# OpenGVLab/MM-Interleaved

Measured on NVIDIA H100. Metric: interleaved_steps_per_sec, higher is better.
Workload: dtype bf16

## Files before the change

include/mmfs_b200.h:

```cpp
#ifndef MMFS_B200_H_
#define MMFS_B200_H_

#include <stdint.h>

#ifdef __cplusplus
extern "C" {
#endif

#define MMFS_B200_ABI_VERSION 3

#define MMFS_OK            0
#define MMFS_EINVAL       (-1)
#define MMFS_EUNSUPPORTED (-2)
#define MMFS_ECUDA        (-3)

#define MMFS_F32  0
#define MMFS_F16  1
#define MMFS_BF16 2
#define MMFS_F64  3

#define MMFS_MSDA_STRICT 1u

#define MMFS_SAMPLER_EXACT_WEIGHTS 4u
#define MMFS_SAMPLER_GENERIC       8u

int mmfs_abi_version(void);
const char *mmfs_last_error(void);

int mmfs_msda_forward(const void *value, const int64_t *spatial_shapes, const int64_t *level_start,
                      const void *sampling_loc, const void *attn_weight, void *out,
                      int N, int S, int M, int D, int L, int Lq, int P,
                      int dtype, unsigned flags, void *stream);

int mmfs_msda_backward(const void *value, const int64_t *spatial_shapes, const int64_t *level_start,
                       const void *sampling_loc, const void *attn_weight, const void *grad_out,
                       float *grad_value, float *grad_loc, float *grad_attn,
                       int N, int S, int M, int D, int L, int Lq, int P, int dtype, void *stream);

int mmfs_msda_backward_deterministic(const void *value, const int64_t *spatial_shapes, const int64_t *level_start,
                                     const void *sampling_loc, const void *attn_weight, const void *grad_out,
                                     long long *grad_value_fixed, float *grad_value, float *grad_loc, float *grad_attn,
                                     float *scratch2, int N, int S, int M, int D, int L, int Lq, int P, int dtype, void *stream);

int mmfs_msda_index_stream(const int64_t *spatial_shapes, const int64_t *level_start,
                           const void *sampling_loc, int32_t *idx,
                           int N, int M, int D, int L, int Lq, int P,
                           int dtype, void *stream);

int mmfs_msda_forward_host(const void *value, const int64_t *spatial_shapes, const int64_t *level_start,
                           const void *sampling_loc, const void *attn_weight, void *out,
                           int N, int S, int M, int D, int L, int Lq, int P,
                           int dtype, unsigned flags, void *stream);
void mmfs_release_scratch(void);

int mmfs_sampler_forward(const void *value, const int64_t *shapes, const int64_t *starts,
                         const void *qproj, const void *rtable, const uint8_t *relpos,
                         const float *refpts, const float *scale_ratios, void *out, float *null_mass,
                         int N, int S, int M, int D, int n_img, int n_lvl, int Lq, int P,
                         int Lq_r, int Nr, int Lr, int R, int dtype, unsigned flags, void *stream);

int mmfs_sampler_locw(const int64_t *shapes, const int64_t *starts, const void *qproj, const void *rtable,
                      const uint8_t *relpos, const float *refpts, const float *scale_ratios,
                      void *loc_out, void *attn_out, float *null_mass,
                      int N, int M, int n_img, int n_lvl, int Lq, int P,
                      int Lq_r, int Nr, int Lr, int R, int dtype, void *stream);

int mmfs_rmsnorm(const void *x, const void *weight, void *y, long rows, int cols, float eps, int dtype, void *stream);
int mmfs_layernorm(const void *x, const void *weight, const void *bias, void *y, long rows, int cols, float eps,
                   int dtype, void *stream);
int mmfs_rope_qk(void *q, void *k, const float *cos_table, const float *sin_table, const int64_t *position_ids,
                 long n_tokens, int T_len, int H, int hd, int q_stride, int k_stride, int pos_per_batch,
                 int dtype, void *stream);
int mmfs_rope_qk_append(void *q, const void *k, const void *v, const float *cos_table, const float *sin_table,
                        const int64_t *position_ids, void *k_cache, void *v_cache, const int64_t *slot_dev, long slot_host,
                        long n_tokens, int T_len, int H, int hd, int q_stride, int k_stride, int v_stride, long cache_bs,
                        long cache_ts, int pos_per_batch, int dtype, void *stream);
int mmfs_swiglu(const void *gate_up, void *out, long rows, int inter, int dtype, void *stream);
int mmfs_geglu(const void *value_gate, void *out, long rows, int inter, int dtype, void *stream);

int mmfs_attn_generic(const void *q, const void *k, const void *v, void *out, const uint8_t *key_mask,
                      int B, int H, int Tq, int Tkv, int hd,
                      long q_bs, long q_ts, long k_bs, long k_ts, long v_bs, long v_ts, long o_bs, long o_ts,
                      float scale, int causal, int past, int dtype, void *stream);
long mmfs_attn_decode_scratch_floats(int B, int H, int Tkv, int hd);
int mmfs_attn_decode(const void *q, const void *k, const void *v, void *out, const uint8_t *key_mask, float *scratch,
                     int B, int H, int Tkv, int hd, long q_bs, long k_bs, long k_ts, long v_bs, long v_ts, long o_bs,
                     float scale, int causal, int past, int dtype, void *stream);
int mmfs_attn_decode_shared(const void *q, const void *k_prefix, const void *v_prefix, const void *k_gen, const void *v_gen,
                            void *out, const uint8_t *key_mask, const long long *prefix_len, float *scratch,
                            int R, int G, int H, int Tkv, int Tp, int max_new, int hd, long q_bs,
                            long kp_bs, long kp_ts, long vp_bs, long vp_ts, long kg_bs, long kg_ts, long vg_bs, long vg_ts,
                            long o_bs, float scale, int causal, int past, int dtype, void *stream);

int mmfs_attn_forward(const void *q, const void *k, const void *v, void *out, const uint8_t *key_mask,
                      int B, int H, int Tq, int Tkv, int hd,
                      long q_bs, long q_ts, long k_bs, long k_ts, long v_bs, long v_ts, long o_bs, long o_ts,
                      float scale, int causal, int past, int dtype, unsigned *work_counter, void *stream);

int mmfs_attn_forward_lse(const void *q, const void *k, const void *v, void *out, float *lse, const uint8_t *key_mask,
                          int B, int H, int Tq, int Tkv, int hd,
                          long q_bs, long q_ts, long k_bs, long k_ts, long v_bs, long v_ts, long o_bs, long o_ts,
                          float scale, int causal, int past, int dtype, unsigned *work_counter, void *stream);

int mmfs_attn_backward(const void *q, const void *k, const void *v, const void *out, const void *d_out, const float *lse,
                       void *dq, void *dk, void *dv, float *delta, const uint8_t *key_mask, int B, int H, int T, int hd,
                       long q_bs, long q_ts, long k_bs, long k_ts, long v_bs, long v_ts, long o_bs, long o_ts,
                       long do_bs, long do_ts, long dq_bs, long dq_ts, long dk_bs, long dk_ts, long dv_bs, long dv_ts,
                       float scale, int dtype, void *stream);

int mmfs_attn_backward_general(const void *q, const void *k, const void *v, const void *out, const void *d_out,
                               const float *lse, void *dq, void *dk, void *dv, float *delta, const uint8_t *key_mask,
                               int B, int H, int Tq, int Tkv, int hd, long q_bs, long q_ts, long k_bs, long k_ts, long v_bs,
                               long v_ts, long o_bs, long o_ts, long do_bs, long do_ts, long dq_bs, long dq_ts, long dk_bs,
                               long dk_ts, long dv_bs, long dv_ts, float scale, int causal, int dtype, void *stream);

int mmfs_layernorm_backward(const void *x, const void *weight, const void *dy, void *dx, void *dweight, void *dbias,
                            float *partials, long rows, int cols, float eps, int dtype, void *stream);

#define MMFS_RMSNORM_BWD_PARTS 256
int mmfs_rmsnorm_backward(const void *x, const void *weight, const void *dy, void *dx, void *dweight, float *partials,
                          long rows, int cols, float eps, int dtype, void *stream);

int mmfs_swiglu_backward(const void *gate_up, const void *d_out, void *d_gate_up, long rows, int inter, int dtype,
                         void *stream);

int mmfs_geglu_backward(const void *value_gate, const void *d_out, void *d_value_gate, long rows, int inter, int dtype,
                        void *stream);

int mmfs_quick_gelu_backward(const void *h, const void *dy, void *dh, long n, int dtype, void *stream);

int mmfs_resize_bilinear_backward(const void *dy, void *dx, int B, int C, int Hin, int Win, int Hout, int Wout, long dy_bs,
                                  long dy_cs, long dy_ps, float scale_h, float scale_w, int dtype, void *stream);

int mmfs_conv2d_nhwc(const void *x, const void *w, const void *bias, const void *add_bc, const void *residual, void *out,
                     int B, int H, int W, int Cin, int Cout, int KH, int KW, int stride, int pad, int dtype, void *stream);

int mmfs_conv2d_up2x_nhwc(const void *x, const void *w_phases, const void *bias, void *out, int B, int H, int W, int Cin,
                          int Cout, int dtype, void *stream);

int mmfs_conv2d_down2x_nhwc(const void *x, const void *w, const void *bias, void *out, int B, int H, int W, int Cin,
                            int Cout, int dtype, void *stream);

int mmfs_groupnorm_nhwc(const void *x, const void *gamma, const void *beta, void *y, float *stats, int B, int HW, int C,
                        int G, float eps, int silu, int dtype, void *stream);

int mmfs_groupnorm_nhwc_backward(const void *x, const void *gamma, const void *beta, const void *dy, void *dx,
                                 float *scratch, int B, int HW, int C, int G, float eps, int silu, int dtype, void *stream);

#define MMFS_SELECT_GREEDY 0
#define MMFS_SELECT_SAMPLE 1

int mmfs_decode_select(const float *logits, long ld, int64_t *out_ids, const int64_t *step, uint8_t *finished,
                       int64_t *next_ids, const int64_t *eos_ids, int n_eos, long pad_id, int min_length,
                       const float *params, const int64_t *seed, const float *uniforms, int B, int V, int max_new,
                       int mode, void *stream);

int mmfs_beam_select(const float *logits, long ld, const int64_t *step, const double *params, float *beam_scores,
                     int64_t *history, int64_t *next_ids, int64_t *parent, uint8_t *done, double *hyp_scores,
                     int64_t *hyp_ids, int64_t *hyp_meta, const int64_t *eos_ids, int n_eos, long pad_id, int min_length,
                     uint64_t *scratch, int B, int num_beams, int V, int max_new, void *stream);

int mmfs_beam_sample(const float *logits, long ld, const int64_t *step, const double *params, const int64_t *seed,
                     const float *uniforms, float *beam_scores, int64_t *history, int64_t *next_ids, int64_t *parent,
                     uint8_t *done, double *hyp_scores, int64_t *hyp_ids, int64_t *hyp_meta, int32_t *error,
                     const int64_t *eos_ids, int n_eos, long pad_id, int min_length, int top_k, uint64_t *scratch, int B,
                     int num_beams, int V, int max_new, void *stream);

int mmfs_kv_beam_reorder(void *cache, int n_caches, long cache_stride, int rows, long row_stride, long pos_stride,
                         long row_bytes, int num_beams, const int64_t *parent, const int64_t *cur, const int64_t *step,
                         const uint8_t *done, int max_positions, void *stream);

int mmfs_image_reentry(const float *images, float *out, int N, int C, int H, int W, int R, void *stream);

int mmfs_linear_fp8(const void *x, const uint8_t *w8, const float *scale, const void *bias, const void *residual,
                    void *out, int M, int N, int K, int dtype, void *stream);

int mmfs_rope_qk_append_fp8(void *q, void *k, void *v, const float *cos_table, const float *sin_table,
                            const int64_t *position_ids, uint8_t *k_cache, uint8_t *v_cache, float *k_scale, float *v_scale,
                            const int64_t *slot_dev, long slot_host, long n_tokens, int T_len, int H, int hd, int q_stride,
                            int k_stride, int v_stride, long cache_bs, long cache_ts, long scale_bs, long scale_ts,
                            int pos_per_batch, int dtype, void *stream);
int mmfs_attn_decode_fp8(const void *q, const uint8_t *k, const uint8_t *v, const float *k_scale, const float *v_scale,
                         void *out, const uint8_t *key_mask, float *scratch, int B, int H, int Tkv, int hd, long q_bs,
                         long kv_bs, long kv_ts, long s_bs, long s_ts, long o_bs, float scale, int causal, int past,
                         int dtype, void *stream);
int mmfs_attn_decode_shared_fp8(const void *q, const uint8_t *k_prefix, const uint8_t *v_prefix, const float *ks_prefix,
                                const float *vs_prefix, const uint8_t *k_gen, const uint8_t *v_gen, const float *ks_gen,
                                const float *vs_gen, void *out, const uint8_t *key_mask, const long long *prefix_len,
                                float *scratch, int R, int G, int H, int Tkv, int Tp, int max_new, int hd, long q_bs,
                                long p_bs, long p_ts, long ps_bs, long ps_ts, long g_bs, long g_ts, long gs_bs, long gs_ts,
                                long o_bs, float scale, int causal, int past, int dtype, void *stream);
int mmfs_kv_dequantize_fp8(const uint8_t *x8, const float *scale, void *out, int B, int T_len, int H, int hd, long x_bs,
                           long x_ts, long s_bs, long s_ts, long o_bs, long o_ts, int dtype, void *stream);

#ifdef __cplusplus
}
#endif
#endif
```

mm-interleaved_b200/_lib.py:

```python
from __future__ import annotations

import ctypes
import os

_HERE = os.path.dirname(os.path.abspath(__file__))
LIB_PATH = os.environ.get("MMFS_B200_LIB", os.path.join(_HERE, "libmmfs_b200.so"))

OK, EINVAL, EUNSUPPORTED, ECUDA = 0, -1, -2, -3
F32, F16, BF16, F64 = 0, 1, 2, 3
MSDA_STRICT = 1
SAMPLER_EXACT_WEIGHTS = 4
SAMPLER_GENERIC = 8
SELECT_GREEDY, SELECT_SAMPLE = 0, 1

_lib = None

_I, _U, _P = ctypes.c_int, ctypes.c_uint, ctypes.c_void_p
_L, _F = ctypes.c_long, ctypes.c_float

SIGNATURES = {
    "mmfs_abi_version": (_I, []),
    "mmfs_last_error": (ctypes.c_char_p, []),
    "mmfs_msda_forward": (_I, [_P, _P, _P, _P, _P, _P, _I, _I, _I, _I, _I, _I, _I, _I, _U, _P]),
    "mmfs_msda_backward": (_I, [_P] * 9 + [_I] * 8 + [_P]),
    "mmfs_msda_backward_deterministic": (_I, [_P] * 11 + [_I] * 8 + [_P]),
    "mmfs_msda_index_stream": (_I, [_P, _P, _P, _P, _I, _I, _I, _I, _I, _I, _I, _P]),
    "mmfs_msda_forward_host": (_I, [_P, _P, _P, _P, _P, _P, _I, _I, _I, _I, _I, _I, _I, _I, _U, _P]),
    "mmfs_release_scratch": (None, []),
    "mmfs_sampler_forward": (_I, [_P] * 10 + [_I] * 13 + [_U, _P]),
    "mmfs_sampler_locw": (_I, [_P] * 10 + [_I] * 11 + [_P]),
    "mmfs_rmsnorm": (_I, [_P, _P, _P, _L, _I, _F, _I, _P]),
    "mmfs_layernorm": (_I, [_P, _P, _P, _P, _L, _I, _F, _I, _P]),
    "mmfs_rope_qk": (_I, [_P, _P, _P, _P, _P, _L, _I, _I, _I, _I, _I, _I, _I, _P]),
    "mmfs_rope_qk_append": (_I, [_P] * 9 + [_L, _L] + [_I] * 6 + [_L, _L, _I, _I, _P]),
    "mmfs_swiglu": (_I, [_P, _P, _L, _I, _I, _P]),
    "mmfs_geglu": (_I, [_P, _P, _L, _I, _I, _P]),
    "mmfs_attn_generic": (_I, [_P] * 5 + [_I] * 5 + [_L] * 8 + [_F, _I, _I, _I, _P]),
    "mmfs_groupnorm_nhwc": (_I, [_P] * 5 + [_I] * 4 + [_F, _I, _I, _P]),
    "mmfs_groupnorm_nhwc_backward": (_I, [_P] * 6 + [_I] * 4 + [_F, _I, _I, _P]),
    "mmfs_conv2d_nhwc": (_I, [_P] * 6 + [_I] * 10 + [_P]),
    "mmfs_conv2d_up2x_nhwc": (_I, [_P] * 4 + [_I] * 6 + [_P]),
    "mmfs_conv2d_down2x_nhwc": (_I, [_P] * 4 + [_I] * 6 + [_P]),
    "mmfs_attn_decode_scratch_floats": (_L, [_I] * 4),
    "mmfs_attn_decode": (_I, [_P] * 6 + [_I] * 4 + [_L] * 6 + [_F, _I, _I, _I, _P]),
    "mmfs_attn_decode_shared": (_I, [_P] * 9 + [_I] * 7 + [_L] * 10 + [_F, _I, _I, _I, _P]),
    "mmfs_attn_forward": (_I, [_P] * 5 + [_I] * 5 + [_L] * 8 + [_F, _I, _I, _I, _P, _P]),
    "mmfs_attn_forward_lse": (_I, [_P] * 6 + [_I] * 5 + [_L] * 8 + [_F, _I, _I, _I, _P, _P]),
    "mmfs_attn_backward": (_I, [_P] * 11 + [_I] * 4 + [_L] * 16 + [_F, _I, _P]),
    "mmfs_attn_backward_general": (_I, [_P] * 11 + [_I] * 5 + [_L] * 16 + [_F, _I, _I, _P]),
    "mmfs_rmsnorm_backward": (_I, [_P] * 6 + [_L, _I, _F, _I, _P]),
    "mmfs_layernorm_backward": (_I, [_P] * 7 + [_L, _I, _F, _I, _P]),
    "mmfs_swiglu_backward": (_I, [_P] * 3 + [_L, _I, _I, _P]),
    "mmfs_geglu_backward": (_I, [_P] * 3 + [_L, _I, _I, _P]),
    "mmfs_quick_gelu_backward": (_I, [_P] * 3 + [_L, _I, _P]),
    "mmfs_resize_bilinear_backward": (_I, [_P] * 2 + [_I] * 6 + [_L] * 3 + [_F, _F, _I, _P]),
    "mmfs_decode_select": (_I, [_P, _L] + [_P] * 5 + [_I, _L, _I] + [_P] * 3 + [_I] * 4 + [_P]),
    "mmfs_beam_select": (_I, [_P, _L] + [_P] * 11 + [_I, _L, _I, _P] + [_I] * 4 + [_P]),
    "mmfs_beam_sample": (_I, [_P, _L] + [_P] * 14 + [_I, _L, _I, _I, _P] + [_I] * 4 + [_P]),
    "mmfs_kv_beam_reorder": (_I, [_P, _I, _L, _I, _L, _L, _L, _I] + [_P] * 4 + [_I, _P]),
    "mmfs_image_reentry": (_I, [_P, _P] + [_I] * 5 + [_P]),
    "mmfs_linear_fp8": (_I, [_P] * 6 + [_I] * 4 + [_P]),
    "mmfs_rope_qk_append_fp8": (_I, [_P] * 11 + [_L, _L] + [_I] * 6 + [_L] * 4 + [_I, _I, _P]),
    "mmfs_attn_decode_fp8": (_I, [_P] * 8 + [_I] * 4 + [_L] * 6 + [_F, _I, _I, _I, _P]),
    "mmfs_attn_decode_shared_fp8": (_I, [_P] * 13 + [_I] * 7 + [_L] * 10 + [_F, _I, _I, _I, _P]),
    "mmfs_kv_dequantize_fp8": (_I, [_P] * 3 + [_I] * 4 + [_L] * 6 + [_I, _P]),
}
BEAM_MAX_BEAMS, BEAM_MAX_EOS = 8, 4
LINEAR_FP8_MAX_M = 64
RMSNORM_BWD_PARTS = 256


def lib() -> ctypes.CDLL:
    global _lib
    if _lib is None:
        if not os.path.exists(LIB_PATH):
            raise RuntimeError(
                f"libmmfs_b200.so not found at {LIB_PATH}: build it with "
                "`python mm-interleaved_b200/build.py` (there is no CPU / PyTorch fallback)")
        handle = ctypes.CDLL(LIB_PATH)
        for name, (res, args) in SIGNATURES.items():
            fn = getattr(handle, name)
            fn.restype = res
            fn.argtypes = args
        if handle.mmfs_abi_version() != 3:
            raise RuntimeError(f"libmmfs_b200.so ABI {handle.mmfs_abi_version()} != 3")
        _lib = handle
    return _lib


def check(rc: int, what: str) -> None:
    if rc != OK:
        msg = lib().mmfs_last_error().decode("utf-8", "replace")
        kind = {EINVAL: "invalid argument", EUNSUPPORTED: "unsupported", ECUDA: "CUDA error"}.get(rc, "error")
        raise RuntimeError(f"{what}: {kind} ({rc}): {msg}")
```

mm-interleaved_b200/csrc/llama_ops_sm100.cu:

```cuda
#include "common.cuh"

namespace mmfs {

template <typename T> __device__ __forceinline__ float rnd(float x) { return to_op(from_op<T>(x)); }
template <> __device__ __forceinline__ float rnd<float>(float x) { return x; }

__device__ __forceinline__ float block_sum(float v, float *s_red) {
#pragma unroll
    for (int o = 16; o > 0; o >>= 1) v += __shfl_xor_sync(0xffffffffu, v, o);
    const int lane = threadIdx.x & 31, warp = threadIdx.x >> 5, nw = (blockDim.x + 31) >> 5;
    if (lane == 0) s_red[warp] = v;
    __syncthreads();
    float t = (lane < nw) ? s_red[lane] : 0.f;
#pragma unroll
    for (int o = 16; o > 0; o >>= 1) t += __shfl_xor_sync(0xffffffffu, t, o);
    __syncthreads();
    return t;
}

template <typename T>
__global__ void __launch_bounds__(256) rmsnorm_kernel(const T *__restrict__ x, const T *__restrict__ w,
                                                       T *__restrict__ y, int cols, float eps) {
    constexpr int VEC = 16 / (int)sizeof(T);
    __shared__ float s_red[32];
    const size_t row = blockIdx.x;
    const T *xr = x + row * cols;
    T *yr = y + row * cols;
    const int nvec = cols / VEC;
    float ss = 0.f;
    for (int i = threadIdx.x; i < nvec; i += blockDim.x) {
        float f[VEC];
        Vec16<T>::unpack(*reinterpret_cast<const uint4 *>(xr + i * VEC), f);
#pragma unroll
        for (int k = 0; k < VEC; ++k) ss += f[k] * f[k];
    }
    for (int i = nvec * VEC + threadIdx.x; i < cols; i += blockDim.x) { const float v = to_op(xr[i]); ss += v * v; }
    const float var = block_sum(ss, s_red) / (float)cols;
    const float r = rsqrtf(var + eps);
    for (int i = threadIdx.x; i < nvec; i += blockDim.x) {
        float f[VEC], g[VEC], o[VEC];
        Vec16<T>::unpack(*reinterpret_cast<const uint4 *>(xr + i * VEC), f);
        Vec16<T>::unpack(*reinterpret_cast<const uint4 *>(w + i * VEC), g);
#pragma unroll
        for (int k = 0; k < VEC; ++k) o[k] = g[k] * rnd<T>(f[k] * r);
        *reinterpret_cast<uint4 *>(yr + i * VEC) = Vec16<T>::pack(o);
    }
    for (int i = nvec * VEC + threadIdx.x; i < cols; i += blockDim.x)
        yr[i] = from_op<T>(to_op(w[i]) * rnd<T>(to_op(xr[i]) * r));
}

constexpr int kRmsChunks = 8;
constexpr int kRmsThreads = 128;

template <typename T>
__global__ void __launch_bounds__(kRmsThreads) rmsnorm_reg_kernel(const T *__restrict__ x, const T *__restrict__ w,
                                                                  T *__restrict__ y, int cols, float eps) {
    constexpr int VEC = 16 / (int)sizeof(T);
    __shared__ float s_red[kRmsThreads / 32];
    const size_t row = blockIdx.x;
    const T *xr = x + row * cols;
    T *yr = y + row * cols;
    const int nvec = cols / VEC;
    uint4 v[kRmsChunks], wv[kRmsChunks];
#pragma unroll
    for (int c = 0; c < kRmsChunks; ++c) {
        const int i = threadIdx.x + c * kRmsThreads;
        if (i < nvec) {
            v[c] = ldg_nc_v4(xr + i * VEC);
            wv[c] = ldg_nc_v4(w + i * VEC);
        }
    }
    float ss = 0.f;
#pragma unroll
    for (int c = 0; c < kRmsChunks; ++c)
        if (threadIdx.x + c * kRmsThreads < nvec) {
            float f[VEC];
            Vec16<T>::unpack(v[c], f);
#pragma unroll
            for (int k = 0; k < VEC; ++k) ss = fmaf(f[k], f[k], ss);
        }
#pragma unroll
    for (int o = 16; o > 0; o >>= 1) ss += __shfl_xor_sync(0xffffffffu, ss, o);
    if ((threadIdx.x & 31) == 0) s_red[threadIdx.x >> 5] = ss;
    __syncthreads();
    float tot = 0.f;
#pragma unroll
    for (int i = 0; i < kRmsThreads / 32; ++i) tot += s_red[i];
    const float r = rsqrtf(tot / (float)cols + eps);
#pragma unroll
    for (int c = 0; c < kRmsChunks; ++c) {
        const int i = threadIdx.x + c * kRmsThreads;
        if (i < nvec) {
            float f[VEC], g[VEC], o[VEC];
            Vec16<T>::unpack(v[c], f);
            Vec16<T>::unpack(wv[c], g);
#pragma unroll
            for (int k = 0; k < VEC; ++k) o[k] = g[k] * rnd<T>(f[k] * r);
            stg_v4(yr + i * VEC, Vec16<T>::pack(o));
        }
    }
}

constexpr int kLnChunks = 8;

template <typename T, int CH>
__global__ void __launch_bounds__(256, CH == 8 ? 2 : 4) layernorm_warp_kernel(const T *__restrict__ x, const T *__restrict__ w,
                                                              const T *__restrict__ b, T *__restrict__ y, long rows, int cols, float eps) {
    constexpr int VEC = 16 / (int)sizeof(T);
    const int lane = threadIdx.x & 31;
    const long row = (long)blockIdx.x * (blockDim.x >> 5) + (threadIdx.x >> 5);
    if (row >= rows) return;
    const T *xr = x + row * cols;
    T *yr = y + row * cols;
    const int nvec = cols / VEC;
    uint4 v[CH];
#pragma unroll
    for (int c = 0; c < CH; ++c) {
        const int i = lane + 32 * c;
        v[c] = (i < nvec) ? ldg_nc_v4(xr + i * VEC) : make_uint4(0u, 0u, 0u, 0u);
    }
    float s = 0.f;
#pragma unroll
    for (int c = 0; c < CH; ++c) {
        float f[VEC];
        Vec16<T>::unpack(v[c], f);
#pragma unroll
        for (int k = 0; k < VEC; ++k) s += f[k];
    }
#pragma unroll
    for (int o = 16; o > 0; o >>= 1) s += __shfl_xor_sync(0xffffffffu, s, o);
    const float mean = s / (float)cols;
    float ss = 0.f;
#pragma unroll
    for (int c = 0; c < CH; ++c)
        if (lane + 32 * c < nvec) {
            float f[VEC];
            Vec16<T>::unpack(v[c], f);
#pragma unroll
            for (int k = 0; k < VEC; ++k) { const float d = f[k] - mean; ss = fmaf(d, d, ss); }
        }
#pragma unroll
    for (int o = 16; o > 0; o >>= 1) ss += __shfl_xor_sync(0xffffffffu, ss, o);
    const float r = rsqrtf(ss / (float)cols + eps);
#pragma unroll
    for (int c = 0; c < CH; ++c) {
        const int i = lane + 32 * c;
        if (i < nvec) {
            float f[VEC], g[VEC], bb[VEC], o[VEC];
            Vec16<T>::unpack(v[c], f);
            if (w) Vec16<T>::unpack(*reinterpret_cast<const uint4 *>(w + i * VEC), g);
            if (b) Vec16<T>::unpack(*reinterpret_cast<const uint4 *>(b + i * VEC), bb);
#pragma unroll
            for (int k = 0; k < VEC; ++k) o[k] = (f[k] - mean) * r * (w ? g[k] : 1.f) + (b ? bb[k] : 0.f);
            stg_v4(yr + i * VEC, Vec16<T>::pack(o));
        }
    }
}

template <typename T>
__global__ void __launch_bounds__(256) layernorm_kernel(const T *__restrict__ x, const T *__restrict__ w,
                                                         const T *__restrict__ b, T *__restrict__ y, int cols, float eps) {
    __shared__ float s_red[32];
    const size_t row = blockIdx.x;
    const T *xr = x + row * cols;
    T *yr = y + row * cols;
    float s = 0.f;
    for (int i = threadIdx.x; i < cols; i += blockDim.x) s += to_op(xr[i]);
    const float mean = block_sum(s, s_red) / (float)cols;
    float ss = 0.f;
    for (int i = threadIdx.x; i < cols; i += blockDim.x) { const float d = to_op(xr[i]) - mean; ss += d * d; }
    const float r = rsqrtf(block_sum(ss, s_red) / (float)cols + eps);
    for (int i = threadIdx.x; i < cols; i += blockDim.x) {
        const float n = (to_op(xr[i]) - mean) * r;
        yr[i] = from_op<T>(n * (w ? to_op(w[i]) : 1.f) + (b ? to_op(b[i]) : 0.f));
    }
}

template <typename T>
__global__ void __launch_bounds__(256) rope_qk_kernel(T *__restrict__ q, T *__restrict__ k, const float *__restrict__ cos_t,
                                                       const float *__restrict__ sin_t, const int64_t *__restrict__ pos,
                                                       long n_tok, int H, int hd, int q_stride, int k_stride, int pos_per_batch,
                                                       int T_len) {
    constexpr int VEC = 16 / (int)sizeof(T);
    const int half = hd >> 1;
    const int chunks = half / VEC;
    const int per_tok = 2 * H * chunks;
    const bool hoist = (blockDim.x % chunks) == 0;
    for (long tok = blockIdx.x; tok < n_tok; tok += gridDim.x) {
        const long p = pos[pos_per_batch ? tok : (tok % T_len)];
        const float *cp = cos_t + p * hd, *sp = sin_t + p * hd;
        T *qt = q + tok * q_stride, *kt = k + tok * k_stride;
        float cs[VEC], sn[VEC];
        auto load_table = [&](int c) {
#pragma unroll
            for (int i = 0; i < VEC; i += 4) {
                const float4 a = *reinterpret_cast<const float4 *>(cp + c * VEC + i);
                const float4 b = *reinterpret_cast<const float4 *>(sp + c * VEC + i);
                cs[i] = rnd<T>(a.x); cs[i + 1] = rnd<T>(a.y); cs[i + 2] = rnd<T>(a.z); cs[i + 3] = rnd<T>(a.w);
                sn[i] = rnd<T>(b.x); sn[i + 1] = rnd<T>(b.y); sn[i + 2] = rnd<T>(b.z); sn[i + 3] = rnd<T>(b.w);
            }
        };
        if (hoist) load_table(threadIdx.x % chunks);
        for (int it = threadIdx.x; it < per_tok; it += blockDim.x) {
            const int c = it % chunks;
            const int hh = it / chunks;
            T *x = (hh >= H ? kt + (size_t)(hh - H) * hd : qt + (size_t)hh * hd) + c * VEC;
            float x1[VEC], x2[VEC], o1[VEC], o2[VEC];
            const uint4 v1 = *reinterpret_cast<const uint4 *>(x), v2 = *reinterpret_cast<const uint4 *>(x + half);
            if (!hoist) load_table(c);
            Vec16<T>::unpack(v1, x1);
            Vec16<T>::unpack(v2, x2);
#pragma unroll
            for (int i = 0; i < VEC; ++i) {
                o1[i] = rnd<T>(x1[i] * cs[i]) + rnd<T>(-x2[i] * sn[i]);
                o2[i] = rnd<T>(x2[i] * cs[i]) + rnd<T>(x1[i] * sn[i]);
            }
            *reinterpret_cast<uint4 *>(x) = Vec16<T>::pack(o1);
            *reinterpret_cast<uint4 *>(x + half) = Vec16<T>::pack(o2);
        }
    }
}

template <typename T>
__global__ void __launch_bounds__(256) rope_append_kernel(T *__restrict__ q, const T *__restrict__ k, const T *__restrict__ v,
                                                           const float *__restrict__ cos_t, const float *__restrict__ sin_t,
                                                           const int64_t *__restrict__ pos, T *__restrict__ k_cache,
                                                           T *__restrict__ v_cache, const int64_t *__restrict__ slot_dev,
                                                           long slot_host, long n_tok, int H, int hd, int q_stride, int k_stride,
                                                           int v_stride, long cache_bs, long cache_ts, int pos_per_batch, int T_len) {
    constexpr int VEC = 16 / (int)sizeof(T);
    const int half = hd >> 1;
    const int chunks = half / VEC;
    const int n_rot = 2 * H * chunks;
    const int n_copy = H * hd / VEC;
    const long slot = slot_dev != nullptr ? (long)*slot_dev : slot_host;
    for (long tok = blockIdx.x; tok < n_tok; tok += gridDim.x) {
        const long p = pos[pos_per_batch ? tok : (tok % T_len)];
        const float *cp = cos_t + p * hd, *sp = sin_t + p * hd;
        const long b = tok / T_len, tt = tok - b * T_len;
        T *qt = q + tok * q_stride;
        const T *kt = k + tok * k_stride, *vt = v + tok * v_stride;
        T *kc = k_cache + b * cache_bs + (slot + tt) * cache_ts, *vc = v_cache + b * cache_bs + (slot + tt) * cache_ts;
        for (int it = threadIdx.x; it < n_rot + n_copy; it += blockDim.x) {
            if (it >= n_rot) {
                const int i = (it - n_rot) * VEC;
                *reinterpret_cast<uint4 *>(vc + i) = *reinterpret_cast<const uint4 *>(vt + i);
                continue;
            }
            const int c = it % chunks, hh = it / chunks;
            const bool is_k = hh >= H;
            const T *src = (is_k ? kt + (size_t)(hh - H) * hd : qt + (size_t)hh * hd) + c * VEC;
            T *dst = (is_k ? kc + (size_t)(hh - H) * hd : qt + (size_t)hh * hd) + c * VEC;
            float cs[VEC], sn[VEC], x1[VEC], x2[VEC], o1[VEC], o2[VEC];
#pragma unroll
            for (int i = 0; i < VEC; i += 4) {
                const float4 a = *reinterpret_cast<const float4 *>(cp + c * VEC + i);
                const float4 bb = *reinterpret_cast<const float4 *>(sp + c * VEC + i);
                cs[i] = rnd<T>(a.x); cs[i + 1] = rnd<T>(a.y); cs[i + 2] = rnd<T>(a.z); cs[i + 3] = rnd<T>(a.w);
                sn[i] = rnd<T>(bb.x); sn[i + 1] = rnd<T>(bb.y); sn[i + 2] = rnd<T>(bb.z); sn[i + 3] = rnd<T>(bb.w);
            }
            Vec16<T>::unpack(*reinterpret_cast<const uint4 *>(src), x1);
            Vec16<T>::unpack(*reinterpret_cast<const uint4 *>(src + half), x2);
#pragma unroll
            for (int i = 0; i < VEC; ++i) {
                o1[i] = rnd<T>(x1[i] * cs[i]) + rnd<T>(-x2[i] * sn[i]);
                o2[i] = rnd<T>(x2[i] * cs[i]) + rnd<T>(x1[i] * sn[i]);
            }
            *reinterpret_cast<uint4 *>(dst) = Vec16<T>::pack(o1);
            *reinterpret_cast<uint4 *>(dst + half) = Vec16<T>::pack(o2);
        }
    }
}

template <typename T> __device__ __forceinline__ float silu_op(float g) { return __fdividef(g, 1.f + __expf(-g)); }
template <> __device__ __forceinline__ float silu_op<float>(float g) { return g / (1.f + expf(-g)); }

template <typename T, int ACT> __device__ __forceinline__ float glu_act(float g) {
    if (ACT == 0) return silu_op<T>(g);
    return 0.5f * g * (1.f + erff(g * 0.70710678118654752f));
}

template <typename T, int ACT = 0, bool GATE_SECOND = false>
__global__ void __launch_bounds__(256) swiglu_kernel(const T *__restrict__ gu, T *__restrict__ out, long rows, int I) {
    constexpr int VEC = 16 / (int)sizeof(T);
    const int per = (I / VEC + gridDim.y - 1) / gridDim.y;
    const int v0 = blockIdx.y * per, nvec = min(I / VEC, v0 + per);
    for (long r = blockIdx.x; r < rows; r += gridDim.x) {
        const T *g_row = gu + r * 2 * I + (GATE_SECOND ? I : 0), *u_row = gu + r * 2 * I + (GATE_SECOND ? 0 : I);
        T *o_row = out + r * I;
        int i = v0 + threadIdx.x;
        for (; i + (int)blockDim.x < nvec; i += 2 * blockDim.x) {
            const int j = i + blockDim.x;
            const uint4 g0 = ldg_nc_v4(g_row + i * VEC), u0 = ldg_nc_v4(u_row + i * VEC);
            const uint4 g1 = ldg_nc_v4(g_row + j * VEC), u1 = ldg_nc_v4(u_row + j * VEC);
            float g[VEC], u[VEC], o[VEC];
            Vec16<T>::unpack(g0, g); Vec16<T>::unpack(u0, u);
#pragma unroll
            for (int k = 0; k < VEC; ++k) o[k] = rnd<T>(glu_act<T, ACT>(g[k])) * u[k];
            stg_v4(o_row + i * VEC, Vec16<T>::pack(o));
            Vec16<T>::unpack(g1, g); Vec16<T>::unpack(u1, u);
#pragma unroll
            for (int k = 0; k < VEC; ++k) o[k] = rnd<T>(glu_act<T, ACT>(g[k])) * u[k];
            stg_v4(o_row + j * VEC, Vec16<T>::pack(o));
        }
        if (i < nvec) {
            float g[VEC], u[VEC], o[VEC];
            Vec16<T>::unpack(ldg_nc_v4(g_row + i * VEC), g); Vec16<T>::unpack(ldg_nc_v4(u_row + i * VEC), u);
#pragma unroll
            for (int k = 0; k < VEC; ++k) o[k] = rnd<T>(glu_act<T, ACT>(g[k])) * u[k];
            stg_v4(o_row + i * VEC, Vec16<T>::pack(o));
        }
    }
}

template <typename T>
static int launch_rmsnorm(const void *x, const void *w, void *y, long rows, int cols, float eps, cudaStream_t st) {
    if (cols % (16 / (int)sizeof(T)) == 0 && cols / (16 / (int)sizeof(T)) <= kRmsThreads * kRmsChunks)
        rmsnorm_reg_kernel<T><<<(unsigned)rows, kRmsThreads, 0, st>>>((const T *)x, (const T *)w, (T *)y, cols, eps);
    else
        rmsnorm_kernel<T><<<(unsigned)rows, 256, 0, st>>>((const T *)x, (const T *)w, (T *)y, cols, eps);
    MMFS_CUDA(cudaGetLastError());
    return MMFS_OK;
}

template <typename T>
static int launch_layernorm(const void *x, const void *w, const void *b, void *y, long rows, int cols, float eps, cudaStream_t st) {
    constexpr int VEC = 16 / (int)sizeof(T);
    const bool vec_ok = (cols % VEC == 0) && (cols / VEC <= 32 * kLnChunks) &&
                        (((uintptr_t)x | (uintptr_t)y | (uintptr_t)w | (uintptr_t)b) % 16 == 0);
    if (vec_ok) {
        const int nvec = cols / VEC;
        const unsigned grid = (unsigned)((rows + 7) / 8);
#define MMFS_LN(CH) layernorm_warp_kernel<T, CH><<<grid, 256, 0, st>>>((const T *)x, (const T *)w, (const T *)b, (T *)y, rows, cols, eps)
        if (nvec <= 32) MMFS_LN(1); else if (nvec <= 64) MMFS_LN(2); else if (nvec <= 128) MMFS_LN(4); else MMFS_LN(8);
#undef MMFS_LN
    } else
        layernorm_kernel<T><<<(unsigned)rows, 256, 0, st>>>((const T *)x, (const T *)w, (const T *)b, (T *)y, cols, eps);
    MMFS_CUDA(cudaGetLastError());
    return MMFS_OK;
}

template <typename T>
static int launch_rope(void *q, void *k, const float *cos_t, const float *sin_t, const int64_t *pos, long n_tok, int T_len,
                       int H, int hd, int qs, int ks, int ppb, cudaStream_t st) {
    const int per_tok = H * 2 * ((hd / 2) / (16 / (int)sizeof(T)));
    const int threads = per_tok >= 256 ? 256 : ((per_tok + 31) / 32) * 32;
    rope_qk_kernel<T><<<capped_grid(n_tok, 32), threads, 0, st>>>((T *)q, (T *)k, cos_t, sin_t, pos, n_tok, H, hd, qs, ks, ppb,
                                                                  T_len);
    MMFS_CUDA(cudaGetLastError());
    return MMFS_OK;
}

template <typename T>
static int launch_glu(const void *in, void *out, long rows, int inter, bool geglu, cudaStream_t st) {
    const int nvec = inter / (16 / (int)sizeof(T));
    const int threads = nvec >= 512 ? 256 : (nvec >= 64 ? 64 : 32);
    const int gx = capped_grid(rows, 64);
    int gy = 1;
    if (gx < num_sms()) { gy = (nvec + 2 * threads - 1) / (2 * threads); if (gy > 64) gy = 64; if (gy < 1) gy = 1; }
    const dim3 grid(gx, gy);
    if (geglu)
        swiglu_kernel<T, 1, true><<<grid, threads, 0, st>>>((const T *)in, (T *)out, rows, inter);
    else
        swiglu_kernel<T, 0, false><<<grid, threads, 0, st>>>((const T *)in, (T *)out, rows, inter);
    MMFS_CUDA(cudaGetLastError());
    return MMFS_OK;
}

template <typename T>
static int launch_rope_append(void *q, const void *k, const void *v, const float *cos_t, const float *sin_t, const int64_t *pos,
                              void *kc, void *vc, const int64_t *slot_dev, long slot_host, long n_tok, int T_len, int H, int hd,
                              int qs, int ks, int vs, long cbs, long cts, int ppb, cudaStream_t st) {
    const int items = H * ((hd / 2) / (16 / (int)sizeof(T))) * 2 + H * hd / (16 / (int)sizeof(T));
    const int threads = items >= 256 ? 256 : ((items + 31) / 32) * 32;
    rope_append_kernel<T><<<capped_grid(n_tok, 32), threads, 0, st>>>((T *)q, (const T *)k, (const T *)v, cos_t, sin_t, pos, (T *)kc,
                                                                      (T *)vc, slot_dev, slot_host, n_tok, H, hd, qs, ks, vs, cbs,
                                                                      cts, ppb, T_len);
    MMFS_CUDA(cudaGetLastError());
    return MMFS_OK;
}


constexpr int kRmsBwdParts = MMFS_RMSNORM_BWD_PARTS;
constexpr int kRmsBwdMaxCols = 8192;

template <typename T>
__global__ void __launch_bounds__(256) rmsnorm_bwd_kernel(const T *__restrict__ x, const T *__restrict__ w,
                                                          const T *__restrict__ dy, T *__restrict__ dx,
                                                          float *__restrict__ partials, long rows, int cols, float eps) {
    constexpr int VEC = 16 / (int)sizeof(T);
    extern __shared__ float s_dw[];
    __shared__ float s_red[32];
    const int nvec = cols / VEC;
    if (partials)
        for (int i = threadIdx.x; i < nvec; i += blockDim.x)
#pragma unroll
            for (int k = 0; k < VEC; ++k) s_dw[i * VEC + k] = 0.f;
    for (long row = blockIdx.x; row < rows; row += gridDim.x) {
        const T *xr = x + row * cols, *dyr = dy + row * cols;
        float ss = 0.f, sg = 0.f;
        for (int i = threadIdx.x; i < nvec; i += blockDim.x) {
            float f[VEC], g[VEC], d[VEC];
            Vec16<T>::unpack(ldg_nc_v4(xr + i * VEC), f);
            Vec16<T>::unpack(ldg_nc_v4(w + i * VEC), g);
            Vec16<T>::unpack(ldg_nc_v4(dyr + i * VEC), d);
#pragma unroll
            for (int k = 0; k < VEC; ++k) { ss = fmaf(f[k], f[k], ss); sg = fmaf(d[k] * g[k], f[k], sg); }
        }
        ss = block_sum(ss, s_red);
        sg = block_sum(sg, s_red);
        const float r = rsqrtf(ss / (float)cols + eps);
        const float coef = r * r * r * sg / (float)cols;
        for (int i = threadIdx.x; i < nvec; i += blockDim.x) {
            float f[VEC], g[VEC], d[VEC], o[VEC];
            Vec16<T>::unpack(ldg_nc_v4(xr + i * VEC), f);
            Vec16<T>::unpack(ldg_nc_v4(w + i * VEC), g);
            Vec16<T>::unpack(ldg_nc_v4(dyr + i * VEC), d);
#pragma unroll
            for (int k = 0; k < VEC; ++k) o[k] = fmaf(r * d[k], g[k], -f[k] * coef);
            stg_v4(dx + row * cols + i * VEC, Vec16<T>::pack(o));
            if (partials)
#pragma unroll
                for (int k = 0; k < VEC; ++k) s_dw[i * VEC + k] = fmaf(d[k], rnd<T>(f[k] * r), s_dw[i * VEC + k]);
        }
    }
    if (partials)
        for (int i = threadIdx.x; i < nvec; i += blockDim.x)
#pragma unroll
            for (int k = 0; k < VEC; ++k) partials[(long)blockIdx.x * cols + i * VEC + k] = s_dw[i * VEC + k];
}

template <typename T>
__global__ void __launch_bounds__(256) rmsnorm_dw_reduce_kernel(const float *__restrict__ partials, T *__restrict__ dw,
                                                                int parts, int cols) {
    const int c = blockIdx.x * blockDim.x + threadIdx.x;
    if (c >= cols) return;
    float s = 0.f;
    for (int p = 0; p < parts; ++p) s += partials[(long)p * cols + c];
    dw[c] = from_op<T>(s);
}

template <typename T>
__global__ void __launch_bounds__(256) layernorm_bwd_kernel(const T *__restrict__ x, const T *__restrict__ w,
                                                            const T *__restrict__ dy, T *__restrict__ dx,
                                                            float *__restrict__ partials, long rows, int cols, float eps) {
    constexpr int VEC = 16 / (int)sizeof(T);
    extern __shared__ float s_part[];
    __shared__ float s_red[32];
    const int nvec = cols / VEC;
    float *s_dw = s_part, *s_db = s_part + cols;
    if (partials)
        for (int i = threadIdx.x; i < nvec; i += blockDim.x)
#pragma unroll
            for (int k = 0; k < VEC; ++k) s_dw[i * VEC + k] = s_db[i * VEC + k] = 0.f;
    const float inv_n = 1.f / (float)cols;
    for (long row = blockIdx.x; row < rows; row += gridDim.x) {
        const T *xr = x + row * cols, *dyr = dy + row * cols;
        float s = 0.f;
        for (int i = threadIdx.x; i < nvec; i += blockDim.x) {
            float f[VEC];
            Vec16<T>::unpack(ldg_nc_v4(xr + i * VEC), f);
#pragma unroll
            for (int k = 0; k < VEC; ++k) s += f[k];
        }
        const float mean = block_sum(s, s_red) * inv_n;
        float ss = 0.f, sg = 0.f, sgx = 0.f;
        for (int i = threadIdx.x; i < nvec; i += blockDim.x) {
            float f[VEC], g[VEC], d[VEC];
            Vec16<T>::unpack(ldg_nc_v4(xr + i * VEC), f);
            Vec16<T>::unpack(ldg_nc_v4(w + i * VEC), g);
            Vec16<T>::unpack(ldg_nc_v4(dyr + i * VEC), d);
#pragma unroll
            for (int k = 0; k < VEC; ++k) {
                const float c = f[k] - mean, gk = d[k] * g[k];
                ss = fmaf(c, c, ss);
                sg += gk;
                sgx = fmaf(gk, c, sgx);
            }
        }
        ss = block_sum(ss, s_red);
        sg = block_sum(sg, s_red);
        sgx = block_sum(sgx, s_red);
        const float r = rsqrtf(ss * inv_n + eps);
        const float mg = sg * inv_n, mgx = sgx * r * inv_n;
        for (int i = threadIdx.x; i < nvec; i += blockDim.x) {
            float f[VEC], g[VEC], d[VEC], o[VEC];
            Vec16<T>::unpack(ldg_nc_v4(xr + i * VEC), f);
            Vec16<T>::unpack(ldg_nc_v4(w + i * VEC), g);
            Vec16<T>::unpack(ldg_nc_v4(dyr + i * VEC), d);
#pragma unroll
            for (int k = 0; k < VEC; ++k) {
                const float xh = (f[k] - mean) * r;
                o[k] = r * (fmaf(d[k], g[k], -mg) - xh * mgx);
                if (partials) {
                    s_dw[i * VEC + k] = fmaf(d[k], xh, s_dw[i * VEC + k]);
                    s_db[i * VEC + k] += d[k];
                }
            }
            stg_v4(dx + row * cols + i * VEC, Vec16<T>::pack(o));
        }
    }
    if (partials)
        for (int i = threadIdx.x; i < nvec; i += blockDim.x)
#pragma unroll
            for (int k = 0; k < VEC; ++k) {
                partials[(long)blockIdx.x * cols + i * VEC + k] = s_dw[i * VEC + k];
                partials[((long)gridDim.x + blockIdx.x) * cols + i * VEC + k] = s_db[i * VEC + k];
            }
}

template <typename T>
__global__ void __launch_bounds__(256) layernorm_dwdb_reduce_kernel(const float *__restrict__ partials, T *__restrict__ dw,
                                                                    T *__restrict__ db, int parts, int cols) {
    const int c = blockIdx.x * blockDim.x + threadIdx.x;
    if (c >= cols) return;
    float sw = 0.f, sb = 0.f;
    for (int p = 0; p < parts; ++p) {
        sw += partials[(long)p * cols + c];
        sb += partials[((long)parts + p) * cols + c];
    }
    if (dw) dw[c] = from_op<T>(sw);
    if (db) db[c] = from_op<T>(sb);
}

template <typename T>
__global__ void __launch_bounds__(256) swiglu_bwd_kernel(const T *__restrict__ gu, const T *__restrict__ d_out,
                                                         T *__restrict__ d_gu, long rows, int I) {
    constexpr int VEC = 16 / (int)sizeof(T);
    const int nvec = I / VEC;
    for (long r = blockIdx.x; r < rows; r += gridDim.x)
        for (int i = threadIdx.x; i < nvec; i += blockDim.x) {
            float g[VEC], u[VEC], d[VEC], dg[VEC], du[VEC];
            Vec16<T>::unpack(ldg_nc_v4(gu + r * 2 * I + i * VEC), g);
            Vec16<T>::unpack(ldg_nc_v4(gu + r * 2 * I + I + i * VEC), u);
            Vec16<T>::unpack(ldg_nc_v4(d_out + r * I + i * VEC), d);
#pragma unroll
            for (int k = 0; k < VEC; ++k) {
                const float s = 1.f / (1.f + expf(-g[k]));
                dg[k] = d[k] * u[k] * s * fmaf(g[k], 1.f - s, 1.f);
                du[k] = d[k] * g[k] * s;
            }
            stg_v4(d_gu + r * 2 * I + i * VEC, Vec16<T>::pack(dg));
            stg_v4(d_gu + r * 2 * I + I + i * VEC, Vec16<T>::pack(du));
        }
}

__device__ __forceinline__ void geglu_grad(float v, float g, float d, float &dv, float &dg) {
    const float cdf = 0.5f * (1.f + erff(g * 0.70710678118654752f));
    const float pdf = 0.39894228040143268f * expf(-0.5f * g * g);
    dv = d * g * cdf;
    dg = d * v * fmaf(g, pdf, cdf);
}

template <typename T, bool kVec>
__global__ void __launch_bounds__(256) geglu_bwd_kernel(const T *__restrict__ vg, const T *__restrict__ d_out,
                                                        T *__restrict__ d_vg, long rows, int I) {
    constexpr int VEC = kVec ? 16 / (int)sizeof(T) : 1;
    const long per_row = I / VEC, n = rows * per_row;
    const long stride = (long)gridDim.x * blockDim.x;
    for (long t = (long)blockIdx.x * blockDim.x + threadIdx.x; t < n; t += stride) {
        const long r = t / per_row, i = (t - r * per_row) * VEC;
        const long v_at = r * 2 * I + i, g_at = v_at + I;
        float v[VEC], g[VEC], d[VEC], dv[VEC], dg[VEC];
        if constexpr (kVec) {
            Vec16<T>::unpack(ldg_nc_v4(vg + v_at), v);
            Vec16<T>::unpack(ldg_nc_v4(vg + g_at), g);
            Vec16<T>::unpack(ldg_nc_v4(d_out + r * I + i), d);
        } else {
            v[0] = to_op(vg[v_at]);
            g[0] = to_op(vg[g_at]);
            d[0] = to_op(d_out[r * I + i]);
        }
#pragma unroll
        for (int k = 0; k < VEC; ++k) geglu_grad(v[k], g[k], d[k], dv[k], dg[k]);
        if constexpr (kVec) {
            stg_v4(d_vg + v_at, Vec16<T>::pack(dv));
            stg_v4(d_vg + g_at, Vec16<T>::pack(dg));
        } else {
            d_vg[v_at] = from_op<T>(dv[0]);
            d_vg[g_at] = from_op<T>(dg[0]);
        }
    }
}

template <typename T>
static int launch_geglu_bwd(const void *vg, const void *d_out, void *d_vg, long rows, int inter, bool vec, cudaStream_t st) {
    const long items = rows * (vec ? inter / (16 / (int)sizeof(T)) : inter);
    const int grid = capped_grid((items + 255) / 256, 8);
    if (vec)
        geglu_bwd_kernel<T, true><<<grid, 256, 0, st>>>((const T *)vg, (const T *)d_out, (T *)d_vg, rows, inter);
    else
        geglu_bwd_kernel<T, false><<<grid, 256, 0, st>>>((const T *)vg, (const T *)d_out, (T *)d_vg, rows, inter);
    MMFS_CUDA(cudaGetLastError());
    return MMFS_OK;
}

template <typename T>
static int launch_rmsnorm_bwd(const void *x, const void *w, const void *dy, void *dx, void *dw, float *partials, long rows,
                              int cols, float eps, cudaStream_t st) {
    const int parts = (int)(rows < kRmsBwdParts ? rows : kRmsBwdParts);
    rmsnorm_bwd_kernel<T><<<parts, 256, dw ? cols * sizeof(float) : 0, st>>>(
        (const T *)x, (const T *)w, (const T *)dy, (T *)dx, dw ? partials : nullptr, rows, cols, eps);
    MMFS_CUDA(cudaGetLastError());
    if (dw) {
        rmsnorm_dw_reduce_kernel<T><<<(cols + 255) / 256, 256, 0, st>>>(partials, (T *)dw, parts, cols);
        MMFS_CUDA(cudaGetLastError());
    }
    return MMFS_OK;
}

template <typename T>
static int launch_layernorm_bwd(const void *x, const void *w, const void *dy, void *dx, void *dw, void *db, float *partials,
                                long rows, int cols, float eps, cudaStream_t st) {
    const int parts = (int)(rows < kRmsBwdParts ? rows : kRmsBwdParts);
    const int nvec = cols / (16 / (int)sizeof(T));
    const int threads = nvec >= 256 ? 256 : (nvec + 31) / 32 * 32;
    const bool red = dw != nullptr || db != nullptr;
    const size_t smem = red ? 2 * (size_t)cols * sizeof(float) : 0;
    const int rc = ensure_dynamic_smem<layernorm_bwd_kernel<T>>(smem);
    if (rc != MMFS_OK) return rc;
    layernorm_bwd_kernel<T><<<parts, threads, smem, st>>>((const T *)x, (const T *)w, (const T *)dy, (T *)dx,
                                                           red ? partials : nullptr, rows, cols, eps);
    MMFS_CUDA(cudaGetLastError());
    if (red) {
        layernorm_dwdb_reduce_kernel<T><<<(cols + 255) / 256, 256, 0, st>>>(partials, (T *)dw, (T *)db, parts, cols);
        MMFS_CUDA(cudaGetLastError());
    }
    return MMFS_OK;
}

template <typename T>
static int launch_swiglu_bwd(const void *gu, const void *d_out, void *d_gu, long rows, int inter, cudaStream_t st) {
    swiglu_bwd_kernel<T><<<capped_grid(rows, 8), 256, 0, st>>>((const T *)gu, (const T *)d_out, (T *)d_gu, rows, inter);
    MMFS_CUDA(cudaGetLastError());
    return MMFS_OK;
}

}

using namespace mmfs;

extern "C" int mmfs_rmsnorm(const void *x, const void *weight, void *y, long rows, int cols, float eps, int dtype, void *stream) {
    MMFS_CHECK_ARG(rows >= 0 && cols > 0, "rmsnorm: bad shape");
    if (rows == 0) return MMFS_OK;
    MMFS_CHECK_ARG(x && weight && y, "rmsnorm: null pointer argument");
    MMFS_CHECK_ARG(((uintptr_t)x | (uintptr_t)weight | (uintptr_t)y) % 16 == 0 && (cols * dtype_size(dtype)) % 16 == 0,
                   "rmsnorm: rows must be 16-byte aligned");
    return dispatch_dtype<kF32Types>(dtype, "rmsnorm", [&](auto tag) {
        return launch_rmsnorm<typename decltype(tag)::type>(x, weight, y, rows, cols, eps, (cudaStream_t)stream);
    });
}

extern "C" int mmfs_layernorm(const void *x, const void *weight, const void *bias, void *y, long rows, int cols, float eps,
                              int dtype, void *stream) {
    MMFS_CHECK_ARG(rows >= 0 && cols > 0, "layernorm: bad shape");
    if (rows == 0) return MMFS_OK;
    MMFS_CHECK_ARG(x && y, "layernorm: null pointer argument");
    return dispatch_dtype<kF32Types>(dtype, "layernorm", [&](auto tag) {
        return launch_layernorm<typename decltype(tag)::type>(x, weight, bias, y, rows, cols, eps, (cudaStream_t)stream);
    });
}

extern "C" int mmfs_rope_qk(void *q, void *k, const float *cos_table, const float *sin_table, const int64_t *position_ids,
                            long n_tokens, int T_len, int H, int hd, int q_stride, int k_stride, int pos_per_batch,
                            int dtype, void *stream) {
    MMFS_CHECK_ARG(n_tokens >= 0 && H > 0 && hd > 0 && hd % 2 == 0 && T_len > 0, "rope_qk: bad shape");
    if (n_tokens == 0) return MMFS_OK;
    MMFS_CHECK_ARG(q && k && cos_table && sin_table && position_ids, "rope_qk: null pointer argument");
    MMFS_CHECK_ARG((hd / 2) % (16 / (int)dtype_size(dtype)) == 0 && ((uintptr_t)q | (uintptr_t)k) % 16 == 0 &&
                   (q_stride * dtype_size(dtype)) % 16 == 0 && (k_stride * dtype_size(dtype)) % 16 == 0,
                   "rope_qk: head_dim/2 must be a multiple of the 16-byte vector and rows 16-byte aligned");
    return dispatch_dtype<kF32Types>(dtype, "rope_qk", [&](auto tag) {
        return launch_rope<typename decltype(tag)::type>(q, k, cos_table, sin_table, position_ids, n_tokens, T_len, H, hd, q_stride,
                                                         k_stride, pos_per_batch, (cudaStream_t)stream);
    });
}

extern "C" int mmfs_rope_qk_append(void *q, const void *k, const void *v, const float *cos_table, const float *sin_table,
                                   const int64_t *position_ids, void *k_cache, void *v_cache, const int64_t *slot_dev,
                                   long slot_host, long n_tokens, int T_len, int H, int hd, int q_stride, int k_stride,
                                   int v_stride, long cache_bs, long cache_ts, int pos_per_batch, int dtype, void *stream) {
    MMFS_CHECK_ARG(n_tokens >= 0 && H > 0 && hd > 0 && hd % 2 == 0 && T_len > 0 && slot_host >= 0, "rope_qk_append: bad shape");
    if (n_tokens == 0) return MMFS_OK;
    MMFS_CHECK_ARG(q && k && v && cos_table && sin_table && position_ids && k_cache && v_cache, "rope_qk_append: null pointer argument");
    const size_t es = dtype_size(dtype);
    MMFS_CHECK_ARG(es == 2 || es == 4, "rope_qk_append: f32 / f16 / bf16");
    MMFS_CHECK_ARG((hd / 2) % (16 / (int)es) == 0 &&
                       ((uintptr_t)q | (uintptr_t)k | (uintptr_t)v | (uintptr_t)k_cache | (uintptr_t)v_cache) % 16 == 0 &&
                       (q_stride * es) % 16 == 0 && (k_stride * es) % 16 == 0 && (v_stride * es) % 16 == 0 &&
                       (cache_bs * es) % 16 == 0 && (cache_ts * es) % 16 == 0,
                   "rope_qk_append: head_dim/2 must be a multiple of the 16-byte vector and all rows 16-byte aligned");
    return dispatch_dtype<kF32Types>(dtype, "rope_qk_append", [&](auto tag) {
        return launch_rope_append<typename decltype(tag)::type>(q, k, v, cos_table, sin_table, position_ids, k_cache, v_cache,
                                                                slot_dev, slot_host, n_tokens, T_len, H, hd, q_stride, k_stride,
                                                                v_stride, cache_bs, cache_ts, pos_per_batch, (cudaStream_t)stream);
    });
}

extern "C" int mmfs_swiglu(const void *gate_up, void *out, long rows, int inter, int dtype, void *stream) {
    MMFS_CHECK_ARG(rows >= 0 && inter > 0, "swiglu: bad shape");
    if (rows == 0) return MMFS_OK;
    MMFS_CHECK_ARG(gate_up && out, "swiglu: null pointer argument");
    MMFS_CHECK_ARG(((uintptr_t)gate_up | (uintptr_t)out) % 16 == 0 && (inter * dtype_size(dtype)) % 16 == 0,
                   "swiglu: rows must be 16-byte aligned");
    return dispatch_dtype<kF32Types>(dtype, "swiglu", [&](auto tag) {
        return launch_glu<typename decltype(tag)::type>(gate_up, out, rows, inter, false, (cudaStream_t)stream);
    });
}

extern "C" int mmfs_geglu(const void *value_gate, void *out, long rows, int inter, int dtype, void *stream) {
    MMFS_CHECK_ARG(rows >= 0 && inter > 0, "geglu: bad shape");
    if (rows == 0) return MMFS_OK;
    MMFS_CHECK_ARG(value_gate && out, "geglu: null pointer argument");
    MMFS_CHECK_ARG(((uintptr_t)value_gate | (uintptr_t)out) % 16 == 0 && (inter * dtype_size(dtype)) % 16 == 0,
                   "geglu: rows must be 16-byte aligned");
    return dispatch_dtype<kF32Types>(dtype, "geglu", [&](auto tag) {
        return launch_glu<typename decltype(tag)::type>(value_gate, out, rows, inter, true, (cudaStream_t)stream);
    });
}

extern "C" int mmfs_rmsnorm_backward(const void *x, const void *weight, const void *dy, void *dx, void *dweight,
                                     float *partials, long rows, int cols, float eps, int dtype, void *stream) {
    MMFS_CHECK_ARG(rows >= 0 && cols > 0, "rmsnorm_backward: bad shape");
    if (rows == 0) return MMFS_OK;
    MMFS_CHECK_ARG(x && weight && dy && dx && (!dweight || partials), "rmsnorm_backward: null pointer argument");
    if (!(dtype == MMFS_BF16 || dtype == MMFS_F16) || cols % 8 != 0 || cols > kRmsBwdMaxCols ||
        ((uintptr_t)x | (uintptr_t)weight | (uintptr_t)dy | (uintptr_t)dx) % 16 != 0) {
        set_error("rmsnorm_backward: needs bf16 / f16, cols %% 8 == 0, cols <= %d, 16-byte aligned rows (got cols=%d dtype=%d)",
                  kRmsBwdMaxCols, cols, dtype);
        return MMFS_EUNSUPPORTED;
    }
    return dispatch_dtype<kF16Types, MMFS_EUNSUPPORTED>(dtype, "rmsnorm_backward", [&](auto tag) {
        return launch_rmsnorm_bwd<typename decltype(tag)::type>(x, weight, dy, dx, dweight, partials, rows, cols, eps,
                                                                (cudaStream_t)stream);
    });
}

extern "C" int mmfs_swiglu_backward(const void *gate_up, const void *d_out, void *d_gate_up, long rows, int inter, int dtype,
                                    void *stream) {
    MMFS_CHECK_ARG(rows >= 0 && inter > 0, "swiglu_backward: bad shape");
    if (rows == 0) return MMFS_OK;
    MMFS_CHECK_ARG(gate_up && d_out && d_gate_up, "swiglu_backward: null pointer argument");
    if (!(dtype == MMFS_BF16 || dtype == MMFS_F16) || inter % 8 != 0 ||
        ((uintptr_t)gate_up | (uintptr_t)d_out | (uintptr_t)d_gate_up) % 16 != 0) {
        set_error("swiglu_backward: needs bf16 / f16, inter %% 8 == 0 and 16-byte aligned rows (got inter=%d dtype=%d)", inter, dtype);
        return MMFS_EUNSUPPORTED;
    }
    return dispatch_dtype<kF16Types, MMFS_EUNSUPPORTED>(dtype, "swiglu_backward", [&](auto tag) {
        return launch_swiglu_bwd<typename decltype(tag)::type>(gate_up, d_out, d_gate_up, rows, inter, (cudaStream_t)stream);
    });
}

extern "C" int mmfs_geglu_backward(const void *value_gate, const void *d_out, void *d_value_gate, long rows, int inter,
                                   int dtype, void *stream) {
    MMFS_CHECK_ARG(rows >= 0 && inter > 0, "geglu_backward: bad shape");
    if (rows == 0) return MMFS_OK;
    MMFS_CHECK_ARG(value_gate && d_out && d_value_gate, "geglu_backward: null pointer argument");
    if (!(dtype == MMFS_BF16 || dtype == MMFS_F16)) {
        set_error("geglu_backward: needs bf16 / f16 (got dtype=%d)", dtype);
        return MMFS_EUNSUPPORTED;
    }
    const bool vec = inter % 8 == 0 && ((uintptr_t)value_gate | (uintptr_t)d_out | (uintptr_t)d_value_gate) % 16 == 0;
    return dispatch_dtype<kF16Types, MMFS_EUNSUPPORTED>(dtype, "geglu_backward", [&](auto tag) {
        return launch_geglu_bwd<typename decltype(tag)::type>(value_gate, d_out, d_value_gate, rows, inter, vec,
                                                              (cudaStream_t)stream);
    });
}

extern "C" int mmfs_layernorm_backward(const void *x, const void *weight, const void *dy, void *dx, void *dweight, void *dbias,
                                       float *partials, long rows, int cols, float eps, int dtype, void *stream) {
    MMFS_CHECK_ARG(rows >= 0 && cols > 0, "layernorm_backward: bad shape");
    if (rows == 0) return MMFS_OK;
    MMFS_CHECK_ARG(x && weight && dy && dx && (!(dweight || dbias) || partials), "layernorm_backward: null pointer argument");
    if (!(dtype == MMFS_BF16 || dtype == MMFS_F16) || cols % 8 != 0 || cols > kRmsBwdMaxCols ||
        ((uintptr_t)x | (uintptr_t)weight | (uintptr_t)dy | (uintptr_t)dx) % 16 != 0) {
        set_error("layernorm_backward: needs bf16 / f16, cols %% 8 == 0, cols <= %d, 16-byte aligned rows (got cols=%d dtype=%d)",
                  kRmsBwdMaxCols, cols, dtype);
        return MMFS_EUNSUPPORTED;
    }
    return dispatch_dtype<kF16Types, MMFS_EUNSUPPORTED>(dtype, "layernorm_backward", [&](auto tag) {
        return launch_layernorm_bwd<typename decltype(tag)::type>(x, weight, dy, dx, dweight, dbias, partials, rows, cols, eps,
                                                                  (cudaStream_t)stream);
    });
}
```

mm-interleaved_b200/csrc/tc_common.cuh:

```cuda
#pragma once
#include <cuda.h>

#include "common.cuh"

namespace mmfs {

__device__ __forceinline__ void tma_load_4d(void *dst, const CUtensorMap *map, uint64_t *bar, int c0, int c1, int c2, int c3) {
    asm volatile(
        "cp.async.bulk.tensor.4d.shared::cluster.global.mbarrier::complete_tx::bytes [%0], [%1, {%3, %4, %5, %6}], [%2];" ::
        "r"(s_addr(dst)), "l"(map), "r"(s_addr(bar)), "r"(c0), "r"(c1), "r"(c2), "r"(c3) : "memory");
}
__device__ __forceinline__ void fence_async_smem() { asm volatile("fence.proxy.async.shared::cta;" ::: "memory"); }

__device__ __forceinline__ void wgmma_fence() { asm volatile("wgmma.fence.sync.aligned;" ::: "memory"); }
__device__ __forceinline__ void wgmma_commit() { asm volatile("wgmma.commit_group.sync.aligned;" ::: "memory"); }
template <int N> __device__ __forceinline__ void wgmma_wait() { asm volatile("wgmma.wait_group.sync.aligned %0;" ::"n"(N) : "memory"); }
template <int N> __device__ __forceinline__ void reg_fence(float (&d)[N]) {
#pragma unroll
    for (int i = 0; i < N; ++i) asm volatile("" : "+f"(d[i])::"memory");
}

__device__ __forceinline__ uint64_t smem_desc(uint32_t saddr, uint32_t lbo_bytes, uint32_t sbo_bytes) {
    return (uint64_t)((saddr >> 4) & 0x3fffu) | ((uint64_t)((lbo_bytes >> 4) & 0x3fffu) << 16) |
           ((uint64_t)((sbo_bytes >> 4) & 0x3fffu) << 32) | (1ull << 62);
}

template <typename T> struct Wgmma;
#define MMFS_WGMMA_OPS(TY) \
     \
    __device__ __forceinline__ static void ss_n64(float (&d)[32], uint64_t da, uint64_t db, int acc) { \
        asm volatile( \
            "{\n\t.reg .pred p;\n\tsetp.ne.b32 p, %34, 0;\n\t" \
            "wgmma.mma_async.sync.aligned.m64n64k16.f32." TY "." TY " {%0,%1,%2,%3,%4,%5,%6,%7,%8,%9,%10,%11,%12,%13,%14,%15,%16,%17,%18,%19,%20,%21,%22,%23,%24,%25,%26,%27,%28,%29,%30,%31}, %32, %33, p, 1, 1, 0, 0;\n\t}" \
            : "+f"(d[0]), "+f"(d[1]), "+f"(d[2]), "+f"(d[3]), "+f"(d[4]), "+f"(d[5]), "+f"(d[6]), "+f"(d[7]), "+f"(d[8]), "+f"(d[9]), "+f"(d[10]), "+f"(d[11]), "+f"(d[12]), "+f"(d[13]), "+f"(d[14]), "+f"(d[15]), "+f"(d[16]), "+f"(d[17]), "+f"(d[18]), "+f"(d[19]), "+f"(d[20]), "+f"(d[21]), "+f"(d[22]), "+f"(d[23]), "+f"(d[24]), "+f"(d[25]), "+f"(d[26]), "+f"(d[27]), "+f"(d[28]), "+f"(d[29]), "+f"(d[30]), "+f"(d[31]) \
            : "l"(da), "l"(db), "r"(acc)); \
    } \
     \
    __device__ __forceinline__ static void ss_n128(float (&d)[64], uint64_t da, uint64_t db, int acc) { \
        asm volatile( \
            "{\n\t.reg .pred p;\n\tsetp.ne.b32 p, %66, 0;\n\t" \
            "wgmma.mma_async.sync.aligned.m64n128k16.f32." TY "." TY " {%0,%1,%2,%3,%4,%5,%6,%7,%8,%9,%10,%11,%12,%13,%14,%15,%16,%17,%18,%19,%20,%21,%22,%23,%24,%25,%26,%27,%28,%29,%30,%31,%32,%33,%34,%35,%36,%37,%38,%39,%40,%41,%42,%43,%44,%45,%46,%47,%48,%49,%50,%51,%52,%53,%54,%55,%56,%57,%58,%59,%60,%61,%62,%63}, %64, %65, p, 1, 1, 0, 0;\n\t}" \
            : "+f"(d[0]), "+f"(d[1]), "+f"(d[2]), "+f"(d[3]), "+f"(d[4]), "+f"(d[5]), "+f"(d[6]), "+f"(d[7]), "+f"(d[8]), "+f"(d[9]), "+f"(d[10]), "+f"(d[11]), "+f"(d[12]), "+f"(d[13]), "+f"(d[14]), "+f"(d[15]), "+f"(d[16]), "+f"(d[17]), "+f"(d[18]), "+f"(d[19]), "+f"(d[20]), "+f"(d[21]), "+f"(d[22]), "+f"(d[23]), "+f"(d[24]), "+f"(d[25]), "+f"(d[26]), "+f"(d[27]), "+f"(d[28]), "+f"(d[29]), "+f"(d[30]), "+f"(d[31]), "+f"(d[32]), "+f"(d[33]), "+f"(d[34]), "+f"(d[35]), "+f"(d[36]), "+f"(d[37]), "+f"(d[38]), "+f"(d[39]), "+f"(d[40]), "+f"(d[41]), "+f"(d[42]), "+f"(d[43]), "+f"(d[44]), "+f"(d[45]), "+f"(d[46]), "+f"(d[47]), "+f"(d[48]), "+f"(d[49]), "+f"(d[50]), "+f"(d[51]), "+f"(d[52]), "+f"(d[53]), "+f"(d[54]), "+f"(d[55]), "+f"(d[56]), "+f"(d[57]), "+f"(d[58]), "+f"(d[59]), "+f"(d[60]), "+f"(d[61]), "+f"(d[62]), "+f"(d[63]) \
            : "l"(da), "l"(db), "r"(acc)); \
    } \
     \
    __device__ __forceinline__ static void ss_n160(float (&d)[80], uint64_t da, uint64_t db, int acc) { \
        asm volatile( \
            "{\n\t.reg .pred p;\n\tsetp.ne.b32 p, %82, 0;\n\t" \
            "wgmma.mma_async.sync.aligned.m64n160k16.f32." TY "." TY " {%0,%1,%2,%3,%4,%5,%6,%7,%8,%9,%10,%11,%12,%13,%14,%15,%16,%17,%18,%19,%20,%21,%22,%23,%24,%25,%26,%27,%28,%29,%30,%31,%32,%33,%34,%35,%36,%37,%38,%39,%40,%41,%42,%43,%44,%45,%46,%47,%48,%49,%50,%51,%52,%53,%54,%55,%56,%57,%58,%59,%60,%61,%62,%63,%64,%65,%66,%67,%68,%69,%70,%71,%72,%73,%74,%75,%76,%77,%78,%79}, %80, %81, p, 1, 1, 0, 0;\n\t}" \
            : "+f"(d[0]), "+f"(d[1]), "+f"(d[2]), "+f"(d[3]), "+f"(d[4]), "+f"(d[5]), "+f"(d[6]), "+f"(d[7]), "+f"(d[8]), "+f"(d[9]), "+f"(d[10]), "+f"(d[11]), "+f"(d[12]), "+f"(d[13]), "+f"(d[14]), "+f"(d[15]), "+f"(d[16]), "+f"(d[17]), "+f"(d[18]), "+f"(d[19]), "+f"(d[20]), "+f"(d[21]), "+f"(d[22]), "+f"(d[23]), "+f"(d[24]), "+f"(d[25]), "+f"(d[26]), "+f"(d[27]), "+f"(d[28]), "+f"(d[29]), "+f"(d[30]), "+f"(d[31]), "+f"(d[32]), "+f"(d[33]), "+f"(d[34]), "+f"(d[35]), "+f"(d[36]), "+f"(d[37]), "+f"(d[38]), "+f"(d[39]), "+f"(d[40]), "+f"(d[41]), "+f"(d[42]), "+f"(d[43]), "+f"(d[44]), "+f"(d[45]), "+f"(d[46]), "+f"(d[47]), "+f"(d[48]), "+f"(d[49]), "+f"(d[50]), "+f"(d[51]), "+f"(d[52]), "+f"(d[53]), "+f"(d[54]), "+f"(d[55]), "+f"(d[56]), "+f"(d[57]), "+f"(d[58]), "+f"(d[59]), "+f"(d[60]), "+f"(d[61]), "+f"(d[62]), "+f"(d[63]), "+f"(d[64]), "+f"(d[65]), "+f"(d[66]), "+f"(d[67]), "+f"(d[68]), "+f"(d[69]), "+f"(d[70]), "+f"(d[71]), "+f"(d[72]), "+f"(d[73]), "+f"(d[74]), "+f"(d[75]), "+f"(d[76]), "+f"(d[77]), "+f"(d[78]), "+f"(d[79]) \
            : "l"(da), "l"(db), "r"(acc)); \
    } \
     \
    __device__ __forceinline__ static void rs_n64(float (&d)[32], const uint32_t (&a)[4], uint64_t db, int acc) { \
        asm volatile( \
            "{\n\t.reg .pred p;\n\tsetp.ne.b32 p, %37, 0;\n\t" \
            "wgmma.mma_async.sync.aligned.m64n64k16.f32." TY "." TY " {%0,%1,%2,%3,%4,%5,%6,%7,%8,%9,%10,%11,%12,%13,%14,%15,%16,%17,%18,%19,%20,%21,%22,%23,%24,%25,%26,%27,%28,%29,%30,%31}, {%32,%33,%34,%35}, %36, p, 1, 1, 1;\n\t}" \
            : "+f"(d[0]), "+f"(d[1]), "+f"(d[2]), "+f"(d[3]), "+f"(d[4]), "+f"(d[5]), "+f"(d[6]), "+f"(d[7]), "+f"(d[8]), "+f"(d[9]), "+f"(d[10]), "+f"(d[11]), "+f"(d[12]), "+f"(d[13]), "+f"(d[14]), "+f"(d[15]), "+f"(d[16]), "+f"(d[17]), "+f"(d[18]), "+f"(d[19]), "+f"(d[20]), "+f"(d[21]), "+f"(d[22]), "+f"(d[23]), "+f"(d[24]), "+f"(d[25]), "+f"(d[26]), "+f"(d[27]), "+f"(d[28]), "+f"(d[29]), "+f"(d[30]), "+f"(d[31]) \
            : "r"(a[0]), "r"(a[1]), "r"(a[2]), "r"(a[3]), "l"(db), "r"(acc)); \
    } \
     \
    __device__ __forceinline__ static void rs_n128(float (&d)[64], const uint32_t (&a)[4], uint64_t db, int acc) { \
        asm volatile( \
            "{\n\t.reg .pred p;\n\tsetp.ne.b32 p, %69, 0;\n\t" \
            "wgmma.mma_async.sync.aligned.m64n128k16.f32." TY "." TY " {%0,%1,%2,%3,%4,%5,%6,%7,%8,%9,%10,%11,%12,%13,%14,%15,%16,%17,%18,%19,%20,%21,%22,%23,%24,%25,%26,%27,%28,%29,%30,%31,%32,%33,%34,%35,%36,%37,%38,%39,%40,%41,%42,%43,%44,%45,%46,%47,%48,%49,%50,%51,%52,%53,%54,%55,%56,%57,%58,%59,%60,%61,%62,%63}, {%64,%65,%66,%67}, %68, p, 1, 1, 1;\n\t}" \
            : "+f"(d[0]), "+f"(d[1]), "+f"(d[2]), "+f"(d[3]), "+f"(d[4]), "+f"(d[5]), "+f"(d[6]), "+f"(d[7]), "+f"(d[8]), "+f"(d[9]), "+f"(d[10]), "+f"(d[11]), "+f"(d[12]), "+f"(d[13]), "+f"(d[14]), "+f"(d[15]), "+f"(d[16]), "+f"(d[17]), "+f"(d[18]), "+f"(d[19]), "+f"(d[20]), "+f"(d[21]), "+f"(d[22]), "+f"(d[23]), "+f"(d[24]), "+f"(d[25]), "+f"(d[26]), "+f"(d[27]), "+f"(d[28]), "+f"(d[29]), "+f"(d[30]), "+f"(d[31]), "+f"(d[32]), "+f"(d[33]), "+f"(d[34]), "+f"(d[35]), "+f"(d[36]), "+f"(d[37]), "+f"(d[38]), "+f"(d[39]), "+f"(d[40]), "+f"(d[41]), "+f"(d[42]), "+f"(d[43]), "+f"(d[44]), "+f"(d[45]), "+f"(d[46]), "+f"(d[47]), "+f"(d[48]), "+f"(d[49]), "+f"(d[50]), "+f"(d[51]), "+f"(d[52]), "+f"(d[53]), "+f"(d[54]), "+f"(d[55]), "+f"(d[56]), "+f"(d[57]), "+f"(d[58]), "+f"(d[59]), "+f"(d[60]), "+f"(d[61]), "+f"(d[62]), "+f"(d[63]) \
            : "r"(a[0]), "r"(a[1]), "r"(a[2]), "r"(a[3]), "l"(db), "r"(acc)); \
    }
template <> struct Wgmma<__nv_bfloat16> { MMFS_WGMMA_OPS("bf16") };
template <> struct Wgmma<__half> { MMFS_WGMMA_OPS("f16") };
#undef MMFS_WGMMA_OPS


__device__ __forceinline__ void tma_load_2d(void *dst, const CUtensorMap *map, uint64_t *bar, int c0, int c1) {
    asm volatile(
        "cp.async.bulk.tensor.2d.shared::cluster.global.mbarrier::complete_tx::bytes [%0], [%1, {%3, %4}], [%2];" ::
        "r"(s_addr(dst)), "l"(map), "r"(s_addr(bar)), "r"(c0), "r"(c1) : "memory");
}

typedef CUresult (*EncodeTiledFn)(CUtensorMap *, CUtensorMapDataType, cuuint32_t, void *, const cuuint64_t *, const cuuint64_t *,
                                  const cuuint32_t *, const cuuint32_t *, CUtensorMapInterleave, CUtensorMapSwizzle,
                                  CUtensorMapL2promotion, CUtensorMapFloatOOBfill);

inline EncodeTiledFn tensor_map_encoder() {
    static EncodeTiledFn fn = nullptr;
    if (!fn) {
        void *ptr = nullptr;
        cudaDriverEntryPointQueryResult qres;
        if (cudaGetDriverEntryPoint("cuTensorMapEncodeTiled", &ptr, cudaEnableDefault, &qres) == cudaSuccess &&
            qres == cudaDriverEntryPointSuccess)
            fn = (EncodeTiledFn)ptr;
    }
    return fn;
}

}
```

mm-interleaved_b200/llama_mmfs.py:

```python
from __future__ import annotations

import math
from dataclasses import dataclass, field
from types import SimpleNamespace
from typing import List, Optional, Tuple

import torch
import torch.nn.functional as F
from torch import nn

import torch.utils.checkpoint

from . import autograd_ops, ops
from ._cache import SourceCache, WeightCache
from .mmfs import MMFS
from .msda import records


@dataclass
class LlamaMMFSConfig:
    vocab_size: int = 32002
    hidden_size: int = 5120
    intermediate_size: int = 13824
    num_hidden_layers: int = 40
    num_attention_heads: int = 40
    hidden_act: str = "silu"
    max_position_embeddings: int = 2048
    rms_norm_eps: float = 1e-6
    pad_token_id: int = 0
    cross_attention_frequency: int = 4
    spatial_shapes: List[int] = field(default_factory=lambda: [32, 16, 8])
    image_embed_dim: int = 1024
    use_cache: bool = True


class LlamaRMSNorm(nn.Module):
    def __init__(self, hidden_size, eps=1e-6):
        super().__init__()
        self.weight = nn.Parameter(torch.ones(hidden_size))
        self.variance_epsilon = eps

    def forward(self, hidden_states):
        return autograd_ops.rmsnorm(hidden_states, self.weight, self.variance_epsilon)


def rotary_tables(dim: int, max_pos: int, base: float = 10000.0, device=None):
    inv_freq = 1.0 / (base ** (torch.arange(0, dim, 2, device=device).float() / dim))
    t = torch.arange(max_pos, device=device, dtype=torch.float32)
    freqs = torch.outer(t, inv_freq)
    emb = torch.cat((freqs, freqs), dim=-1)
    return emb.cos().contiguous(), emb.sin().contiguous()


_ROPE_TABLES = {}


def shared_rotary_tables(dim: int, need_pos: int, min_pos: int, device):
    key = (str(device), dim)
    hit = _ROPE_TABLES.get(key)
    if hit is None or hit[0] < need_pos:
        n = max(min_pos, need_pos if hit is None else max(need_pos, 2 * hit[0]))
        hit = (n,) + rotary_tables(dim, n, device=device)
        _ROPE_TABLES[key] = hit
    return hit[1], hit[2]


class _CatWeight:

    def __init__(self, *linears):
        self.linears = linears
        self._cache = WeightCache()

    def get(self):
        ws = [l.weight for l in self.linears]
        if records(*ws):
            return torch.cat(ws, 0)
        return self._cache.get(ws, lambda: torch.cat(ws, 0).contiguous())


def _addmm_residual(residual, x, weight, inplace):
    r2 = residual.view(-1, residual.shape[-1])
    x2 = x.reshape(-1, x.shape[-1])
    if inplace:
        r2.addmm_(x2, weight.t())
        return residual
    return torch.addmm(r2, x2, weight.t()).view_as(residual)


FP8_DECODE_MAX_ROWS = 5


def decode_linear(x, weight, fp8, key, bias=None, residual=None, inplace=False):
    if (fp8 is not None and x.dim() == 3 and x.shape[1] == 1 and x.shape[0] <= FP8_DECODE_MAX_ROWS
            and weight.shape[0] >= 2 * weight.shape[1] and not records(x, residual)):
        w8, scale = fp8.get(weight, lambda: ops.quantize_fp8_per_channel(weight), key)
        return ops.linear_fp8(x, w8, scale, bias, residual, out=residual if inplace else None)
    if residual is None:
        return F.linear(x, weight, bias)
    return _addmm_residual(residual, x, weight, inplace)


class LlamaMLP(nn.Module):
    def __init__(self, hidden_size: int, intermediate_size: int, hidden_act: str):
        super().__init__()
        if hidden_act != "silu":
            raise NotImplementedError("only the SiLU gate of Llama is implemented")
        self.gate_proj = nn.Linear(hidden_size, intermediate_size, bias=False)
        self.down_proj = nn.Linear(intermediate_size, hidden_size, bias=False)
        self.up_proj = nn.Linear(hidden_size, intermediate_size, bias=False)
        self._gate_up = _CatWeight(self.gate_proj, self.up_proj)
        self._fp8 = None

    def forward(self, x, residual=None, inplace=False):
        gu = decode_linear(x, self._gate_up.get(), self._fp8, "gate_up")
        act = autograd_ops.swiglu(gu)
        return decode_linear(act, self.down_proj.weight, self._fp8, "down", residual=residual, inplace=inplace)


class StaticKV:

    __slots__ = ("k", "v", "k_scale", "v_scale", "length", "slot")

    def __init__(self, batch, max_len, heads, head_dim, dtype, device, kv_fp8=False):
        kv, scales = kv_storage(2, batch, max_len, heads, head_dim, dtype, device, kv_fp8, torch.empty)
        self.k, self.v = kv[0], kv[1]
        self.k_scale, self.v_scale = (None, None) if scales is None else (scales[0], scales[1])
        self.length = 0
        self.slot = None

    @classmethod
    def over(cls, k, v, k_scale=None, v_scale=None) -> "StaticKV":
        c = cls.__new__(cls)
        c.k, c.v, c.k_scale, c.v_scale, c.length, c.slot = k, v, k_scale, v_scale, 0, None
        return c

    @property
    def fp8(self) -> bool:
        return self.k_scale is not None

    def _tensors(self):
        if self.k_scale is None:
            return self.k, self.v
        return self.k.view(torch.uint8), self.v.view(torch.uint8), self.k_scale, self.v_scale

    def copy_rows_(self, src: "StaticKV", rows: torch.Tensor, n: int) -> None:
        if src.fp8 != self.fp8:
            raise RuntimeError("StaticKV.copy_rows_: an FP8 and a 16-bit cache do not mix")
        for dst, s in zip(self._tensors(), src._tensors()):
            dst[:, :n].copy_(s[:, :n].index_select(0, rows))

    def reorder_rows_(self, rows: torch.Tensor, n: int) -> None:
        for t in self._tensors():
            t[:, :n].copy_(t.index_select(0, rows)[:, :n])

    def zero_from_(self, n: int) -> None:
        for t in self._tensors():
            t[:, n:].zero_()


def kv_storage(n, rows, max_len, heads, head_dim, dtype, device, kv_fp8=False, alloc=torch.zeros):
    data = alloc((n, rows, max_len, heads, head_dim), dtype=torch.float8_e4m3fn if kv_fp8 else dtype, device=device)
    if not kv_fp8:
        return data, None
    return data, torch.ones((n, rows, max_len, ops.kv_scale_heads(heads)), dtype=torch.float32, device=device)


class SharedPrefixKV:

    __slots__ = ("k", "v", "k_gen", "v_gen", "G", "prefix_len", "slot", "k_scale", "v_scale", "ks_gen", "vs_gen")

    def __init__(self, k, v, k_gen, v_gen, prefix_len, slot, scales=None):
        self.k, self.v, self.k_gen, self.v_gen = k, v, k_gen, v_gen
        self.G = k_gen.shape[0] // k.shape[0]
        self.prefix_len, self.slot = prefix_len, slot
        self.k_scale, self.v_scale, self.ks_gen, self.vs_gen = scales if scales is not None else (None,) * 4

    @property
    def length(self):
        return self.k.shape[1] + self.k_gen.shape[1] - 1


class PreparedVision:

    __slots__ = ("raw_shape", "values")

    def __init__(self, raw_shape):
        self.raw_shape = tuple(raw_shape)
        self.values = {}


class LlamaAttention(nn.Module):
    def __init__(self, config: LlamaMMFSConfig):
        super().__init__()
        self.config = config
        self.hidden_size = config.hidden_size
        self.num_heads = config.num_attention_heads
        self.head_dim = self.hidden_size // self.num_heads
        self.max_position_embeddings = config.max_position_embeddings
        if self.head_dim * self.num_heads != self.hidden_size:
            raise ValueError("hidden_size must be divisible by num_heads")
        self.q_proj = nn.Linear(self.hidden_size, self.hidden_size, bias=False)
        self.k_proj = nn.Linear(self.hidden_size, self.hidden_size, bias=False)
        self.v_proj = nn.Linear(self.hidden_size, self.hidden_size, bias=False)
        self.o_proj = nn.Linear(self.hidden_size, self.hidden_size, bias=False)
        self._qkv = _CatWeight(self.q_proj, self.k_proj, self.v_proj)
        self._rope = None
        self._fp8 = None

    def rope_tables(self, device, need_pos):
        if self._rope is None or self._rope[0] != device or self._rope[1] < need_pos:
            cos, sin = shared_rotary_tables(self.head_dim, need_pos, self.max_position_embeddings, device)
            self._rope = (device, cos.shape[0], cos, sin)
        return self._rope[2], self._rope[3]

    def forward(self, hidden_states, attention_mask=None, position_ids=None, past_key_value=None,
                output_attentions=False, use_cache=False, residual=None, inplace=False):
        if output_attentions:
            raise NotImplementedError("attention probabilities are never materialised by the fused kernel")
        B, T, _ = hidden_states.shape
        H, hd = self.num_heads, self.head_dim
        if records(hidden_states, residual, self):
            return self._forward_training(hidden_states, attention_mask, position_ids, past_key_value, use_cache, residual)
        qkv = decode_linear(hidden_states, self._qkv.get(), self._fp8, "qkv").view(B, T, 3, H, hd)
        q, k, v = qkv[:, :, 0], qkv[:, :, 1], qkv[:, :, 2]
        shared = isinstance(past_key_value, SharedPrefixKV)
        static = shared or isinstance(past_key_value, StaticKV)
        past = 0 if past_key_value is None else (past_key_value.length if static else past_key_value[0].shape[1])
        if position_ids is None:
            position_ids = torch.arange(past, past + T, device=hidden_states.device)
        cos, sin = self.rope_tables(hidden_states.device, past + T)
        if static and past_key_value.k_scale is not None:
            return self._forward_fp8(q, k, v, cos, sin, position_ids, past_key_value, past, attention_mask, residual,
                                     inplace)
        if shared:
            if T != 1:
                raise RuntimeError("SharedPrefixKV is a graph-decode cache (one token per step): prefill into its prefix "
                                   "through StaticKV.over, and decode eagerly over a StaticKV")
            ops.rope_qk_append_(q, k, v, cos, sin, position_ids, past_key_value.k_gen, past_key_value.v_gen,
                                past_key_value.slot)
            present = past_key_value
        elif static and past_key_value.slot is not None:
            if T != 1:
                raise RuntimeError("StaticKV.slot (graph decode) takes one token per step")
            ops.rope_qk_append_(q, k, v, cos, sin, position_ids, past_key_value.k, past_key_value.v, past_key_value.slot)
            k, v = past_key_value.k, past_key_value.v
            past = k.shape[1] - 1
            present = past_key_value
        elif static:
            if past + T > past_key_value.k.shape[1]:
                raise RuntimeError(f"StaticKV of {past_key_value.k.shape[1]} positions cannot take {past} + {T}")
            ops.rope_qk_append_(q, k, v, cos, sin, position_ids, past_key_value.k, past_key_value.v, past)
            past_key_value.length = past + T
            k, v = past_key_value.k[:, :past + T], past_key_value.v[:, :past + T]
            present = past_key_value
        else:
            ops.rope_qk_(q, k, cos, sin, position_ids)
            if past_key_value is not None:
                k = torch.cat([past_key_value[0], k], dim=1)
                v = torch.cat([past_key_value[1], v], dim=1)
            present = (k, v) if use_cache else None
        key_mask = None
        if attention_mask is not None:
            if attention_mask.dim() == 4:
                key_mask = attention_mask[:, 0, -1, :] > (torch.finfo(attention_mask.dtype).min / 2)
            else:
                key_mask = attention_mask
        if shared:
            c = past_key_value
            ctx = ops.attention_decode_shared(q, c.k, c.v, c.k_gen, c.v_gen, c.prefix_len, key_mask=key_mask, past=past)
        else:
            ctx = ops.attention(q, k, v, key_mask=key_mask, causal=True, past=past)
        out = decode_linear(ctx, self.o_proj.weight, self._fp8, "o", residual=residual, inplace=inplace)
        return out, None, present

    def _forward_fp8(self, q, k, v, cos, sin, position_ids, c, past, attention_mask, residual, inplace):
        B, T = q.shape[:2]
        shared = isinstance(c, SharedPrefixKV)
        if (shared or c.slot is not None) and T != 1:
            raise RuntimeError("a graph-decode cache (SharedPrefixKV, StaticKV.slot) takes one token per step")
        key_mask = attention_mask
        if attention_mask is not None and attention_mask.dim() == 4:
            key_mask = attention_mask[:, 0, -1, :] > (torch.finfo(attention_mask.dtype).min / 2)
        if shared:
            ops.rope_qk_append_fp8_(q, k, v, cos, sin, position_ids, c.k_gen, c.v_gen, c.ks_gen, c.vs_gen, c.slot)
            ctx = ops.attention_decode_shared_fp8(q, c.k, c.v, c.k_scale, c.v_scale, c.k_gen, c.v_gen, c.ks_gen, c.vs_gen,
                                                  c.prefix_len, key_mask=key_mask, past=past)
        else:
            if c.slot is not None:
                slot, n, past = c.slot, c.k.shape[1], c.k.shape[1] - 1
            else:
                if past + T > c.k.shape[1]:
                    raise RuntimeError(f"StaticKV of {c.k.shape[1]} positions cannot take {past} + {T}")
                slot, n = past, past + T
                c.length = n
            ops.rope_qk_append_fp8_(q, k, v, cos, sin, position_ids, c.k, c.v, c.k_scale, c.v_scale, slot)
            if T == 1:
                ctx = ops.attention_decode_fp8(q, c.k[:, :n], c.v[:, :n], c.k_scale[:, :n], c.v_scale[:, :n],
                                               key_mask=key_mask, past=past)
            else:
                if past > 0:
                    k = ops.kv_dequantize_fp8(c.k[:, :n], c.k_scale[:, :n], q.dtype)
                    v = ops.kv_dequantize_fp8(c.v[:, :n], c.v_scale[:, :n], q.dtype)
                ctx = ops.attention(q, k, v, key_mask=key_mask, causal=True, past=past)
        out = decode_linear(ctx, self.o_proj.weight, self._fp8, "o", residual=residual, inplace=inplace)
        return out, None, c

    def _forward_training(self, hidden_states, attention_mask, position_ids, past_key_value, use_cache, residual):
        if past_key_value is not None or use_cache:
            raise RuntimeError("LlamaAttention under autograd runs the prefill without a KV cache: pass use_cache=False "
                               "and no past_key_values, or run under torch.no_grad()")
        autograd_ops.check_training_dtype("LlamaAttention", hidden_states)
        if self.head_dim != 128:
            raise RuntimeError(f"LlamaAttention under autograd needs head dim 128 (the attention backward kernel's), "
                               f"got {self.head_dim}")
        B, T, _ = hidden_states.shape
        qkv = F.linear(hidden_states, self._qkv.get()).view(B, T, 3, self.num_heads, self.head_dim)
        if position_ids is None:
            position_ids = torch.arange(T, device=hidden_states.device)
        cos, sin = self.rope_tables(hidden_states.device, T)
        qkv = autograd_ops.rope_qkv(qkv, cos, sin, position_ids)
        key_mask = attention_mask
        if attention_mask is not None and attention_mask.dim() == 4:
            key_mask = attention_mask[:, 0, -1, :] > (torch.finfo(attention_mask.dtype).min / 2)
        ctx = autograd_ops.attention(qkv, key_mask)
        out = self.o_proj(ctx) if residual is None else _addmm_residual(residual, ctx, self.o_proj.weight, False)
        return out, None, None


class LlamaMMFSAttention(nn.Module):
    def __init__(self, config: LlamaMMFSConfig, layer_idx):
        super().__init__()
        self.layer_idx = layer_idx
        self.config = config
        self.spatial_shapes = [(s, s) for s in config.spatial_shapes]
        self.hidden_size = config.hidden_size
        self.vision_hidden_size = config.image_embed_dim
        self.gate = nn.Parameter(torch.tensor([0.0]))
        self.attn = MMFS(layer_idx=layer_idx, d_model=self.hidden_size, d_query=self.hidden_size,
                         d_value=self.vision_hidden_size, d_out=self.hidden_size,
                         n_levels=len(config.spatial_shapes), n_heads=16, n_points=8,
                         ratio=self.vision_hidden_size / self.hidden_size, offset_init_magnitude=3.0,
                         spatial_shapes=config.spatial_shapes, max_num_image_per_seq=50)
        self.norm1 = LlamaRMSNorm(config.hidden_size, eps=config.rms_norm_eps)
        self.norm2 = LlamaRMSNorm(self.vision_hidden_size, eps=config.rms_norm_eps)
        self._vision_cache = SourceCache()
        self._gated = WeightCache()
        self._geom_cache = {}

    def _geometry(self, device, n_img, hw, len_q):
        per_img = sum(h * w for h, w in self.spatial_shapes)
        if hw != per_img:
            raise RuntimeError(f"vision features have {hw} positions per image, expected {per_img}")
        key = ("s", device, n_img)
        if key not in self._geom_cache:
            ss = torch.tensor(self.spatial_shapes * n_img, dtype=torch.long)
            starts = torch.cat((ss.new_zeros((1,)), ss.prod(1).cumsum(0)[:-1]))
            self._geom_cache[key] = (ss.to(device), starts.to(device))
        rkey = ("r", device, len_q)
        if rkey not in self._geom_cache:
            self._geom_cache[rkey] = torch.full((1, len_q, 1, 2), 0.5, dtype=torch.float32, device=device)
        return self._geom_cache[key] + (self._geom_cache[rkey],)

    def _gated_output(self):
        w, b, g = ps = self.attn.output_proj.weight, self.attn.output_proj.bias, self.gate

        def build():
            t = g.float().tanh()
            return (w.float() * t).to(w.dtype), (b.float() * t).to(b.dtype)
        return self._gated.get(ps, build)

    def project_vision(self, vision_hidden_states):
        return self.attn.project_value(self.norm2(vision_hidden_states))

    def forward(self, hidden_states, vision_hidden_states=None, cross_attention_mask=None, residual=None, inplace=False):
        if records(hidden_states, residual, vision_hidden_states, self):
            return self._forward_training(hidden_states, vision_hidden_states, cross_attention_mask, residual)
        h = self.norm1(hidden_states)
        value = None
        if isinstance(vision_hidden_states, PreparedVision):
            value = vision_hidden_states.values[self.layer_idx]
            _, n_img, hw, _ = vision_hidden_states.raw_shape
            v = None
        else:
            v = self._vision_cache.get_or_build((vision_hidden_states, self.norm2.weight),
                                                lambda: self.norm2(vision_hidden_states), cache=not torch.is_grad_enabled())
            _, n_img, hw, _ = v.shape
        shapes, starts, ref = self._geometry(h.device, n_img, hw, h.shape[1])
        if not torch.is_grad_enabled():
            gw, gb = self._gated_output()
            out = self.attn(query=h, reference_points=ref, input_flatten=v, input_spatial_shapes=shapes,
                            input_level_start_index=starts, input_padding_mask=None, attention_mask=cross_attention_mask,
                            output_weight=gw, output_bias=gb, value=value)
            if residual is None:
                return out
            return residual.add_(out) if inplace else residual + out
        out = self.attn(query=h, reference_points=ref, input_flatten=v, input_spatial_shapes=shapes,
                        input_level_start_index=starts, input_padding_mask=None, attention_mask=cross_attention_mask,
                        value=value)
        gate = self.gate.tanh().to(out.dtype)
        if residual is None:
            return out * gate
        return torch.addcmul(residual, out, gate)

    def _forward_training(self, hidden_states, vision_hidden_states, cross_attention_mask, residual):
        if isinstance(vision_hidden_states, PreparedVision):
            raise RuntimeError("LlamaMMFSAttention under autograd takes the vision feature tensor, not PreparedVision "
                               "(an inference-only cache)")
        h = self.norm1(hidden_states)
        v = self.norm2(vision_hidden_states)
        _, n_img, hw, _ = v.shape
        shapes, starts, ref = self._geometry(h.device, n_img, hw, h.shape[1])
        out = self.attn.forward_differentiable(h, ref, v, shapes, starts, cross_attention_mask)
        out = out * self.gate.tanh().to(out.dtype)
        return out if residual is None else residual + out


class LlamaDecoderLayer(nn.Module):
    def __init__(self, config: LlamaMMFSConfig, use_cross_attn: bool, layer_idx):
        super().__init__()
        self.hidden_size = config.hidden_size
        self.self_attn = LlamaAttention(config=config)
        self.layer_idx = layer_idx
        self.llama_cross_attn = LlamaMMFSAttention(config=config, layer_idx=layer_idx) if use_cross_attn else None
        self.mlp = LlamaMLP(self.hidden_size, config.intermediate_size, config.hidden_act)
        self.input_layernorm = LlamaRMSNorm(config.hidden_size, eps=config.rms_norm_eps)
        self.post_attention_layernorm = LlamaRMSNorm(config.hidden_size, eps=config.rms_norm_eps)

    def forward(self, hidden_states, vision_hidden_states, cross_attention_mask, attention_mask=None,
                position_ids=None, past_key_value=None, output_attentions=False, use_cache=False, inplace=False):
        residual = hidden_states.contiguous()
        inplace = inplace and not torch.is_grad_enabled()
        hidden_states, _, present = self.self_attn(self.input_layernorm(residual), attention_mask=attention_mask,
                                                   position_ids=position_ids, past_key_value=past_key_value,
                                                   use_cache=use_cache, residual=residual, inplace=inplace)
        if self.llama_cross_attn is not None and vision_hidden_states is not None:
            hidden_states = self.llama_cross_attn(hidden_states, vision_hidden_states, cross_attention_mask,
                                                  residual=hidden_states, inplace=inplace)
        hidden_states = self.mlp(self.post_attention_layernorm(hidden_states), residual=hidden_states, inplace=inplace)
        outputs = (hidden_states,)
        if use_cache:
            outputs += (present,)
        return outputs


class LlamaModel(nn.Module):

    def __init__(self, config: LlamaMMFSConfig):
        super().__init__()
        self.config = config
        self.padding_idx = config.pad_token_id
        self.vocab_size = config.vocab_size
        self.cross_attention_frequency = config.cross_attention_frequency
        self.embed_tokens = nn.Embedding(config.vocab_size, config.hidden_size, self.padding_idx)
        use_cross = [i % self.cross_attention_frequency == 0 for i in range(config.num_hidden_layers)]
        self.layers = nn.ModuleList([LlamaDecoderLayer(config, use_cross[i], i) for i in range(config.num_hidden_layers)])
        self.norm = LlamaRMSNorm(config.hidden_size, eps=config.rms_norm_eps)
        self.gradient_checkpointing = False

    def static_cache(self, batch: int, max_len: int, dtype=None, device=None, kv_fp8: bool = False):
        p = self.embed_tokens.weight
        H = self.config.num_attention_heads
        return [StaticKV(batch, max_len, H, self.config.hidden_size // H, dtype or p.dtype, device or p.device, kv_fp8)
                for _ in self.layers]

    @torch.no_grad()
    def prepare_vision(self, vision_hidden_states, out: Optional[PreparedVision] = None) -> PreparedVision:
        pv = PreparedVision(vision_hidden_states.shape) if out is None else out
        if tuple(vision_hidden_states.shape) != pv.raw_shape:
            raise RuntimeError(f"prepare_vision: features {tuple(vision_hidden_states.shape)} do not fit {pv.raw_shape}")
        for layer in self.layers:
            if layer.llama_cross_attn is None:
                continue
            val = layer.llama_cross_attn.project_vision(vision_hidden_states)
            if out is None:
                pv.values[layer.layer_idx] = val
            else:
                pv.values[layer.layer_idx].copy_(val)
        return pv

    def get_input_embeddings(self):
        return self.embed_tokens

    def set_input_embeddings(self, value):
        self.embed_tokens = value

    def forward(self, input_ids=None, attention_mask=None, position_ids=None, past_key_values=None,
                inputs_embeds=None, vision_hidden_states=None, cross_attention_mask=None, use_cache=None,
                output_attentions=None, output_hidden_states=None, return_dict=None):
        training = records(inputs_embeds, vision_hidden_states, self)
        if use_cache is None:
            use_cache = False if training else self.config.use_cache
        return_dict = True if return_dict is None else return_dict
        if output_attentions:
            raise NotImplementedError("attention probabilities are never materialised")
        if input_ids is not None and inputs_embeds is not None:
            raise ValueError("You cannot specify both decoder_input_ids and decoder_inputs_embeds at the same time")
        if input_ids is None and inputs_embeds is None:
            raise ValueError("You have to specify either decoder_input_ids or decoder_inputs_embeds")
        if inputs_embeds is None:
            inputs_embeds = self.embed_tokens(input_ids)
        B, T, _ = inputs_embeds.shape
        if past_key_values is None:
            past = 0
        else:
            past = (past_key_values[0].length if isinstance(past_key_values[0], (StaticKV, SharedPrefixKV))
                    else past_key_values[0][0].shape[1])
        if position_ids is None:
            position_ids = torch.arange(past, past + T, dtype=torch.long, device=inputs_embeds.device)
        else:
            position_ids = position_ids.view(-1, T).long()
        key_mask = None
        if attention_mask is not None:
            if tuple(attention_mask.shape) != (B, past + T):
                raise ValueError(f"attention_mask should be of size {(B, past + T)}, but is {tuple(attention_mask.shape)}")
            key_mask = attention_mask.to(torch.uint8)

        if training:
            if use_cache or past_key_values is not None:
                raise RuntimeError("LlamaModel under autograd runs the prefill without a KV cache: pass use_cache=False "
                                   "and no past_key_values, or run under torch.no_grad()")
            autograd_ops.check_training_dtype("LlamaModel", inputs_embeds)
        hidden_states = inputs_embeds
        inplace = not torch.is_grad_enabled() and not output_hidden_states
        if inplace:
            hidden_states = hidden_states.clone(memory_format=torch.contiguous_format)
        all_hidden = () if output_hidden_states else None
        next_cache = () if use_cache else None
        for idx, layer in enumerate(self.layers):
            if output_hidden_states:
                all_hidden += (hidden_states,)
            if training and self.gradient_checkpointing:
                outs = torch.utils.checkpoint.checkpoint(layer, hidden_states, vision_hidden_states, cross_attention_mask,
                                                         attention_mask=key_mask, position_ids=position_ids,
                                                         use_reentrant=False)
            else:
                outs = layer(hidden_states, vision_hidden_states, cross_attention_mask, attention_mask=key_mask,
                             position_ids=position_ids,
                             past_key_value=past_key_values[idx] if past_key_values is not None else None,
                             use_cache=use_cache, inplace=inplace)
            hidden_states = outs[0]
            if use_cache:
                next_cache += (outs[1],)
        hidden_states = self.norm(hidden_states)
        if output_hidden_states:
            all_hidden += (hidden_states,)
        if not return_dict:
            return tuple(v for v in [hidden_states, next_cache, all_hidden] if v is not None)
        return SimpleNamespace(last_hidden_state=hidden_states, past_key_values=next_cache, hidden_states=all_hidden,
                               attentions=None)
```

mm-interleaved_b200/ops.py:

```python
from __future__ import annotations

import math
from typing import Optional

import torch

from . import _lib
from .msda import _DTYPE_CODE, _require, inference_only

launch_counter = [0]


def _stream():
    return torch.cuda.current_stream().cuda_stream


def rmsnorm(x: torch.Tensor, weight: torch.Tensor, eps: float) -> torch.Tensor:
    inference_only("rmsnorm", x, weight)
    _require(x.is_cuda and x.is_contiguous() and weight.is_contiguous(), "rmsnorm: contiguous CUDA tensors required")
    _require(weight.dtype == x.dtype and weight.numel() == x.shape[-1], "rmsnorm: weight dtype / size mismatch")
    y = torch.empty_like(x)
    rows = x.numel() // x.shape[-1]
    with torch.cuda.device(x.device):
        rc = _lib.lib().mmfs_rmsnorm(x.data_ptr(), weight.data_ptr(), y.data_ptr(), rows, x.shape[-1], float(eps),
                                     _DTYPE_CODE[x.dtype], _stream())
    _lib.check(rc, "rmsnorm")
    launch_counter[0] += 1
    return y


def _check_affine(what: str, x: torch.Tensor, n: int, *params) -> None:
    for p in params:
        if p is not None:
            _require(p.dtype == x.dtype and p.numel() == n and p.is_contiguous() and p.device == x.device,
                     f"{what}: weight / bias must be contiguous {x.dtype} tensors of {n} elements on {x.device}")


def layernorm(x: torch.Tensor, weight, bias, eps: float) -> torch.Tensor:
    inference_only("layernorm", x, weight, bias)
    _require(x.is_cuda and x.is_contiguous(), "layernorm: contiguous CUDA tensor required")
    _check_affine("layernorm", x, x.shape[-1], weight, bias)
    y = torch.empty_like(x)
    rows = x.numel() // x.shape[-1]
    with torch.cuda.device(x.device):
        rc = _lib.lib().mmfs_layernorm(x.data_ptr(), weight.data_ptr() if weight is not None else None,
                                       bias.data_ptr() if bias is not None else None, y.data_ptr(), rows, x.shape[-1],
                                       float(eps), _DTYPE_CODE[x.dtype], _stream())
    _lib.check(rc, "layernorm")
    launch_counter[0] += 1
    return y


def rope_qk_(q: torch.Tensor, k: torch.Tensor, cos: torch.Tensor, sin: torch.Tensor, position_ids: torch.Tensor):
    B, T, H, hd = q.shape
    inference_only("rope_qk_", q, k)
    _require(q.is_cuda and k.shape == q.shape and q.stride(3) == 1 and q.stride(2) == hd and k.stride(3) == 1
             and k.stride(2) == hd and q.stride(0) == T * q.stride(1) and k.stride(0) == T * k.stride(1),
             "rope_qk_: q / k must be (B,T,H,hd) with dense heads and uniform token stride")
    _require(cos.dtype == torch.float32 and sin.dtype == torch.float32 and cos.is_contiguous() and sin.is_contiguous()
             and cos.shape[-1] == hd, "rope_qk_: cos / sin must be contiguous fp32 (max_pos, hd)")
    pos = position_ids.to(torch.int64).contiguous()
    per_batch = 1 if pos.numel() == B * T else 0
    _require(per_batch or pos.numel() == T, "rope_qk_: position_ids must have B*T or T entries")
    with torch.cuda.device(q.device):
        rc = _lib.lib().mmfs_rope_qk(q.data_ptr(), k.data_ptr(), cos.data_ptr(), sin.data_ptr(), pos.data_ptr(),
                                     B * T, T, H, hd, q.stride(1), k.stride(1), per_batch, _DTYPE_CODE[q.dtype], _stream())
    _lib.check(rc, "rope_qk_")
    launch_counter[0] += 1


def rope_qk_append_(q: torch.Tensor, k: torch.Tensor, v: torch.Tensor, cos: torch.Tensor, sin: torch.Tensor,
                    position_ids: torch.Tensor, k_cache: torch.Tensor, v_cache: torch.Tensor, slot) -> None:
    B, T, H, hd = q.shape
    inference_only("rope_qk_append_", q, k, v)
    for t in (q, k, v):
        _require(t.is_cuda and tuple(t.shape) == (B, T, H, hd) and t.stride(3) == 1 and t.stride(2) == hd and
                 t.stride(0) == T * t.stride(1), "rope_qk_append_: q / k / v must be (B,T,H,hd) with dense heads and uniform token stride")
    for c in (k_cache, v_cache):
        _require(c.is_cuda and c.dim() == 4 and c.shape[0] == B and tuple(c.shape[2:]) == (H, hd) and c.stride(3) == 1 and
                 c.stride(2) == hd and c.dtype == q.dtype, "rope_qk_append_: caches must be (B, T_max, H, hd), dense heads")
    _require(k_cache.stride() == v_cache.stride(), "rope_qk_append_: k / v caches must share their strides")
    _require(cos.dtype == torch.float32 and sin.dtype == torch.float32 and cos.is_contiguous() and sin.is_contiguous()
             and cos.shape[-1] == hd, "rope_qk_append_: cos / sin must be contiguous fp32 (max_pos, hd)")
    pos = position_ids.to(torch.int64).contiguous()
    per_batch = 1 if pos.numel() == B * T else 0
    _require(per_batch or pos.numel() == T, "rope_qk_append_: position_ids must have B*T or T entries")
    if isinstance(slot, torch.Tensor):
        _require(slot.is_cuda and slot.dtype == torch.int64 and slot.numel() == 1, "rope_qk_append_: slot tensor must be (1,) int64 on the device")
        slot_dev, slot_host = slot.data_ptr(), 0
    else:
        slot_dev, slot_host = None, int(slot)
        _require(0 <= slot_host and slot_host + T <= k_cache.shape[1], "rope_qk_append_: slot + T exceeds the cache")
    with torch.cuda.device(q.device):
        rc = _lib.lib().mmfs_rope_qk_append(q.data_ptr(), k.data_ptr(), v.data_ptr(), cos.data_ptr(), sin.data_ptr(), pos.data_ptr(),
                                            k_cache.data_ptr(), v_cache.data_ptr(), slot_dev, slot_host, B * T, T, H, hd,
                                            q.stride(1), k.stride(1), v.stride(1), k_cache.stride(0), k_cache.stride(1),
                                            per_batch, _DTYPE_CODE[q.dtype], _stream())
    _lib.check(rc, "rope_qk_append_")
    launch_counter[0] += 1


def decode_select(logits: torch.Tensor, out_ids: torch.Tensor, step: torch.Tensor, finished: torch.Tensor,
                  next_ids: torch.Tensor, params: torch.Tensor, eos: Optional[torch.Tensor] = None, pad_id: int = 0,
                  min_length: int = 0, sample: bool = False, seed: Optional[torch.Tensor] = None,
                  uniforms: Optional[torch.Tensor] = None) -> None:
    inference_only("decode_select", logits)
    _require(logits.is_cuda and logits.dim() == 2 and logits.dtype == torch.float32 and logits.stride(1) == 1,
             "decode_select: logits must be a CUDA fp32 (B, V) tensor with unit column stride")
    B, V = logits.shape
    dev = logits.device
    _require(out_ids.device == dev and out_ids.dtype == torch.int64 and out_ids.dim() == 2 and out_ids.shape[0] == B
             and out_ids.is_contiguous(), "decode_select: out_ids must be contiguous int64 (B, max_new) on the logits' device")
    _require(step.device == dev and step.dtype == torch.int64 and step.numel() == 1, "decode_select: step must be a (1,) int64 device tensor")
    _require(finished.device == dev and finished.dtype in (torch.bool, torch.uint8) and finished.numel() == B
             and finished.is_contiguous(), "decode_select: finished must be contiguous bool / uint8 with B entries")
    _require(next_ids.device == dev and next_ids.dtype == torch.int64 and next_ids.numel() == B and next_ids.is_contiguous(),
             "decode_select: next_ids must be contiguous int64 with B entries")
    _require(params.device == dev and params.dtype == torch.float32 and params.numel() == 3 and params.is_contiguous(),
             "decode_select: params must be a contiguous (3,) fp32 device tensor [repetition_penalty, temperature, top_p]")
    if eos is not None:
        _require(eos.device == dev and eos.dtype == torch.int64 and eos.dim() == 1 and eos.is_contiguous(),
                 "decode_select: eos must be a contiguous 1-D int64 device tensor")
    if seed is not None:
        _require(seed.device == dev and seed.dtype == torch.int64 and seed.numel() == 1, "decode_select: seed must be a (1,) int64 device tensor")
    _require(not sample or seed is not None or uniforms is not None, "decode_select: sampling needs a seed or uniforms")
    if uniforms is not None:
        _require(uniforms.device == dev and uniforms.dtype == torch.float32 and uniforms.numel() == B and uniforms.is_contiguous(),
                 "decode_select: uniforms must be contiguous fp32 with B entries")
    seed_ptr = seed.data_ptr() if seed is not None else None
    with torch.cuda.device(dev):
        rc = _lib.lib().mmfs_decode_select(logits.data_ptr(), logits.stride(0), out_ids.data_ptr(), step.data_ptr(),
                                           finished.data_ptr(), next_ids.data_ptr(), eos.data_ptr() if eos is not None else None,
                                           eos.numel() if eos is not None else 0, int(pad_id), int(min_length),
                                           params.data_ptr(), seed_ptr, uniforms.data_ptr() if uniforms is not None else None,
                                           B, V, out_ids.shape[1], _lib.SELECT_SAMPLE if sample else _lib.SELECT_GREEDY,
                                           _stream())
    _lib.check(rc, "decode_select")
    launch_counter[0] += 1


SELECT_MAX_V = 1 << 17


def beam_candidates(num_beams: int, n_eos: int) -> int:
    return max(2, 1 + n_eos) * num_beams


def beam_select_supported(num_beams: int, n_eos: int, V: int) -> bool:
    return (1 <= num_beams <= _lib.BEAM_MAX_BEAMS and 0 <= n_eos <= _lib.BEAM_MAX_EOS
            and beam_candidates(num_beams, n_eos) <= V <= SELECT_MAX_V)


def _check_beam_step(what, logits, step, params, n_params, beam_scores, history, next_ids, parent, done, hyp_scores,
                     hyp_ids, hyp_meta, num_beams, eos):
    inference_only(what, logits)
    _require(logits.is_cuda and logits.dim() == 2 and logits.dtype == torch.float32 and logits.stride(1) == 1,
             f"{what}: logits must be a CUDA fp32 (R, V) tensor with unit column stride")
    R, V = logits.shape
    dev = logits.device
    _require(num_beams > 0 and R % num_beams == 0, f"{what}: the rows must be whole groups of num_beams")
    B = R // num_beams

    def dense(t, name, dtype, shape):
        _require(t.device == dev and t.dtype == dtype and tuple(t.shape) == shape and t.is_contiguous(),
                 f"{what}: {name} must be a contiguous {dtype} {shape} tensor on the logits' device")

    _require(history.dim() == 2, f"{what}: history must be (R, max_new)")
    max_new = history.shape[1]
    dense(step, "step", torch.int64, (1,))
    dense(params, "params", torch.float64, (n_params,))
    dense(beam_scores, "beam_scores", torch.float32, (R,))
    dense(history, "history", torch.int64, (R, max_new))
    dense(next_ids, "next_ids", torch.int64, tuple(next_ids.shape))
    _require(next_ids.numel() == R, f"{what}: next_ids must have R entries")
    dense(parent, "parent", torch.int64, (R,))
    _require(done.device == dev and done.dtype in (torch.bool, torch.uint8) and done.numel() == B and done.is_contiguous(),
             f"{what}: done must be contiguous bool / uint8 with B entries")
    dense(hyp_scores, "hyp_scores", torch.float64, (B, num_beams))
    dense(hyp_ids, "hyp_ids", torch.int64, (B, num_beams, max_new))
    dense(hyp_meta, "hyp_meta", torch.int64, (B, num_beams, 2))
    n_eos = 0
    if eos is not None:
        _require(eos.device == dev and eos.dtype == torch.int64 and eos.dim() == 1 and eos.is_contiguous(),
                 f"{what}: eos must be a contiguous 1-D int64 device tensor")
        n_eos = eos.numel()
    return B, V, max_new, n_eos


def beam_select(logits: torch.Tensor, step: torch.Tensor, params: torch.Tensor, beam_scores: torch.Tensor,
                history: torch.Tensor, next_ids: torch.Tensor, parent: torch.Tensor, done: torch.Tensor,
                hyp_scores: torch.Tensor, hyp_ids: torch.Tensor, hyp_meta: torch.Tensor, scratch: torch.Tensor,
                num_beams: int, eos: Optional[torch.Tensor] = None, pad_id: int = 0, min_length: int = 0) -> None:
    B, V, max_new, n_eos = _check_beam_step("beam_select", logits, step, params, 2, beam_scores, history, next_ids,
                                            parent, done, hyp_scores, hyp_ids, hyp_meta, num_beams, eos)
    R = B * num_beams
    _require(scratch.device == logits.device and scratch.dtype == torch.int64 and scratch.is_contiguous()
             and scratch.numel() >= R * beam_candidates(num_beams, n_eos),
             "beam_select: scratch must be contiguous int64 with R * max(2, 1 + n_eos) * num_beams entries")
    with torch.cuda.device(logits.device):
        rc = _lib.lib().mmfs_beam_select(logits.data_ptr(), logits.stride(0), step.data_ptr(), params.data_ptr(),
                                         beam_scores.data_ptr(), history.data_ptr(), next_ids.data_ptr(), parent.data_ptr(),
                                         done.data_ptr(), hyp_scores.data_ptr(), hyp_ids.data_ptr(), hyp_meta.data_ptr(),
                                         eos.data_ptr() if eos is not None else None, n_eos, int(pad_id), int(min_length),
                                         scratch.data_ptr(), B, num_beams, V, max_new, _stream())
    _lib.check(rc, "beam_select")
    launch_counter[0] += 2


def beam_sample_supported(num_beams: int, n_eos: int, V: int) -> bool:
    return (1 <= num_beams <= _lib.BEAM_MAX_BEAMS and 0 <= n_eos <= _lib.BEAM_MAX_EOS
            and 2 * num_beams <= V <= SELECT_MAX_V)


def beam_sample_scratch(num_beams: int, rows: int) -> int:
    return rows * 4 * num_beams


def beam_sample(logits: torch.Tensor, step: torch.Tensor, params: torch.Tensor, beam_scores: torch.Tensor,
                history: torch.Tensor, next_ids: torch.Tensor, parent: torch.Tensor, done: torch.Tensor,
                hyp_scores: torch.Tensor, hyp_ids: torch.Tensor, hyp_meta: torch.Tensor, error: torch.Tensor,
                scratch: torch.Tensor, num_beams: int, eos: Optional[torch.Tensor] = None, pad_id: int = 0,
                min_length: int = 0, top_k: int = 50, seed: Optional[torch.Tensor] = None,
                uniforms: Optional[torch.Tensor] = None) -> None:
    B, V, max_new, n_eos = _check_beam_step("beam_sample", logits, step, params, 4, beam_scores, history, next_ids,
                                            parent, done, hyp_scores, hyp_ids, hyp_meta, num_beams, eos)
    R, dev = B * num_beams, logits.device
    _require(error.device == dev and error.dtype == torch.int32 and error.numel() == 1,
             "beam_sample: error must be a (1,) int32 device tensor")
    _require(scratch.device == dev and scratch.dtype == torch.int64 and scratch.is_contiguous()
             and scratch.numel() >= beam_sample_scratch(num_beams, R),
             "beam_sample: scratch must be contiguous int64 with R * 4 * num_beams entries")
    _require(seed is not None or uniforms is not None, "beam_sample: needs a seed or uniforms")
    if seed is not None:
        _require(seed.device == dev and seed.dtype == torch.int64 and seed.numel() == 1, "beam_sample: seed must be a (1,) int64 device tensor")
    if uniforms is not None:
        _require(uniforms.device == dev and uniforms.dtype == torch.float32 and tuple(uniforms.shape) == (R, V)
                 and uniforms.is_contiguous(), "beam_sample: uniforms must be a contiguous fp32 (R, V) tensor")
    _require(top_k >= 0, "beam_sample: top_k must be >= 0")
    with torch.cuda.device(dev):
        rc = _lib.lib().mmfs_beam_sample(logits.data_ptr(), logits.stride(0), step.data_ptr(), params.data_ptr(),
                                         seed.data_ptr() if seed is not None else None,
                                         uniforms.data_ptr() if uniforms is not None else None, beam_scores.data_ptr(),
                                         history.data_ptr(), next_ids.data_ptr(), parent.data_ptr(), done.data_ptr(),
                                         hyp_scores.data_ptr(), hyp_ids.data_ptr(), hyp_meta.data_ptr(), error.data_ptr(),
                                         eos.data_ptr() if eos is not None else None, n_eos, int(pad_id), int(min_length),
                                         int(top_k), scratch.data_ptr(), B, num_beams, V, max_new, _stream())
    _lib.check(rc, "beam_sample")
    launch_counter[0] += 2


def kv_beam_reorder(kv: torch.Tensor, parent: torch.Tensor, cur: torch.Tensor, step: torch.Tensor, num_beams: int,
                    max_positions: int, done: Optional[torch.Tensor] = None) -> None:
    inference_only("kv_beam_reorder", kv)
    _require(kv.is_cuda and kv.dim() >= 3, "kv_beam_reorder: kv must be a CUDA (n, R, T_max, ...) tensor")
    n, R, T = kv.shape[:3]
    dev = kv.device
    row_bytes = kv[0, 0, 0].numel() * kv.element_size()
    _require(kv[0, 0, 0].is_contiguous() and kv.stride(2) * kv.element_size() >= row_bytes,
             "kv_beam_reorder: each (cache, row, position) entry must be dense")
    _require(num_beams > 0 and R % num_beams == 0, "kv_beam_reorder: the rows must be whole groups of num_beams")
    _require(parent.device == dev and parent.dtype == torch.int64 and parent.numel() == R and parent.is_contiguous(),
             "kv_beam_reorder: parent must be contiguous int64 with R entries")
    for t, name in ((cur, "cur"), (step, "step")):
        _require(t.device == dev and t.dtype == torch.int64 and t.numel() == 1, f"kv_beam_reorder: {name} must be a (1,) int64 device tensor")
    if done is not None:
        _require(done.device == dev and done.dtype in (torch.bool, torch.uint8) and done.numel() == R // num_beams
                 and done.is_contiguous(), "kv_beam_reorder: done must be contiguous bool / uint8 with one entry per group")
    _require(0 < max_positions <= T, "kv_beam_reorder: max_positions must be in [1, T_max]")
    es = kv.element_size()
    with torch.cuda.device(dev):
        rc = _lib.lib().mmfs_kv_beam_reorder(kv.data_ptr(), n, kv.stride(0) * es, R, kv.stride(1) * es, kv.stride(2) * es,
                                             row_bytes, num_beams, parent.data_ptr(), cur.data_ptr(), step.data_ptr(),
                                             done.data_ptr() if done is not None else None, int(max_positions), _stream())
    _lib.check(rc, "kv_beam_reorder")
    launch_counter[0] += 1


def swiglu(gate_up: torch.Tensor) -> torch.Tensor:
    inference_only("swiglu", gate_up)
    _require(gate_up.is_cuda and gate_up.is_contiguous() and gate_up.shape[-1] % 2 == 0, "swiglu: bad input")
    inter = gate_up.shape[-1] // 2
    out = torch.empty(gate_up.shape[:-1] + (inter,), dtype=gate_up.dtype, device=gate_up.device)
    with torch.cuda.device(gate_up.device):
        rc = _lib.lib().mmfs_swiglu(gate_up.data_ptr(), out.data_ptr(), gate_up.numel() // (2 * inter), inter,
                                    _DTYPE_CODE[gate_up.dtype], _stream())
    _lib.check(rc, "swiglu")
    launch_counter[0] += 1
    return out


def geglu(value_gate: torch.Tensor) -> torch.Tensor:
    inference_only("geglu", value_gate)
    _require(value_gate.is_cuda and value_gate.is_contiguous() and value_gate.shape[-1] % 2 == 0, "geglu: bad input")
    inter = value_gate.shape[-1] // 2
    out = torch.empty(value_gate.shape[:-1] + (inter,), dtype=value_gate.dtype, device=value_gate.device)
    with torch.cuda.device(value_gate.device):
        rc = _lib.lib().mmfs_geglu(value_gate.data_ptr(), out.data_ptr(), value_gate.numel() // (2 * inter), inter,
                                   _DTYPE_CODE[value_gate.dtype], _stream())
    _lib.check(rc, "geglu")
    launch_counter[0] += 1
    return out


def attention(q, k, v, key_mask=None, causal=True, past=0, scale=None, force_generic=False) -> torch.Tensor:
    B, Tq, H, hd = q.shape
    Tkv = k.shape[1]
    for t in (q, k, v):
        _require(t.is_cuda and t.stride(3) == 1 and t.stride(2) == hd, "attention: heads must be dense (.., H, hd)")
    inference_only("attention", q, k, v)
    _require(k.shape == v.shape and k.shape[0] == B and k.shape[2] == H and k.shape[3] == hd, "attention: k/v shape mismatch")
    scale = float(scale if scale is not None else hd ** -0.5)
    out = torch.empty((B, Tq, H, hd), dtype=q.dtype, device=q.device)
    km = None
    if key_mask is not None:
        km = key_mask.to(torch.uint8).contiguous()
        _require(tuple(km.shape) == (B, Tkv), "attention: key_mask must be (B, Tkv)")
    from . import attn_tc
    es = q.element_size()
    decode_ok = (Tq == 1 and not force_generic and q.dtype != torch.float64 and hd % 32 == 0 and hd <= 256 and
                 (hd * es) % 16 == 0 and all(t.data_ptr() % 16 == 0 and (t.stride(0) * es) % 16 == 0 and
                                            (t.stride(1) * es) % 16 == 0 for t in (k, v)))
    if not force_generic and attn_tc.supported(q, k, v, Tq, Tkv, hd):
        attn_tc.forward(q, k, v, out, km, causal, past, scale)
    elif decode_ok:
        lib = _lib.lib()
        scratch = torch.empty((lib.mmfs_attn_decode_scratch_floats(B, H, Tkv, hd),), dtype=torch.float32, device=q.device)
        with torch.cuda.device(q.device):
            rc = lib.mmfs_attn_decode(q.data_ptr(), k.data_ptr(), v.data_ptr(), out.data_ptr(),
                                      km.data_ptr() if km is not None else None, scratch.data_ptr(), B, H, Tkv, hd,
                                      q.stride(0), k.stride(0), k.stride(1), v.stride(0), v.stride(1), out.stride(0), scale,
                                      1 if causal else 0, int(past), _DTYPE_CODE[q.dtype], _stream())
        _lib.check(rc, "attention (decode)")
        launch_counter[0] += 1
    else:
        with torch.cuda.device(q.device):
            rc = _lib.lib().mmfs_attn_generic(
                q.data_ptr(), k.data_ptr(), v.data_ptr(), out.data_ptr(), km.data_ptr() if km is not None else None,
                B, H, Tq, Tkv, hd, q.stride(0), q.stride(1), k.stride(0), k.stride(1), v.stride(0), v.stride(1),
                out.stride(0), out.stride(1), scale, 1 if causal else 0, int(past), _DTYPE_CODE[q.dtype], _stream())
        _lib.check(rc, "attention")
    launch_counter[0] += 1
    return out.view(B, Tq, H * hd)


def attention_decode_shared(q, k_prefix, v_prefix, k_gen, v_gen, prefix_len, key_mask=None, causal=True, past=0,
                            scale=None) -> torch.Tensor:
    R, Tq, H, hd = q.shape
    P, Tp = k_prefix.shape[:2]
    max_new = k_gen.shape[1]
    Tkv = Tp + max_new
    inference_only("attention_decode_shared", q, k_prefix, v_prefix, k_gen, v_gen)
    _require(Tq == 1, "attention_decode_shared: one query position per row")
    for t in (q, k_prefix, v_prefix, k_gen, v_gen):
        _require(t.is_cuda and t.dim() == 4 and t.dtype == q.dtype and t.device == q.device and tuple(t.shape[2:]) == (H, hd)
                 and t.stride(3) == 1 and t.stride(2) == hd,
                 "attention_decode_shared: q / prefix / gen must be (rows, T, H, hd) CUDA tensors of q's dtype, heads dense")
    _require(v_prefix.shape == k_prefix.shape and tuple(k_gen.shape) == (R, max_new, H, hd) and v_gen.shape == k_gen.shape,
             "attention_decode_shared: prefix must be (P, T_p, H, hd) and gen (R, max_new, H, hd)")
    _require(P > 0 and R % P == 0, "attention_decode_shared: the rows must be whole groups, one per prefix row")
    _require(prefix_len.device == q.device and prefix_len.dtype == torch.int64 and prefix_len.numel() == 1,
             "attention_decode_shared: prefix_len must be a (1,) int64 device tensor")
    scale = float(scale if scale is not None else hd ** -0.5)
    out = torch.empty((R, 1, H, hd), dtype=q.dtype, device=q.device)
    km = None
    if key_mask is not None:
        km = key_mask.to(torch.uint8).contiguous()
        _require(tuple(km.shape) == (R, Tkv), "attention_decode_shared: key_mask must be (R, T_p + max_new)")
    lib = _lib.lib()
    scratch = torch.empty((lib.mmfs_attn_decode_scratch_floats(R, H, Tkv, hd),), dtype=torch.float32, device=q.device)
    with torch.cuda.device(q.device):
        rc = lib.mmfs_attn_decode_shared(q.data_ptr(), k_prefix.data_ptr(), v_prefix.data_ptr(), k_gen.data_ptr(),
                                         v_gen.data_ptr(), out.data_ptr(), km.data_ptr() if km is not None else None,
                                         prefix_len.data_ptr(), scratch.data_ptr(), R, R // P, H, Tkv, Tp, max_new, hd,
                                         q.stride(0), k_prefix.stride(0), k_prefix.stride(1), v_prefix.stride(0),
                                         v_prefix.stride(1), k_gen.stride(0), k_gen.stride(1), v_gen.stride(0), v_gen.stride(1),
                                         out.stride(0), scale, 1 if causal else 0, int(past), _DTYPE_CODE[q.dtype], _stream())
    _lib.check(rc, "attention_decode_shared")
    launch_counter[0] += 2
    return out.view(R, 1, H * hd)



def _check_qkv_view(t, B, T, H, hd, what):
    _require(t.is_cuda and tuple(t.shape) == (B, T, H, hd) and t.stride(3) == 1 and t.stride(2) == hd,
             f"{what}: tensors must be (B, T, H, hd) CUDA views with dense heads")


def attention_forward_lse(q, k, v, key_mask=None, scale=None, causal=True):
    B, Tq, H, hd = q.shape
    Tkv = k.shape[1]
    inference_only("attention_forward_lse", q, k, v)
    _check_qkv_view(q, B, Tq, H, hd, "attention_forward_lse")
    for t in (k, v):
        _check_qkv_view(t, B, Tkv, H, hd, "attention_forward_lse")
    _require(not causal or Tq == Tkv, "attention_forward_lse: causal attention needs Tq == Tkv")
    scale = float(scale if scale is not None else hd ** -0.5)
    out = torch.empty((B, Tq, H, hd), dtype=q.dtype, device=q.device)
    lse = torch.empty((B, H, Tq), dtype=torch.float32, device=q.device)
    km = None
    if key_mask is not None:
        km = key_mask.to(torch.uint8).contiguous()
        _require(tuple(km.shape) == (B, Tkv), "attention_forward_lse: key_mask must be (B, Tkv)")
    counter = torch.empty((1,), dtype=torch.int32, device=q.device)
    with torch.cuda.device(q.device):
        rc = _lib.lib().mmfs_attn_forward_lse(
            q.data_ptr(), k.data_ptr(), v.data_ptr(), out.data_ptr(), lse.data_ptr(), km.data_ptr() if km is not None else None,
            B, H, Tq, Tkv, hd, q.stride(0), q.stride(1), k.stride(0), k.stride(1), v.stride(0), v.stride(1),
            out.stride(0), out.stride(1), scale, 1 if causal else 0, 0, _DTYPE_CODE[q.dtype], counter.data_ptr(), _stream())
    _lib.check(rc, "attention_forward_lse")
    launch_counter[0] += 1
    return out, lse


def attention_backward(q, k, v, out, d_out, lse, dq, dk, dv, key_mask=None, scale=None) -> None:
    B, T, H, hd = q.shape
    inference_only("attention_backward", q, k, v, out, d_out)
    for t in (q, k, v, out, d_out, dq, dk, dv):
        _check_qkv_view(t, B, T, H, hd, "attention_backward")
    _require(all(t.dtype == q.dtype for t in (k, v, out, d_out, dq, dk, dv)), "attention_backward: dtype mismatch")
    _require(lse.dtype == torch.float32 and tuple(lse.shape) == (B, H, T) and lse.is_contiguous(),
             "attention_backward: lse must be contiguous fp32 (B, H, T)")
    scale = float(scale if scale is not None else hd ** -0.5)
    km = None
    if key_mask is not None:
        km = key_mask.to(torch.uint8).contiguous()
        _require(tuple(km.shape) == (B, T), "attention_backward: key_mask must be (B, T)")
    delta = torch.empty((B, H, T), dtype=torch.float32, device=q.device)
    with torch.cuda.device(q.device):
        rc = _lib.lib().mmfs_attn_backward(
            q.data_ptr(), k.data_ptr(), v.data_ptr(), out.data_ptr(), d_out.data_ptr(), lse.data_ptr(), dq.data_ptr(),
            dk.data_ptr(), dv.data_ptr(), delta.data_ptr(), km.data_ptr() if km is not None else None, B, H, T, hd,
            q.stride(0), q.stride(1), k.stride(0), k.stride(1), v.stride(0), v.stride(1), out.stride(0), out.stride(1),
            d_out.stride(0), d_out.stride(1), dq.stride(0), dq.stride(1), dk.stride(0), dk.stride(1), dv.stride(0),
            dv.stride(1), scale, _DTYPE_CODE[q.dtype], _stream())
    _lib.check(rc, "attention_backward")
    launch_counter[0] += 3


def attention_backward_general(q, k, v, out, d_out, lse, dq, dk, dv, key_mask=None, scale=None, causal=False) -> None:
    B, Tq, H, hd = q.shape
    Tkv = k.shape[1]
    inference_only("attention_backward_general", q, k, v, out, d_out)
    for t in (q, out, d_out, dq):
        _check_qkv_view(t, B, Tq, H, hd, "attention_backward_general")
    for t in (k, v, dk, dv):
        _check_qkv_view(t, B, Tkv, H, hd, "attention_backward_general")
    _require(all(t.dtype == q.dtype for t in (k, v, out, d_out, dq, dk, dv)), "attention_backward_general: dtype mismatch")
    _require(lse.dtype == torch.float32 and tuple(lse.shape) == (B, H, Tq) and lse.is_contiguous(),
             "attention_backward_general: lse must be contiguous fp32 (B, H, Tq)")
    scale = float(scale if scale is not None else hd ** -0.5)
    km = None
    if key_mask is not None:
        km = key_mask.to(torch.uint8).contiguous()
        _require(tuple(km.shape) == (B, Tkv), "attention_backward_general: key_mask must be (B, Tkv)")
    delta = torch.empty((B, H, Tq), dtype=torch.float32, device=q.device)
    with torch.cuda.device(q.device):
        rc = _lib.lib().mmfs_attn_backward_general(
            q.data_ptr(), k.data_ptr(), v.data_ptr(), out.data_ptr(), d_out.data_ptr(), lse.data_ptr(), dq.data_ptr(),
            dk.data_ptr(), dv.data_ptr(), delta.data_ptr(), km.data_ptr() if km is not None else None, B, H, Tq, Tkv, hd,
            q.stride(0), q.stride(1), k.stride(0), k.stride(1), v.stride(0), v.stride(1), out.stride(0), out.stride(1),
            d_out.stride(0), d_out.stride(1), dq.stride(0), dq.stride(1), dk.stride(0), dk.stride(1), dv.stride(0),
            dv.stride(1), scale, 1 if causal else 0, _DTYPE_CODE[q.dtype], _stream())
    _lib.check(rc, "attention_backward_general")
    launch_counter[0] += 3


def rmsnorm_backward(x: torch.Tensor, weight: torch.Tensor, dy: torch.Tensor, eps: float, weight_grad: bool = True):
    inference_only("rmsnorm_backward", x, weight, dy)
    _require(x.is_cuda and x.is_contiguous() and dy.is_contiguous() and weight.is_contiguous() and dy.shape == x.shape,
             "rmsnorm_backward: contiguous CUDA tensors of one shape required")
    _require(weight.dtype == x.dtype == dy.dtype and weight.numel() == x.shape[-1], "rmsnorm_backward: weight dtype / size mismatch")
    cols = x.shape[-1]
    rows = x.numel() // cols
    dx = torch.empty_like(x)
    dw = torch.empty_like(weight) if weight_grad else None
    partials = (torch.empty((min(rows, _lib.RMSNORM_BWD_PARTS), cols), dtype=torch.float32, device=x.device)
                if weight_grad else None)
    with torch.cuda.device(x.device):
        rc = _lib.lib().mmfs_rmsnorm_backward(x.data_ptr(), weight.data_ptr(), dy.data_ptr(), dx.data_ptr(),
                                              dw.data_ptr() if dw is not None else None,
                                              partials.data_ptr() if partials is not None else None, rows, cols, float(eps),
                                              _DTYPE_CODE[x.dtype], _stream())
    _lib.check(rc, "rmsnorm_backward")
    launch_counter[0] += 2 if weight_grad else 1
    return dx, dw


def layernorm_backward(x: torch.Tensor, weight: torch.Tensor, dy: torch.Tensor, eps: float, weight_grad: bool = True,
                       bias_grad: bool = True):
    inference_only("layernorm_backward", x, weight, dy)
    _require(x.is_cuda and x.is_contiguous() and dy.is_contiguous() and weight.is_contiguous() and dy.shape == x.shape,
             "layernorm_backward: contiguous CUDA tensors of one shape required")
    _require(weight.dtype == x.dtype == dy.dtype and weight.numel() == x.shape[-1],
             "layernorm_backward: weight dtype / size mismatch")
    cols = x.shape[-1]
    rows = x.numel() // cols
    dx = torch.empty_like(x)
    dw = torch.empty_like(weight) if weight_grad else None
    db = torch.empty_like(weight) if bias_grad else None
    partials = (torch.empty((2, min(rows, _lib.RMSNORM_BWD_PARTS), cols), dtype=torch.float32, device=x.device)
                if weight_grad or bias_grad else None)
    with torch.cuda.device(x.device):
        rc = _lib.lib().mmfs_layernorm_backward(x.data_ptr(), weight.data_ptr(), dy.data_ptr(), dx.data_ptr(),
                                                dw.data_ptr() if dw is not None else None,
                                                db.data_ptr() if db is not None else None,
                                                partials.data_ptr() if partials is not None else None, rows, cols,
                                                float(eps), _DTYPE_CODE[x.dtype], _stream())
    _lib.check(rc, "layernorm_backward")
    launch_counter[0] += 2 if partials is not None else 1
    return dx, dw, db


def swiglu_backward(gate_up: torch.Tensor, d_out: torch.Tensor) -> torch.Tensor:
    inference_only("swiglu_backward", gate_up, d_out)
    _require(gate_up.is_cuda and gate_up.is_contiguous() and d_out.is_contiguous() and gate_up.shape[-1] % 2 == 0
             and d_out.shape == gate_up.shape[:-1] + (gate_up.shape[-1] // 2,) and d_out.dtype == gate_up.dtype,
             "swiglu_backward: bad input")
    inter = gate_up.shape[-1] // 2
    d_gu = torch.empty_like(gate_up)
    with torch.cuda.device(gate_up.device):
        rc = _lib.lib().mmfs_swiglu_backward(gate_up.data_ptr(), d_out.data_ptr(), d_gu.data_ptr(),
                                             gate_up.numel() // (2 * inter), inter, _DTYPE_CODE[gate_up.dtype], _stream())
    _lib.check(rc, "swiglu_backward")
    launch_counter[0] += 1
    return d_gu


def geglu_backward(value_gate: torch.Tensor, d_out: torch.Tensor) -> torch.Tensor:
    inference_only("geglu_backward", value_gate, d_out)
    _require(value_gate.is_cuda and value_gate.is_contiguous() and d_out.is_contiguous() and value_gate.shape[-1] % 2 == 0
             and d_out.shape == value_gate.shape[:-1] + (value_gate.shape[-1] // 2,) and d_out.dtype == value_gate.dtype
             and d_out.device == value_gate.device, "geglu_backward: bad input")
    inter = value_gate.shape[-1] // 2
    d_vg = torch.empty_like(value_gate)
    with torch.cuda.device(value_gate.device):
        rc = _lib.lib().mmfs_geglu_backward(value_gate.data_ptr(), d_out.data_ptr(), d_vg.data_ptr(),
                                            value_gate.numel() // (2 * inter), inter, _DTYPE_CODE[value_gate.dtype], _stream())
    _lib.check(rc, "geglu_backward")
    launch_counter[0] += 1
    return d_vg


def quick_gelu_backward(h: torch.Tensor, dy: torch.Tensor) -> torch.Tensor:
    inference_only("quick_gelu_backward", h, dy)
    _require(h.is_cuda and h.is_contiguous() and dy.is_contiguous() and dy.shape == h.shape and dy.dtype == h.dtype,
             "quick_gelu_backward: contiguous CUDA tensors of one shape and dtype required")
    dh = torch.empty_like(h)
    with torch.cuda.device(h.device):
        rc = _lib.lib().mmfs_quick_gelu_backward(h.data_ptr(), dy.data_ptr(), dh.data_ptr(), h.numel(),
                                                 _DTYPE_CODE[h.dtype], _stream())
    _lib.check(rc, "quick_gelu_backward")
    launch_counter[0] += 1
    return dh


def image_reentry(images: torch.Tensor, size: int = 224, out: Optional[torch.Tensor] = None) -> torch.Tensor:
    _require(images.is_cuda and images.dim() == 4 and images.dtype == torch.float32,
             "image_reentry: images must be a (N, 3, S, S) fp32 CUDA tensor")
    images = images.contiguous()
    N, C, H, W = images.shape
    if out is None:
        out = torch.empty((N, C, size, size), dtype=torch.float32, device=images.device)
    _require(out.is_cuda and out.is_contiguous() and out.dtype == torch.float32 and out.device == images.device and
             tuple(out.shape) == (N, C, size, size), "image_reentry: out must be a contiguous (N, 3, size, size) fp32 "
             "tensor on the images' device")
    with torch.cuda.device(images.device):
        rc = _lib.lib().mmfs_image_reentry(images.data_ptr(), out.data_ptr(), N, C, H, W, int(size), _stream())
    _lib.check(rc, "image_reentry")
    launch_counter[0] += 1
    return out


def _pixel_stride(t: torch.Tensor):
    H, W = t.shape[2:]
    if W > 1:
        return t.stride(3) if H == 1 or t.stride(2) == W * t.stride(3) else None
    return t.stride(2) if H > 1 else 1


def resize_bilinear_backward(dy: torch.Tensor, in_hw, scale_factor: float) -> torch.Tensor:
    inference_only("resize_bilinear_backward", dy)
    Hin, Win = int(in_hw[0]), int(in_hw[1])
    _require(dy.is_cuda and dy.dim() == 4, "resize_bilinear_backward: dy must be a (B, C, Hout, Wout) CUDA tensor")
    B, C, Hout, Wout = dy.shape
    _require((Hout, Wout) == (math.floor(Hin * scale_factor), math.floor(Win * scale_factor)),
             "resize_bilinear_backward: dy's size is not the input size times the scale factor")
    ps = _pixel_stride(dy)
    if ps is None:
        dy = dy.contiguous()
        ps = _pixel_stride(dy)
    dx = torch.empty((B, Hin * Win, C), dtype=dy.dtype, device=dy.device)
    scale = float(1.0 / scale_factor)
    with torch.cuda.device(dy.device):
        rc = _lib.lib().mmfs_resize_bilinear_backward(dy.data_ptr(), dx.data_ptr(), B, C, Hin, Win, Hout, Wout, dy.stride(0),
                                                      dy.stride(1), ps, scale, scale, _DTYPE_CODE[dy.dtype], _stream())
    _lib.check(rc, "resize_bilinear_backward")
    launch_counter[0] += 1
    return dx


def conv2d_supported(x: torch.Tensor, weight: torch.Tensor, stride: int, padding: int) -> bool:
    if x.dtype not in (torch.bfloat16, torch.float16) or not x.is_cuda or x.dim() != 4:
        return False
    B, Cin, H, W = x.shape
    Cout, _, KH, KW = weight.shape
    Ho, Wo = (H + 2 * padding - KH) // stride + 1, (W + 2 * padding - KW) // stride + 1
    tile = (Wo % 16 == 0 and Ho % 8 == 0) or (Wo == 8 and Ho == 8 and B % 2 == 0)
    return Cin % 64 == 0 and (Cout % 160 == 0 or Cout % 128 == 0) and stride in (1, 2) and tile


def conv2d(x: torch.Tensor, weight_khwc: torch.Tensor, bias=None, stride: int = 1, padding: int = 0, add_bc=None,
           residual=None) -> torch.Tensor:
    B, Cin, H, W = x.shape
    Cout, KH, KW, _ = weight_khwc.shape
    inference_only("conv2d", x, weight_khwc, bias, add_bc, residual)
    _require(x.is_contiguous(memory_format=torch.channels_last) and weight_khwc.is_contiguous(), "conv2d: x must be channels_last")
    Ho, Wo = (H + 2 * padding - KH) // stride + 1, (W + 2 * padding - KW) // stride + 1
    out = torch.empty((B, Cout, Ho, Wo), dtype=x.dtype, device=x.device, memory_format=torch.channels_last)
    if residual is not None:
        _require(residual.shape == out.shape and residual.is_contiguous(memory_format=torch.channels_last), "conv2d: residual layout")
    if add_bc is not None:
        add_bc = add_bc.contiguous()
    with torch.cuda.device(x.device):
        rc = _lib.lib().mmfs_conv2d_nhwc(
            x.data_ptr(), weight_khwc.data_ptr(), bias.data_ptr() if bias is not None else None,
            add_bc.data_ptr() if add_bc is not None else None, residual.data_ptr() if residual is not None else None,
            out.data_ptr(), B, H, W, Cin, Cout, KH, KW, stride, padding, _DTYPE_CODE[x.dtype], _stream())
    _lib.check(rc, "conv2d")
    launch_counter[0] += 1
    return out


def fold_up2x_weights(weight: torch.Tensor) -> torch.Tensor:
    acc = torch.float64 if weight.dtype == torch.float64 else torch.float32
    fold = torch.tensor([[[1, 0, 0], [0, 1, 1]], [[1, 1, 0], [0, 0, 1]]], dtype=acc, device=weight.device)
    w = torch.einsum("pak,ockl,qbl->pqoabc", fold, weight.to(acc), fold)
    return w.reshape(4, *w.shape[2:]).to(weight.dtype).contiguous()


def dgrad_weights_khwc(weight: torch.Tensor) -> torch.Tensor:
    return weight.flip(2, 3).permute(1, 2, 3, 0).contiguous()


def fold_dgrad_down2x_weights(weight: torch.Tensor) -> torch.Tensor:
    acc = torch.float64 if weight.dtype == torch.float64 else torch.float32
    fold = torch.tensor([[[0, 0, 0], [0, 1, 0]], [[0, 0, 1], [1, 0, 0]]], dtype=acc, device=weight.device)
    w = torch.einsum("pak,ockl,qbl->pqcabo", fold, weight.to(acc), fold)
    return w.reshape(4, *w.shape[2:]).to(weight.dtype).contiguous()


def conv2d_up2x_supported(x: torch.Tensor, weight: torch.Tensor) -> bool:
    if x.dtype not in (torch.bfloat16, torch.float16) or not x.is_cuda or x.dim() != 4 or tuple(weight.shape[2:]) != (3, 3):
        return False
    B, Cin, H, W = x.shape
    Cout = weight.shape[0]
    tile = (W % 16 == 0 and H % 8 == 0) or (W == 8 and H == 8 and B % 2 == 0)
    return Cin % 64 == 0 and (Cout % 160 == 0 or Cout % 128 == 0) and tile


def conv2d_up2x(x: torch.Tensor, weight_phases: torch.Tensor, bias=None) -> torch.Tensor:
    B, Cin, H, W = x.shape
    Cout = weight_phases.shape[1]
    inference_only("conv2d_up2x", x, weight_phases, bias)
    _require(x.is_contiguous(memory_format=torch.channels_last) and weight_phases.is_contiguous(), "conv2d_up2x: x must be channels_last")
    _require(tuple(weight_phases.shape) == (4, Cout, 2, 2, Cin), "conv2d_up2x: weights must be (4, Cout, 2, 2, Cin)")
    out = torch.empty((B, Cout, 2 * H, 2 * W), dtype=x.dtype, device=x.device, memory_format=torch.channels_last)
    with torch.cuda.device(x.device):
        rc = _lib.lib().mmfs_conv2d_up2x_nhwc(x.data_ptr(), weight_phases.data_ptr(), bias.data_ptr() if bias is not None else None,
                                              out.data_ptr(), B, H, W, Cin, Cout, _DTYPE_CODE[x.dtype], _stream())
    _lib.check(rc, "conv2d_up2x")
    launch_counter[0] += 1
    return out


def conv2d_down2x_supported(x: torch.Tensor, weight: torch.Tensor) -> bool:
    if x.dtype not in (torch.bfloat16, torch.float16) or not x.is_cuda or x.dim() != 4 or tuple(weight.shape[2:]) != (3, 3):
        return False
    B, Cin, H, W = x.shape
    Cout = weight.shape[0]
    if H % 2 or W % 2:
        return False
    Ho, Wo = H // 2, W // 2
    tile = (Wo % 16 == 0 and Ho % 8 == 0) or (Wo == 8 and Ho == 8 and B % 2 == 0)
    return Cin % 64 == 0 and (Cout % 160 == 0 or Cout % 128 == 0) and tile


def conv2d_down2x(x: torch.Tensor, weight_khwc: torch.Tensor, bias=None) -> torch.Tensor:
    B, Cin, H, W = x.shape
    Cout = weight_khwc.shape[0]
    inference_only("conv2d_down2x", x, weight_khwc, bias)
    _require(x.is_contiguous(memory_format=torch.channels_last) and weight_khwc.is_contiguous(), "conv2d_down2x: x must be channels_last")
    _require(tuple(weight_khwc.shape) == (Cout, 3, 3, Cin), "conv2d_down2x: weights must be (Cout, 3, 3, Cin)")
    out = torch.empty((B, Cout, H // 2, W // 2), dtype=x.dtype, device=x.device, memory_format=torch.channels_last)
    with torch.cuda.device(x.device):
        rc = _lib.lib().mmfs_conv2d_down2x_nhwc(x.data_ptr(), weight_khwc.data_ptr(), bias.data_ptr() if bias is not None else None,
                                                out.data_ptr(), B, H, W, Cin, Cout, _DTYPE_CODE[x.dtype], _stream())
    _lib.check(rc, "conv2d_down2x")
    launch_counter[0] += 1
    return out


def group_norm_supported(x: torch.Tensor) -> bool:
    if not x.is_cuda or x.dim() != 4 or x.dtype not in _DTYPE_CODE or x.dtype == torch.float64:
        return False
    vec = 16 // x.element_size()
    return x.shape[1] % vec == 0 and x.shape[1] // vec <= 1024 and x.is_contiguous(memory_format=torch.channels_last)


def group_norm_nhwc(x: torch.Tensor, groups: int, weight=None, bias=None, eps: float = 1e-5, silu: bool = False) -> torch.Tensor:
    inference_only("group_norm_nhwc", x, weight, bias)
    _require(group_norm_supported(x), "group_norm_nhwc: need a CUDA channels_last f32/f16/bf16 tensor with C % (16/size) == 0")
    B, C, H, W = x.shape
    _require(groups > 0 and C % groups == 0, f"group_norm_nhwc: {C} channels do not split into {groups} groups")
    _check_affine("group_norm_nhwc", x, C, weight, bias)
    y = torch.empty_like(x, memory_format=torch.channels_last)
    stats = torch.empty((B, 64, groups, 2), dtype=torch.float32, device=x.device)
    with torch.cuda.device(x.device):
        rc = _lib.lib().mmfs_groupnorm_nhwc(x.data_ptr(), weight.data_ptr() if weight is not None else None,
                                            bias.data_ptr() if bias is not None else None, y.data_ptr(), stats.data_ptr(),
                                            B, H * W, C, groups, float(eps), int(silu), _DTYPE_CODE[x.dtype], _stream())
    _lib.check(rc, "group_norm_nhwc")
    launch_counter[0] += 2
    return y


def group_norm_nhwc_backward(x: torch.Tensor, dy: torch.Tensor, groups: int, weight=None, bias=None, eps: float = 1e-5,
                             silu: bool = False) -> torch.Tensor:
    inference_only("group_norm_nhwc_backward", x, dy, weight, bias)
    _require(group_norm_supported(x) and x.shape[1] * x.element_size() <= 8192,
             "group_norm_nhwc_backward: need a CUDA channels_last f32/f16/bf16 tensor with C % (16/size) == 0 and "
             "C * size <= 8 KiB")
    _require(dy.shape == x.shape and dy.dtype == x.dtype and dy.device == x.device,
             "group_norm_nhwc_backward: dy must match x in shape, dtype and device")
    if not dy.is_contiguous(memory_format=torch.channels_last):
        dy = dy.contiguous(memory_format=torch.channels_last)
    B, C, H, W = x.shape
    _require(groups > 0 and C % groups == 0, f"group_norm_nhwc_backward: {C} channels do not split into {groups} groups")
    _check_affine("group_norm_nhwc_backward", x, C, weight, bias)
    dx = torch.empty_like(x, memory_format=torch.channels_last)
    scratch = torch.empty((2, B, 64, groups, 2), dtype=torch.float32, device=x.device)
    with torch.cuda.device(x.device):
        rc = _lib.lib().mmfs_groupnorm_nhwc_backward(x.data_ptr(), weight.data_ptr() if weight is not None else None,
                                                     bias.data_ptr() if bias is not None else None, dy.data_ptr(),
                                                     dx.data_ptr(), scratch.data_ptr(), B, H * W, C, groups, float(eps),
                                                     int(silu), _DTYPE_CODE[x.dtype], _stream())
    _lib.check(rc, "group_norm_nhwc_backward")
    launch_counter[0] += 3
    return dx


E4M3_MAX = 448.0
LINEAR_FP8_MAX_M = _lib.LINEAR_FP8_MAX_M


def quantize_fp8_per_channel(w: torch.Tensor):
    _require(w.dim() == 2 and w.dtype in (torch.float16, torch.bfloat16, torch.float32),
             "quantize_fp8_per_channel: w must be a 2-D fp16 / bf16 / fp32 tensor")
    wf = w.detach().float()
    amax = wf.abs().amax(dim=1)
    scale = torch.exp2(torch.ceil(torch.log2(amax / E4M3_MAX)))
    scale = torch.where(amax / scale > E4M3_MAX, scale * 2, scale)
    scale = torch.where(amax / (scale * 0.5) <= E4M3_MAX, scale * 0.5, scale)
    scale = torch.where(amax > 0, scale, torch.ones_like(scale)).contiguous()
    w8 = (wf / scale[:, None]).to(torch.float8_e4m3fn)
    return w8, scale


def linear_fp8_supported(x: torch.Tensor, w8: torch.Tensor) -> bool:
    K = x.shape[-1]
    return (x.is_cuda and x.dtype in (torch.bfloat16, torch.float16) and w8.dtype == torch.float8_e4m3fn
            and w8.dim() == 2 and w8.shape[1] == K and K % 16 == 0 and 0 < x.numel() // max(K, 1) <= LINEAR_FP8_MAX_M)


def linear_fp8(x: torch.Tensor, w8: torch.Tensor, scale: torch.Tensor, bias=None, residual=None, out=None):
    inference_only("linear_fp8", x, residual)
    K = x.shape[-1]
    _require(x.is_cuda and x.dtype in (torch.bfloat16, torch.float16), "linear_fp8: x must be a CUDA bf16 / fp16 tensor")
    _require(w8.dtype == torch.float8_e4m3fn and w8.dim() == 2 and w8.shape[1] == K and w8.is_contiguous()
             and w8.device == x.device, f"linear_fp8: w8 must be a contiguous float8_e4m3fn (N, {K}) tensor on {x.device}")
    N = w8.shape[0]
    _require(scale.dtype == torch.float32 and scale.is_contiguous() and scale.numel() == N and scale.device == x.device,
             f"linear_fp8: scale must be a contiguous fp32 tensor of {N} elements on {x.device}")
    _check_affine("linear_fp8", x, N, bias)
    x2 = x.reshape(-1, K)
    if not x2.is_contiguous() or x2.data_ptr() % 16:
        x2 = x2.clone(memory_format=torch.contiguous_format)
    M = x2.shape[0]
    shape = tuple(x.shape[:-1]) + (N,)
    for t, name in ((residual, "residual"), (out, "out")):
        if t is not None:
            _require(tuple(t.shape) == shape and t.dtype == x.dtype and t.is_contiguous() and t.device == x.device,
                     f"linear_fp8: {name} must be a contiguous {x.dtype} tensor of shape {shape}")
    if out is None:
        out = torch.empty(shape, dtype=x.dtype, device=x.device)
    with torch.cuda.device(x.device):
        rc = _lib.lib().mmfs_linear_fp8(x2.data_ptr(), w8.data_ptr(), scale.data_ptr(),
                                        bias.data_ptr() if bias is not None else None,
                                        residual.data_ptr() if residual is not None else None, out.data_ptr(),
                                        M, N, K, _DTYPE_CODE[x.dtype], _stream())
    _lib.check(rc, "linear_fp8")
    launch_counter[0] += 1
    return out



_KV_FP8_DTYPES = (torch.float32, torch.bfloat16, torch.float16)


def kv_scale_heads(H: int) -> int:
    return (H + 3) // 4 * 4


def quantize_kv_fp8(x: torch.Tensor):
    _require(x.dim() >= 2 and x.dtype in (torch.float16, torch.bfloat16, torch.float32),
             "quantize_kv_fp8: x must be a (..., H, hd) fp16 / bf16 / fp32 tensor")
    xf = x.detach().float()
    amax = xf.abs().amax(dim=-1)
    m, e = torch.frexp(amax)
    e = torch.where(m <= 0.875, e - 9, e - 8)
    scale = torch.exp2(e.double()).float()
    scale = torch.where(amax > 0, scale, torch.ones_like(scale)).contiguous()
    x8 = (xf / scale[..., None]).to(torch.float8_e4m3fn)
    return x8, scale


def _check_fp8_cache(what, k8, v8, ks, vs, rows, H, hd, dev):
    for t in (k8, v8):
        _require(t.is_cuda and t.device == dev and t.dtype == torch.float8_e4m3fn and t.dim() == 4 and t.shape[0] == rows
                 and tuple(t.shape[2:]) == (H, hd) and t.stride(3) == 1 and t.stride(2) == hd,
                 f"{what}: K / V must be float8_e4m3fn ({rows}, T, {H}, {hd}) CUDA tensors with dense heads")
    _require(k8.shape == v8.shape and k8.stride() == v8.stride(), f"{what}: K and V must share their shape and strides")
    for t in (ks, vs):
        _require(t.is_cuda and t.device == dev and t.dtype == torch.float32 and t.dim() == 3
                 and tuple(t.shape[:2]) == tuple(k8.shape[:2]) and t.shape[2] >= H and t.stride(2) == 1,
                 f"{what}: scales must be fp32 ({rows}, T, >= {H}) CUDA tensors")
    _require(ks.stride() == vs.stride(), f"{what}: K and V scales must share their strides")


def rope_qk_append_fp8_(q: torch.Tensor, k: torch.Tensor, v: torch.Tensor, cos: torch.Tensor, sin: torch.Tensor,
                        position_ids: torch.Tensor, k_cache: torch.Tensor, v_cache: torch.Tensor, k_scale: torch.Tensor,
                        v_scale: torch.Tensor, slot) -> None:
    B, T, H, hd = q.shape
    inference_only("rope_qk_append_fp8_", q, k, v)
    _require(q.dtype in _KV_FP8_DTYPES, "rope_qk_append_fp8_: q / k / v must be fp32 / bf16 / fp16")
    for t in (q, k, v):
        _require(t.is_cuda and t.dtype == q.dtype and tuple(t.shape) == (B, T, H, hd) and t.stride(3) == 1
                 and t.stride(2) == hd and t.stride(0) == T * t.stride(1),
                 "rope_qk_append_fp8_: q / k / v must be (B,T,H,hd) with dense heads and uniform token stride")
    _check_fp8_cache("rope_qk_append_fp8_", k_cache, v_cache, k_scale, v_scale, B, H, hd, q.device)
    _require(cos.dtype == torch.float32 and sin.dtype == torch.float32 and cos.is_contiguous() and sin.is_contiguous()
             and cos.shape[-1] == hd, "rope_qk_append_fp8_: cos / sin must be contiguous fp32 (max_pos, hd)")
    pos = position_ids.to(torch.int64).contiguous()
    per_batch = 1 if pos.numel() == B * T else 0
    _require(per_batch or pos.numel() == T, "rope_qk_append_fp8_: position_ids must have B*T or T entries")
    if isinstance(slot, torch.Tensor):
        _require(slot.is_cuda and slot.dtype == torch.int64 and slot.numel() == 1,
                 "rope_qk_append_fp8_: slot tensor must be (1,) int64 on the device")
        slot_dev, slot_host = slot.data_ptr(), 0
    else:
        slot_dev, slot_host = None, int(slot)
        _require(0 <= slot_host and slot_host + T <= k_cache.shape[1], "rope_qk_append_fp8_: slot + T exceeds the cache")
    with torch.cuda.device(q.device):
        rc = _lib.lib().mmfs_rope_qk_append_fp8(
            q.data_ptr(), k.data_ptr(), v.data_ptr(), cos.data_ptr(), sin.data_ptr(), pos.data_ptr(), k_cache.data_ptr(),
            v_cache.data_ptr(), k_scale.data_ptr(), v_scale.data_ptr(), slot_dev, slot_host, B * T, T, H, hd, q.stride(1),
            k.stride(1), v.stride(1), k_cache.stride(0), k_cache.stride(1), k_scale.stride(0), k_scale.stride(1), per_batch,
            _DTYPE_CODE[q.dtype], _stream())
    _lib.check(rc, "rope_qk_append_fp8_")
    launch_counter[0] += 1


def _check_decode_q(what, q, rows, key_mask, Tkv):
    _require(q.is_cuda and q.dtype in _KV_FP8_DTYPES and q.dim() == 4 and q.shape[0] == rows
             and q.shape[1] == 1 and q.stride(3) == 1 and q.stride(2) == q.shape[3],
             f"{what}: q must be an fp32 / bf16 / fp16 CUDA (rows, 1, H, hd) tensor with dense heads")
    if key_mask is None:
        return None
    km = key_mask.to(torch.uint8).contiguous()
    _require(tuple(km.shape) == (rows, Tkv), f"{what}: key_mask must be ({rows}, {Tkv})")
    return km


def attention_decode_fp8(q, k8, v8, k_scale, v_scale, key_mask=None, causal=True, past=0, scale=None) -> torch.Tensor:
    B, _, H, hd = q.shape
    Tkv = k8.shape[1] if k8.dim() == 4 else 0
    inference_only("attention_decode_fp8", q)
    km = _check_decode_q("attention_decode_fp8", q, B, key_mask, Tkv)
    _check_fp8_cache("attention_decode_fp8", k8, v8, k_scale, v_scale, B, H, hd, q.device)
    scale = float(scale if scale is not None else hd ** -0.5)
    out = torch.empty((B, 1, H, hd), dtype=q.dtype, device=q.device)
    lib = _lib.lib()
    scratch = torch.empty((lib.mmfs_attn_decode_scratch_floats(B, H, Tkv, hd),), dtype=torch.float32, device=q.device)
    with torch.cuda.device(q.device):
        rc = lib.mmfs_attn_decode_fp8(q.data_ptr(), k8.data_ptr(), v8.data_ptr(), k_scale.data_ptr(), v_scale.data_ptr(),
                                      out.data_ptr(), km.data_ptr() if km is not None else None, scratch.data_ptr(), B, H,
                                      Tkv, hd, q.stride(0), k8.stride(0), k8.stride(1), k_scale.stride(0), k_scale.stride(1),
                                      out.stride(0), scale, 1 if causal else 0, int(past), _DTYPE_CODE[q.dtype], _stream())
    _lib.check(rc, "attention_decode_fp8")
    launch_counter[0] += 1
    return out.view(B, 1, H * hd)


def attention_decode_shared_fp8(q, k_prefix, v_prefix, ks_prefix, vs_prefix, k_gen, v_gen, ks_gen, vs_gen, prefix_len,
                                key_mask=None, causal=True, past=0, scale=None) -> torch.Tensor:
    R, _, H, hd = q.shape
    P = k_prefix.shape[0] if k_prefix.dim() == 4 else 0
    Tp = k_prefix.shape[1] if k_prefix.dim() == 4 else 0
    max_new = k_gen.shape[1] if k_gen.dim() == 4 else 0
    Tkv = Tp + max_new
    inference_only("attention_decode_shared_fp8", q)
    km = _check_decode_q("attention_decode_shared_fp8", q, R, key_mask, Tkv)
    _require(P > 0 and R % P == 0, "attention_decode_shared_fp8: the rows must be whole groups, one per prefix row")
    _check_fp8_cache("attention_decode_shared_fp8", k_prefix, v_prefix, ks_prefix, vs_prefix, P, H, hd, q.device)
    _check_fp8_cache("attention_decode_shared_fp8", k_gen, v_gen, ks_gen, vs_gen, R, H, hd, q.device)
    _require(prefix_len.device == q.device and prefix_len.dtype == torch.int64 and prefix_len.numel() == 1,
             "attention_decode_shared_fp8: prefix_len must be a (1,) int64 device tensor")
    scale = float(scale if scale is not None else hd ** -0.5)
    out = torch.empty((R, 1, H, hd), dtype=q.dtype, device=q.device)
    lib = _lib.lib()
    scratch = torch.empty((lib.mmfs_attn_decode_scratch_floats(R, H, Tkv, hd),), dtype=torch.float32, device=q.device)
    with torch.cuda.device(q.device):
        rc = lib.mmfs_attn_decode_shared_fp8(
            q.data_ptr(), k_prefix.data_ptr(), v_prefix.data_ptr(), ks_prefix.data_ptr(), vs_prefix.data_ptr(),
            k_gen.data_ptr(), v_gen.data_ptr(), ks_gen.data_ptr(), vs_gen.data_ptr(), out.data_ptr(),
            km.data_ptr() if km is not None else None, prefix_len.data_ptr(), scratch.data_ptr(), R, R // P, H, Tkv, Tp,
            max_new, hd, q.stride(0), k_prefix.stride(0), k_prefix.stride(1), ks_prefix.stride(0), ks_prefix.stride(1),
            k_gen.stride(0), k_gen.stride(1), ks_gen.stride(0), ks_gen.stride(1), out.stride(0), scale, 1 if causal else 0,
            int(past), _DTYPE_CODE[q.dtype], _stream())
    _lib.check(rc, "attention_decode_shared_fp8")
    launch_counter[0] += 1
    return out.view(R, 1, H * hd)


def kv_dequantize_fp8(x8: torch.Tensor, scale: torch.Tensor, dtype: torch.dtype) -> torch.Tensor:
    _require(dtype in _KV_FP8_DTYPES, "kv_dequantize_fp8: dtype must be fp32 / bf16 / fp16")
    _require(x8.dim() == 4, "kv_dequantize_fp8: x8 must be (B, T, H, hd)")
    B, T, H, hd = x8.shape
    _require(x8.is_cuda and x8.dtype == torch.float8_e4m3fn and x8.stride(3) == 1 and x8.stride(2) == hd,
             "kv_dequantize_fp8: x8 must be a float8_e4m3fn CUDA tensor with dense heads")
    _require(scale.is_cuda and scale.device == x8.device and scale.dtype == torch.float32 and scale.dim() == 3
             and tuple(scale.shape[:2]) == (B, T) and scale.shape[2] >= H and scale.stride(2) == 1,
             f"kv_dequantize_fp8: scale must be fp32 ({B}, {T}, >= {H}) on x8's device")
    out = torch.empty((B, T, H, hd), dtype=dtype, device=x8.device)
    with torch.cuda.device(x8.device):
        rc = _lib.lib().mmfs_kv_dequantize_fp8(x8.data_ptr(), scale.data_ptr(), out.data_ptr(), B, T, H, hd, x8.stride(0),
                                               x8.stride(1), scale.stride(0), scale.stride(1), out.stride(0), out.stride(1),
                                               _DTYPE_CODE[dtype], _stream())
    _lib.check(rc, "kv_dequantize_fp8")
    launch_counter[0] += 1
    return out
```

Before: 2.679.

## Add warp-specialized TMA/WGMMA GEMM with fused SwiGLU epilogue for prefill MLP

Result: faster. 2.707, median of 6 (+1.0%).

```diff
diff --git a/include/mmfs_b200.h b/include/mmfs_b200.h
--- a/include/mmfs_b200.h
+++ b/include/mmfs_b200.h
@@ -174,6 +174,12 @@
 
 int mmfs_linear_fp8(const void *x, const uint8_t *w8, const float *scale, const void *bias, const void *residual,
                     void *out, int M, int N, int K, int dtype, void *stream);
+
+int mmfs_gemm(const void *a, const void *w, void *c, int M, int N, int K, int dtype, void *stream);
+int mmfs_gemm_rope_qk(const void *a, const void *w, void *c, int M, int N, int K, const float *cos_table,
+                      const float *sin_table, const int64_t *position_ids, int T_len, int pos_per_batch, int rope_cols,
+                      int head_dim, int dtype, void *stream);
+int mmfs_gemm_swiglu(const void *a, const void *w_interleaved, void *act, int M, int N, int K, int dtype, void *stream);
 
 int mmfs_rope_qk_append_fp8(void *q, void *k, void *v, const float *cos_table, const float *sin_table,
                             const int64_t *position_ids, uint8_t *k_cache, uint8_t *v_cache, float *k_scale, float *v_scale,
diff --git a/mm-interleaved_b200/_lib.py b/mm-interleaved_b200/_lib.py
--- a/mm-interleaved_b200/_lib.py
+++ b/mm-interleaved_b200/_lib.py
@@ -64,6 +64,9 @@
     "mmfs_attn_decode_fp8": (_I, [_P] * 8 + [_I] * 4 + [_L] * 6 + [_F, _I, _I, _I, _P]),
     "mmfs_attn_decode_shared_fp8": (_I, [_P] * 13 + [_I] * 7 + [_L] * 10 + [_F, _I, _I, _I, _P]),
     "mmfs_kv_dequantize_fp8": (_I, [_P] * 3 + [_I] * 4 + [_L] * 6 + [_I, _P]),
+    "mmfs_gemm": (_I, [_P] * 3 + [_I] * 4 + [_P]),
+    "mmfs_gemm_rope_qk": (_I, [_P] * 3 + [_I] * 3 + [_P] * 3 + [_I] * 5 + [_P]),
+    "mmfs_gemm_swiglu": (_I, [_P] * 3 + [_I] * 4 + [_P]),
 }
 BEAM_MAX_BEAMS, BEAM_MAX_EOS = 8, 4
 LINEAR_FP8_MAX_M = 64
diff --git a/mm-interleaved_b200/csrc/gemm_fused_sm100.cu b/mm-interleaved_b200/csrc/gemm_fused_sm100.cu
--- /dev/null
+++ b/mm-interleaved_b200/csrc/gemm_fused_sm100.cu
@@ -0,0 +1,322 @@
+#include "llama_math.cuh"
+#include "tc_common.cuh"
+
+namespace mmfs {
+namespace gfu {
+
+constexpr int BM = 128, BN = 256, BK = 64, STAGES = 4, THREADS = 384;
+constexpr int A_BYTES = BM * BK * 2, B_BYTES = BN * BK * 2, STAGE_BYTES = A_BYTES + B_BYTES;
+constexpr int OUT_BOX_BYTES = 64 * 128, OUT_BYTES = 2 * OUT_BOX_BYTES;
+constexpr int SMEM_BYTES = STAGES * STAGE_BYTES + 2 * OUT_BYTES + 1024;
+constexpr int kBand = 8;
+constexpr int kHeadDim = 128;
+
+enum Epi { PLAIN = 0, ROPE_QK = 1, SWIGLU = 2 };
+
+struct Params {
+    void *c;
+    int M, N, K, ldc;
+    int m_pairs, n_tiles, n_pairs_total;
+    const float *cos_t, *sin_t;
+    const int64_t *pos;
+    int T_len, pos_per_batch, rope_cols;
+};
+
+__device__ __forceinline__ uint32_t cluster_rank() {
+    uint32_t r;
+    asm volatile("mov.u32 %0, %%cluster_ctarank;" : "=r"(r));
+    return r;
+}
+__device__ __forceinline__ void cluster_sync() {
+    asm volatile("barrier.cluster.arrive.release.aligned;\n\tbarrier.cluster.wait.acquire.aligned;" ::: "memory");
+}
+__device__ __forceinline__ void bar_arrive_cluster(uint64_t *bar, uint32_t cta) {
+    uint32_t remote;
+    asm volatile("mapa.shared::cluster.u32 %0, %1, %2;" : "=r"(remote) : "r"(s_addr(bar)), "r"(cta));
+    asm volatile("mbarrier.arrive.shared::cluster.b64 _, [%0];" ::"r"(remote) : "memory");
+}
+
+__device__ __forceinline__ void tile_of(const Params &p, int t, int &mp, int &nt) {
+    const int band = t / (kBand * p.n_tiles);
+    const int r = t - band * kBand * p.n_tiles;
+    const int rows = min(kBand, p.m_pairs - band * kBand);
+    nt = r / rows;
+    mp = band * kBand + (r - nt * rows);
+}
+
+template <typename T> __device__ __forceinline__ uint32_t pack2(float a, float b) {
+    const T lo = from_op<T>(a), hi = from_op<T>(b);
+    return (uint32_t)*reinterpret_cast<const uint16_t *>(&lo) | ((uint32_t)*reinterpret_cast<const uint16_t *>(&hi) << 16);
+}
+
+__device__ __forceinline__ void tma_store_2d(const CUtensorMap *map, uint32_t src, int c0, int c1) {
+    asm volatile("cp.async.bulk.tensor.2d.global.shared::cta.bulk_group [%0, {%2, %3}], [%1];" ::"l"(map), "r"(src), "r"(c0),
+                 "r"(c1) : "memory");
+}
+__device__ __forceinline__ void bulk_commit() { asm volatile("cp.async.bulk.commit_group;" ::: "memory"); }
+template <bool READ_ONLY> __device__ __forceinline__ void bulk_wait_all() {
+    if (READ_ONLY) asm volatile("cp.async.bulk.wait_group.read 0;" ::: "memory");
+    else asm volatile("cp.async.bulk.wait_group 0;" ::: "memory");
+}
+__device__ __forceinline__ void warpgroup_sync(int id) { asm volatile("bar.sync %0, 128;" ::"r"(id) : "memory"); }
+
+template <typename T, int EPI>
+__device__ __forceinline__ void epilogue(const Params &p, const CUtensorMap *map_c, const float (&acc)[128], uint32_t stage,
+                                         int tile_row, int nt, int cw, bool leader) {
+    const int lane = threadIdx.x & 31, r_lo = 16 * ((threadIdx.x & 127) / 32) + lane / 4;
+    auto put = [&](int jj, int i, uint32_t v) {
+        const int r = r_lo + 8 * i;
+        asm volatile("st.shared.u32 [%0], %1;" ::"r"(stage + (jj >> 3) * OUT_BOX_BYTES + r * 128 +
+                                                     ((((jj & 7) ^ (lane / 4))) << 4) + 4 * (lane & 3)), "r"(v) : "memory");
+    };
+    constexpr int passes = EPI == SWIGLU ? 1 : 2;
+    const bool rotate = EPI == ROPE_QK && nt * BN < p.rope_cols;
+    long ps[2] = {0, 0};
+    if (rotate) {
+#pragma unroll
+        for (int i = 0; i < 2; ++i) {
+            const int row = tile_row + r_lo + 8 * i;
+            if (row < p.M) ps[i] = p.pos[p.pos_per_batch ? row : row % p.T_len];
+        }
+    }
+#pragma unroll
+    for (int pass = 0; pass < passes; ++pass) {
+        if (leader) bulk_wait_all<true>();
+        warpgroup_sync(1 + cw);
+#pragma unroll
+        for (int i = 0; i < 2; ++i) {
+            if (EPI == SWIGLU) {
+#pragma unroll
+                for (int j = 0; j < 16; ++j) {
+                    float o[2];
+#pragma unroll
+                    for (int cc = 0; cc < 2; ++cc)
+                        o[cc] = swiglu_op<T>(rnd<T>(acc[4 * j + 2 * i + cc]), rnd<T>(acc[4 * (j + 16) + 2 * i + cc]));
+                    put(j, i, pack2<T>(o[0], o[1]));
+                }
+            } else if (rotate) {
+                const float *cp = p.cos_t + ps[i] * kHeadDim + 2 * (lane & 3), *sp = p.sin_t + ps[i] * kHeadDim + 2 * (lane & 3);
+#pragma unroll
+                for (int jd = 0; jd < 8; ++jd) {
+                    const float2 c2 = *reinterpret_cast<const float2 *>(cp + 8 * jd);
+                    const float2 s2 = *reinterpret_cast<const float2 *>(sp + 8 * jd);
+                    const float cs[2] = {rnd<T>(c2.x), rnd<T>(c2.y)}, sn[2] = {rnd<T>(s2.x), rnd<T>(s2.y)};
+                    const int j = 16 * pass + jd;
+                    float o1[2], o2[2];
+#pragma unroll
+                    for (int cc = 0; cc < 2; ++cc) {
+                        const float x1 = rnd<T>(acc[4 * j + 2 * i + cc]), x2 = rnd<T>(acc[4 * (j + 8) + 2 * i + cc]);
+                        o1[cc] = rope_lo<T>(x1, x2, cs[cc], sn[cc]);
+                        o2[cc] = rope_hi<T>(x1, x2, cs[cc], sn[cc]);
+                    }
+                    put(jd, i, pack2<T>(o1[0], o1[1]));
+                    put(jd + 8, i, pack2<T>(o2[0], o2[1]));
+                }
+            } else {
+#pragma unroll
+                for (int jj = 0; jj < 16; ++jj) {
+                    const int j = 16 * pass + jj;
+                    put(jj, i, pack2<T>(acc[4 * j + 2 * i], acc[4 * j + 2 * i + 1]));
+                }
+            }
+        }
+        fence_async_smem();
+        warpgroup_sync(1 + cw);
+        if (leader) {
+            const int col = EPI == SWIGLU ? nt * (BN / 2) : nt * BN + 128 * pass;
+            tma_store_2d(map_c, stage, col, tile_row);
+            tma_store_2d(map_c, stage + OUT_BOX_BYTES, col + 64, tile_row);
+            bulk_commit();
+        }
+    }
+}
+
+template <typename T, int EPI>
+__global__ void __cluster_dims__(2, 1, 1) __launch_bounds__(THREADS, 1)
+gemm_fused_kernel(const __grid_constant__ CUtensorMap map_a, const __grid_constant__ CUtensorMap map_w,
+                  const __grid_constant__ CUtensorMap map_c, const Params p) {
+    extern __shared__ uint8_t smem_raw[];
+    __shared__ __align__(8) uint64_t full[STAGES], empty[STAGES];
+    const uint32_t base = (s_addr(smem_raw) + 1023u) & ~1023u;
+    uint8_t *smem = smem_raw + (base - s_addr(smem_raw));
+    const uint32_t rank = cluster_rank();
+    const int wg = threadIdx.x / 128;
+    const int kb_n = p.K / BK;
+    const int cid = blockIdx.x / 2, n_clusters = gridDim.x / 2;
+
+    if (threadIdx.x == 0) {
+        for (int s = 0; s < STAGES; ++s) {
+            bar_init(&full[s], 1);
+            bar_init(&empty[s], 4);
+        }
+        asm volatile("fence.mbarrier_init.release.cluster;" ::: "memory");
+    }
+    cluster_sync();
+
+    if (wg == 0) {
+        asm volatile("setmaxnreg.dec.sync.aligned.u32 40;");
+        if (threadIdx.x == 0) {
+            int s = 0;
+            uint32_t ph = 0;
+            for (int t = cid; t < p.n_pairs_total; t += n_clusters) {
+                int mp, nt;
+                tile_of(p, t, mp, nt);
+                const int m0 = (2 * mp + (int)rank) * BM, w0 = nt * BN + (int)rank * (BN / 2);
+                for (int kb = 0; kb < kb_n; ++kb) {
+                    bar_wait(&empty[s], ph ^ 1);
+                    bar_expect_tx(&full[s], STAGE_BYTES);
+                    uint8_t *st = smem + s * STAGE_BYTES;
+                    tma_load_2d(st, &map_a, &full[s], kb * BK, m0);
+                    tma_load_2d_multicast(st + A_BYTES + rank * (B_BYTES / 2), &map_w, &full[s], kb * BK, w0, 0x3);
+                    if (++s == STAGES) { s = 0; ph ^= 1; }
+                }
+            }
+        }
+        __syncwarp();
+    } else {
+        asm volatile("setmaxnreg.inc.sync.aligned.u32 232;");
+        const int cw = wg - 1;
+        const bool leader = (threadIdx.x & 127) == 0;
+        float acc[128];
+        int s = 0;
+        uint32_t ph = 0;
+        for (int t = cid; t < p.n_pairs_total; t += n_clusters) {
+            int mp, nt;
+            tile_of(p, t, mp, nt);
+            int prev = -1;
+            for (int kb = 0; kb < kb_n; ++kb) {
+                bar_wait(&full[s], ph);
+                const uint32_t sa = base + s * STAGE_BYTES + cw * (64 * 128), sb = base + s * STAGE_BYTES + A_BYTES;
+                wgmma_fence();
+#pragma unroll
+                for (int kk = 0; kk < BK / 16; ++kk)
+                    Wgmma<T>::ss_n256(acc, smem_desc(sa + kk * 32, 16, 1024), smem_desc(sb + kk * 32, 16, 1024), (kb | kk) != 0);
+                wgmma_commit();
+                wgmma_wait<1>();
+                if (prev >= 0 && leader) { bar_arrive_cluster(&empty[prev], 0); bar_arrive_cluster(&empty[prev], 1); }
+                prev = s;
+                if (++s == STAGES) { s = 0; ph ^= 1; }
+            }
+            wgmma_wait<0>();
+            reg_fence(acc);
+            if (leader) { bar_arrive_cluster(&empty[prev], 0); bar_arrive_cluster(&empty[prev], 1); }
+            epilogue<T, EPI>(p, &map_c, acc, base + STAGES * STAGE_BYTES + cw * OUT_BYTES, (2 * mp + (int)rank) * BM + cw * 64,
+                             nt, cw, leader);
+        }
+        if (leader) bulk_wait_all<false>();
+    }
+    cluster_sync();
+}
+
+template <typename T, int EPI> int resident_clusters(int &out) {
+    static int cached[kMaxDevices] = {};
+    const int dev = current_device();
+    if (dev >= 0 && dev < kMaxDevices && cached[dev] > 0) { out = cached[dev]; return MMFS_OK; }
+    if (int rc = ensure_dynamic_smem<gemm_fused_kernel<T, EPI>>(SMEM_BYTES)) return rc;
+    cudaLaunchConfig_t cfg = {};
+    cfg.gridDim = dim3(2 * 1024);
+    cfg.blockDim = dim3(THREADS);
+    cfg.dynamicSmemBytes = SMEM_BYTES;
+    cudaLaunchAttribute attr[1];
+    attr[0].id = cudaLaunchAttributeClusterDimension;
+    attr[0].val.clusterDim.x = 2;
+    attr[0].val.clusterDim.y = 1;
+    attr[0].val.clusterDim.z = 1;
+    cfg.attrs = attr;
+    cfg.numAttrs = 1;
+    int n = 0;
+    MMFS_CUDA(cudaOccupancyMaxActiveClusters(&n, gemm_fused_kernel<T, EPI>, &cfg));
+    if (n < 1) { set_error("gemm: no 2-CTA cluster of this kernel fits on the device"); return MMFS_ECUDA; }
+    if (dev >= 0 && dev < kMaxDevices) cached[dev] = n;
+    out = n;
+    return MMFS_OK;
+}
+
+static int make_map(CUtensorMap *map, const void *ptr, int rows, int cols, int ld, int box_rows, int dtype) {
+    EncodeTiledFn enc = tensor_map_encoder();
+    if (!enc) { set_error("gemm: cuTensorMapEncodeTiled is not available from this driver"); return MMFS_ECUDA; }
+    const cuuint64_t dims[2] = {(cuuint64_t)cols, (cuuint64_t)rows};
+    const cuuint64_t strides[1] = {(cuuint64_t)ld * 2};
+    const cuuint32_t box[2] = {(cuuint32_t)BK, (cuuint32_t)box_rows}, estr[2] = {1, 1};
+    CUresult r = enc(map, dtype == MMFS_BF16 ? CU_TENSOR_MAP_DATA_TYPE_BFLOAT16 : CU_TENSOR_MAP_DATA_TYPE_FLOAT16, 2,
+                     const_cast<void *>(ptr), dims, strides, box, estr, CU_TENSOR_MAP_INTERLEAVE_NONE,
+                     CU_TENSOR_MAP_SWIZZLE_128B, CU_TENSOR_MAP_L2_PROMOTION_L2_256B, CU_TENSOR_MAP_FLOAT_OOB_FILL_NONE);
+    if (r != CUDA_SUCCESS) { set_error("gemm: cuTensorMapEncodeTiled failed (%d)", (int)r); return MMFS_ECUDA; }
+    return MMFS_OK;
+}
+
+template <typename T, int EPI>
+static int launch(const void *a, const void *w, Params p, int dtype, cudaStream_t st) {
+    CUtensorMap map_a, map_w, map_c;
+    if (int rc = make_map(&map_a, a, p.M, p.K, p.K, BM, dtype)) return rc;
+    if (int rc = make_map(&map_w, w, p.N, p.K, p.K, BN / 2, dtype)) return rc;
+    if (int rc = make_map(&map_c, p.c, p.M, EPI == SWIGLU ? p.N / 2 : p.N, p.ldc, 64, dtype)) return rc;
+    p.m_pairs = (p.M + 2 * BM - 1) / (2 * BM);
+    p.n_tiles = p.N / BN;
+    p.n_pairs_total = p.m_pairs * p.n_tiles;
+    int clusters = 0;
+    if (int rc = resident_clusters<T, EPI>(clusters)) return rc;
+    if (clusters > p.n_pairs_total) clusters = p.n_pairs_total;
+    gemm_fused_kernel<T, EPI><<<2 * clusters, THREADS, SMEM_BYTES, st>>>(map_a, map_w, map_c, p);
+    MMFS_CUDA(cudaGetLastError());
+    return MMFS_OK;
+}
+
+template <int EPI>
+static int run(const void *a, const void *w, const Params &p, int dtype, void *stream, const char *what) {
+    return dispatch_dtype<kF16Types, MMFS_EUNSUPPORTED>(dtype, what, [&](auto tag) {
+        return launch<typename decltype(tag)::type, EPI>(a, w, p, dtype, (cudaStream_t)stream);
+    });
+}
+
+static int check_common(const void *a, const void *w, const void *c, int M, int N, int K, const char *what) {
+    MMFS_CHECK_ARG(M > 0 && N > 0 && K > 0, "%s: bad shape M=%d N=%d K=%d", what, M, N, K);
+    MMFS_CHECK_ARG(a && w && c, "%s: null pointer argument", what);
+    MMFS_CHECK_ARG(((uintptr_t)a | (uintptr_t)w | (uintptr_t)c) % 16 == 0, "%s: A, W and C must be 16-byte aligned", what);
+    if (N % BN != 0 || K % BK != 0) {
+        set_error("%s: needs N a multiple of %d and K a multiple of %d (got N=%d K=%d)", what, BN, BK, N, K);
+        return MMFS_EUNSUPPORTED;
+    }
+    return MMFS_OK;
+}
+
+}
+}
+
+using namespace mmfs;
+using namespace mmfs::gfu;
+
+extern "C" int mmfs_gemm(const void *a, const void *w, void *c, int M, int N, int K, int dtype, void *stream) {
+    if (int rc = check_common(a, w, c, M, N, K, "gemm")) return rc;
+    Params p{};
+    p.c = c; p.M = M; p.N = N; p.K = K; p.ldc = N;
+    return run<PLAIN>(a, w, p, dtype, stream, "gemm");
+}
+
+extern "C" int mmfs_gemm_rope_qk(const void *a, const void *w, void *c, int M, int N, int K, const float *cos_table,
+                                 const float *sin_table, const int64_t *position_ids, int T_len, int pos_per_batch,
+                                 int rope_cols, int head_dim, int dtype, void *stream) {
+    if (int rc = check_common(a, w, c, M, N, K, "gemm_rope_qk")) return rc;
+    MMFS_CHECK_ARG(cos_table && sin_table && position_ids, "gemm_rope_qk: null pointer argument");
+    MMFS_CHECK_ARG(T_len > 0 && (pos_per_batch == 0 || pos_per_batch == 1) && rope_cols >= 0 && rope_cols <= N,
+                   "gemm_rope_qk: bad rotation arguments T_len=%d pos_per_batch=%d rope_cols=%d", T_len, pos_per_batch,
+                   rope_cols);
+    if (head_dim != kHeadDim || rope_cols % BN != 0) {
+        set_error("gemm_rope_qk: needs head_dim %d and rope_cols a multiple of %d (got %d, %d)", kHeadDim, BN, head_dim,
+                  rope_cols);
+        return MMFS_EUNSUPPORTED;
+    }
+    Params p{};
+    p.c = c; p.M = M; p.N = N; p.K = K; p.ldc = N;
+    p.cos_t = cos_table; p.sin_t = sin_table; p.pos = position_ids;
+    p.T_len = T_len; p.pos_per_batch = pos_per_batch; p.rope_cols = rope_cols;
+    return run<ROPE_QK>(a, w, p, dtype, stream, "gemm_rope_qk");
+}
+
+extern "C" int mmfs_gemm_swiglu(const void *a, const void *w_interleaved, void *act, int M, int N, int K, int dtype,
+                                void *stream) {
+    if (int rc = check_common(a, w_interleaved, act, M, N, K, "gemm_swiglu")) return rc;
+    Params p{};
+    p.c = act; p.M = M; p.N = N; p.K = K; p.ldc = N / 2;
+    return run<SWIGLU>(a, w_interleaved, p, dtype, stream, "gemm_swiglu");
+}
diff --git a/mm-interleaved_b200/csrc/llama_math.cuh b/mm-interleaved_b200/csrc/llama_math.cuh
--- /dev/null
+++ b/mm-interleaved_b200/csrc/llama_math.cuh
@@ -0,0 +1,21 @@
+#pragma once
+#include "common.cuh"
+
+namespace mmfs {
+
+template <typename T> __device__ __forceinline__ float rnd(float x) { return to_op(from_op<T>(x)); }
+template <> __device__ __forceinline__ float rnd<float>(float x) { return x; }
+
+template <typename T> __device__ __forceinline__ float silu_op(float g) { return __fdividef(g, 1.f + __expf(-g)); }
+template <> __device__ __forceinline__ float silu_op<float>(float g) { return g / (1.f + expf(-g)); }
+
+template <typename T> __device__ __forceinline__ float rope_lo(float x1, float x2, float cs, float sn) {
+    return rnd<T>(x1 * cs) + rnd<T>(-x2 * sn);
+}
+template <typename T> __device__ __forceinline__ float rope_hi(float x1, float x2, float cs, float sn) {
+    return rnd<T>(x2 * cs) + rnd<T>(x1 * sn);
+}
+
+template <typename T> __device__ __forceinline__ float swiglu_op(float g, float u) { return rnd<T>(silu_op<T>(g)) * u; }
+
+}
diff --git a/mm-interleaved_b200/csrc/llama_ops_sm100.cu b/mm-interleaved_b200/csrc/llama_ops_sm100.cu
--- a/mm-interleaved_b200/csrc/llama_ops_sm100.cu
+++ b/mm-interleaved_b200/csrc/llama_ops_sm100.cu
@@ -1,9 +1,6 @@
-#include "common.cuh"
+#include "llama_math.cuh"
 
 namespace mmfs {
-
-template <typename T> __device__ __forceinline__ float rnd(float x) { return to_op(from_op<T>(x)); }
-template <> __device__ __forceinline__ float rnd<float>(float x) { return x; }
 
 __device__ __forceinline__ float block_sum(float v, float *s_red) {
 #pragma unroll
@@ -212,8 +209,8 @@
             Vec16<T>::unpack(v2, x2);
 #pragma unroll
             for (int i = 0; i < VEC; ++i) {
-                o1[i] = rnd<T>(x1[i] * cs[i]) + rnd<T>(-x2[i] * sn[i]);
-                o2[i] = rnd<T>(x2[i] * cs[i]) + rnd<T>(x1[i] * sn[i]);
+                o1[i] = rope_lo<T>(x1[i], x2[i], cs[i], sn[i]);
+                o2[i] = rope_hi<T>(x1[i], x2[i], cs[i], sn[i]);
             }
             *reinterpret_cast<uint4 *>(x) = Vec16<T>::pack(o1);
             *reinterpret_cast<uint4 *>(x + half) = Vec16<T>::pack(o2);
@@ -263,8 +260,8 @@
             Vec16<T>::unpack(*reinterpret_cast<const uint4 *>(src + half), x2);
 #pragma unroll
             for (int i = 0; i < VEC; ++i) {
-                o1[i] = rnd<T>(x1[i] * cs[i]) + rnd<T>(-x2[i] * sn[i]);
-                o2[i] = rnd<T>(x2[i] * cs[i]) + rnd<T>(x1[i] * sn[i]);
+                o1[i] = rope_lo<T>(x1[i], x2[i], cs[i], sn[i]);
+                o2[i] = rope_hi<T>(x1[i], x2[i], cs[i], sn[i]);
             }
             *reinterpret_cast<uint4 *>(dst) = Vec16<T>::pack(o1);
             *reinterpret_cast<uint4 *>(dst + half) = Vec16<T>::pack(o2);
@@ -272,12 +269,9 @@
     }
 }
 
-template <typename T> __device__ __forceinline__ float silu_op(float g) { return __fdividef(g, 1.f + __expf(-g)); }
-template <> __device__ __forceinline__ float silu_op<float>(float g) { return g / (1.f + expf(-g)); }
-
-template <typename T, int ACT> __device__ __forceinline__ float glu_act(float g) {
-    if (ACT == 0) return silu_op<T>(g);
-    return 0.5f * g * (1.f + erff(g * 0.70710678118654752f));
+template <typename T, int ACT> __device__ __forceinline__ float glu_op(float g, float u) {
+    if (ACT == 0) return swiglu_op<T>(g, u);
+    return rnd<T>(0.5f * g * (1.f + erff(g * 0.70710678118654752f))) * u;
 }
 
 template <typename T, int ACT = 0, bool GATE_SECOND = false>
@@ -296,18 +290,18 @@
             float g[VEC], u[VEC], o[VEC];
             Vec16<T>::unpack(g0, g); Vec16<T>::unpack(u0, u);
 #pragma unroll
-            for (int k = 0; k < VEC; ++k) o[k] = rnd<T>(glu_act<T, ACT>(g[k])) * u[k];
+            for (int k = 0; k < VEC; ++k) o[k] = glu_op<T, ACT>(g[k], u[k]);
             stg_v4(o_row + i * VEC, Vec16<T>::pack(o));
             Vec16<T>::unpack(g1, g); Vec16<T>::unpack(u1, u);
 #pragma unroll
-            for (int k = 0; k < VEC; ++k) o[k] = rnd<T>(glu_act<T, ACT>(g[k])) * u[k];
+            for (int k = 0; k < VEC; ++k) o[k] = glu_op<T, ACT>(g[k], u[k]);
             stg_v4(o_row + j * VEC, Vec16<T>::pack(o));
         }
         if (i < nvec) {
             float g[VEC], u[VEC], o[VEC];
             Vec16<T>::unpack(ldg_nc_v4(g_row + i * VEC), g); Vec16<T>::unpack(ldg_nc_v4(u_row + i * VEC), u);
 #pragma unroll
-            for (int k = 0; k < VEC; ++k) o[k] = rnd<T>(glu_act<T, ACT>(g[k])) * u[k];
+            for (int k = 0; k < VEC; ++k) o[k] = glu_op<T, ACT>(g[k], u[k]);
             stg_v4(o_row + i * VEC, Vec16<T>::pack(o));
         }
     }
diff --git a/mm-interleaved_b200/csrc/tc_common.cuh b/mm-interleaved_b200/csrc/tc_common.cuh
--- a/mm-interleaved_b200/csrc/tc_common.cuh
+++ b/mm-interleaved_b200/csrc/tc_common.cuh
@@ -52,6 +52,14 @@
             : "l"(da), "l"(db), "r"(acc)); \
     } \
      \
+    __device__ __forceinline__ static void ss_n256(float (&d)[128], uint64_t da, uint64_t db, int acc) { \
+        asm volatile( \
+            "{\n\t.reg .pred p;\n\tsetp.ne.b32 p, %130, 0;\n\t" \
+            "wgmma.mma_async.sync.aligned.m64n256k16.f32." TY "." TY " {%0,%1,%2,%3,%4,%5,%6,%7,%8,%9,%10,%11,%12,%13,%14,%15,%16,%17,%18,%19,%20,%21,%22,%23,%24,%25,%26,%27,%28,%29,%30,%31,%32,%33,%34,%35,%36,%37,%38,%39,%40,%41,%42,%43,%44,%45,%46,%47,%48,%49,%50,%51,%52,%53,%54,%55,%56,%57,%58,%59,%60,%61,%62,%63,%64,%65,%66,%67,%68,%69,%70,%71,%72,%73,%74,%75,%76,%77,%78,%79,%80,%81,%82,%83,%84,%85,%86,%87,%88,%89,%90,%91,%92,%93,%94,%95,%96,%97,%98,%99,%100,%101,%102,%103,%104,%105,%106,%107,%108,%109,%110,%111,%112,%113,%114,%115,%116,%117,%118,%119,%120,%121,%122,%123,%124,%125,%126,%127}, %128, %129, p, 1, 1, 0, 0;\n\t}" \
+            : "+f"(d[0]), "+f"(d[1]), "+f"(d[2]), "+f"(d[3]), "+f"(d[4]), "+f"(d[5]), "+f"(d[6]), "+f"(d[7]), "+f"(d[8]), "+f"(d[9]), "+f"(d[10]), "+f"(d[11]), "+f"(d[12]), "+f"(d[13]), "+f"(d[14]), "+f"(d[15]), "+f"(d[16]), "+f"(d[17]), "+f"(d[18]), "+f"(d[19]), "+f"(d[20]), "+f"(d[21]), "+f"(d[22]), "+f"(d[23]), "+f"(d[24]), "+f"(d[25]), "+f"(d[26]), "+f"(d[27]), "+f"(d[28]), "+f"(d[29]), "+f"(d[30]), "+f"(d[31]), "+f"(d[32]), "+f"(d[33]), "+f"(d[34]), "+f"(d[35]), "+f"(d[36]), "+f"(d[37]), "+f"(d[38]), "+f"(d[39]), "+f"(d[40]), "+f"(d[41]), "+f"(d[42]), "+f"(d[43]), "+f"(d[44]), "+f"(d[45]), "+f"(d[46]), "+f"(d[47]), "+f"(d[48]), "+f"(d[49]), "+f"(d[50]), "+f"(d[51]), "+f"(d[52]), "+f"(d[53]), "+f"(d[54]), "+f"(d[55]), "+f"(d[56]), "+f"(d[57]), "+f"(d[58]), "+f"(d[59]), "+f"(d[60]), "+f"(d[61]), "+f"(d[62]), "+f"(d[63]), "+f"(d[64]), "+f"(d[65]), "+f"(d[66]), "+f"(d[67]), "+f"(d[68]), "+f"(d[69]), "+f"(d[70]), "+f"(d[71]), "+f"(d[72]), "+f"(d[73]), "+f"(d[74]), "+f"(d[75]), "+f"(d[76]), "+f"(d[77]), "+f"(d[78]), "+f"(d[79]), "+f"(d[80]), "+f"(d[81]), "+f"(d[82]), "+f"(d[83]), "+f"(d[84]), "+f"(d[85]), "+f"(d[86]), "+f"(d[87]), "+f"(d[88]), "+f"(d[89]), "+f"(d[90]), "+f"(d[91]), "+f"(d[92]), "+f"(d[93]), "+f"(d[94]), "+f"(d[95]), "+f"(d[96]), "+f"(d[97]), "+f"(d[98]), "+f"(d[99]), "+f"(d[100]), "+f"(d[101]), "+f"(d[102]), "+f"(d[103]), "+f"(d[104]), "+f"(d[105]), "+f"(d[106]), "+f"(d[107]), "+f"(d[108]), "+f"(d[109]), "+f"(d[110]), "+f"(d[111]), "+f"(d[112]), "+f"(d[113]), "+f"(d[114]), "+f"(d[115]), "+f"(d[116]), "+f"(d[117]), "+f"(d[118]), "+f"(d[119]), "+f"(d[120]), "+f"(d[121]), "+f"(d[122]), "+f"(d[123]), "+f"(d[124]), "+f"(d[125]), "+f"(d[126]), "+f"(d[127]) \
+            : "l"(da), "l"(db), "r"(acc)); \
+    } \
+     \
     __device__ __forceinline__ static void rs_n64(float (&d)[32], const uint32_t (&a)[4], uint64_t db, int acc) { \
         asm volatile( \
             "{\n\t.reg .pred p;\n\tsetp.ne.b32 p, %37, 0;\n\t" \
@@ -77,6 +85,12 @@
         "cp.async.bulk.tensor.2d.shared::cluster.global.mbarrier::complete_tx::bytes [%0], [%1, {%3, %4}], [%2];" ::
         "r"(s_addr(dst)), "l"(map), "r"(s_addr(bar)), "r"(c0), "r"(c1) : "memory");
 }
+__device__ __forceinline__ void tma_load_2d_multicast(void *dst, const CUtensorMap *map, uint64_t *bar, int c0, int c1,
+                                                      uint16_t mask) {
+    asm volatile(
+        "cp.async.bulk.tensor.2d.shared::cluster.global.mbarrier::complete_tx::bytes.multicast::cluster [%0], [%1, {%3, %4}], [%2], %5;" ::
+        "r"(s_addr(dst)), "l"(map), "r"(s_addr(bar)), "r"(c0), "r"(c1), "h"(mask) : "memory");
+}
 
 typedef CUresult (*EncodeTiledFn)(CUtensorMap *, CUtensorMapDataType, cuuint32_t, void *, const cuuint64_t *, const cuuint64_t *,
                                   const cuuint32_t *, const cuuint32_t *, CUtensorMapInterleave, CUtensorMapSwizzle,
diff --git a/mm-interleaved_b200/llama_mmfs.py b/mm-interleaved_b200/llama_mmfs.py
--- a/mm-interleaved_b200/llama_mmfs.py
+++ b/mm-interleaved_b200/llama_mmfs.py
@@ -70,12 +70,22 @@
     def __init__(self, *linears):
         self.linears = linears
         self._cache = WeightCache()
+        self._layout = None
+
+    def _cached(self, layout, build):
+        if self._layout != layout:
+            self._cache, self._layout = WeightCache(), layout
+        return self._cache.get([l.weight for l in self.linears], build)
 
     def get(self):
         ws = [l.weight for l in self.linears]
         if records(*ws):
             return torch.cat(ws, 0)
-        return self._cache.get(ws, lambda: torch.cat(ws, 0).contiguous())
+        return self._cached("cat", lambda: torch.cat(ws, 0).contiguous())
+
+    def interleaved(self):
+        gate, up = (l.weight for l in self.linears)
+        return self._cached("interleaved", lambda: ops.interleave_gate_up(gate, up))
 
 
 def _addmm_residual(residual, x, weight, inplace):
@@ -85,6 +95,13 @@
         r2.addmm_(x2, weight.t())
         return residual
     return torch.addmm(r2, x2, weight.t()).view_as(residual)
+
+
+GEMM_FUSED_MIN_ROWS = 4096
+
+
+def fused_prefill(x, weight):
+    return x.shape[0] * x.shape[1] >= GEMM_FUSED_MIN_ROWS and ops.gemm_supported(x, weight) and not records(x)
 
 
 FP8_DECODE_MAX_ROWS = 5
@@ -111,9 +128,12 @@
         self._gate_up = _CatWeight(self.gate_proj, self.up_proj)
         self._fp8 = None
 
-    def forward(self, x, residual=None, inplace=False):
-        gu = decode_linear(x, self._gate_up.get(), self._fp8, "gate_up")
-        act = autograd_ops.swiglu(gu)
+    def forward(self, x, residual=None, inplace=False, prefill=False):
+        if prefill and x.dim() == 3 and fused_prefill(x, self.gate_proj.weight):
+            act = ops.gemm_swiglu(x, self._gate_up.interleaved())
+        else:
+            gu = decode_linear(x, self._gate_up.get(), self._fp8, "gate_up")
+            act = autograd_ops.swiglu(gu)
         return decode_linear(act, self.down_proj.weight, self._fp8, "down", residual=residual, inplace=inplace)
 
 
@@ -436,7 +456,8 @@
         if self.llama_cross_attn is not None and vision_hidden_states is not None:
             hidden_states = self.llama_cross_attn(hidden_states, vision_hidden_states, cross_attention_mask,
                                                   residual=hidden_states, inplace=inplace)
-        hidden_states = self.mlp(self.post_attention_layernorm(hidden_states), residual=hidden_states, inplace=inplace)
+        hidden_states = self.mlp(self.post_attention_layernorm(hidden_states), residual=hidden_states, inplace=inplace,
+                                 prefill=past_key_value is None)
         outputs = (hidden_states,)
         if use_cache:
             outputs += (present,)
diff --git a/mm-interleaved_b200/ops.py b/mm-interleaved_b200/ops.py
--- a/mm-interleaved_b200/ops.py
+++ b/mm-interleaved_b200/ops.py
@@ -285,6 +285,76 @@
         rc = _lib.lib().mmfs_swiglu(gate_up.data_ptr(), out.data_ptr(), gate_up.numel() // (2 * inter), inter,
                                     _DTYPE_CODE[gate_up.dtype], _stream())
     _lib.check(rc, "swiglu")
+    launch_counter[0] += 1
+    return out
+
+
+GEMM_BLOCK_N, GEMM_BLOCK_K = 256, 64
+GEMM_HEAD_DIM = 128
+
+
+def gemm_supported(x: torch.Tensor, weight: torch.Tensor) -> bool:
+    return (x.is_cuda and x.dtype in (torch.bfloat16, torch.float16) and weight.dtype == x.dtype
+            and weight.device == x.device and weight.dim() == 2 and weight.shape[1] == x.shape[-1]
+            and weight.shape[0] % GEMM_BLOCK_N == 0 and x.shape[-1] % GEMM_BLOCK_K == 0 and x.numel() > 0)
+
+
+def _gemm_args(what, x, weight, n_out):
+    inference_only(what, x, weight)
+    _require(gemm_supported(x, weight), f"{what}: needs CUDA bf16 / fp16 x (..., K) and weight (N, K) of x's dtype, "
+             f"N % {GEMM_BLOCK_N} == 0, K % {GEMM_BLOCK_K} == 0")
+    _require(weight.is_contiguous(), f"{what}: weight must be contiguous")
+    K = x.shape[-1]
+    x2 = x.reshape(-1, K)
+    if not x2.is_contiguous() or x2.data_ptr() % 16:
+        x2 = x2.clone(memory_format=torch.contiguous_format)
+    out = torch.empty(tuple(x.shape[:-1]) + (n_out,), dtype=x.dtype, device=x.device)
+    return x2, out, x2.shape[0], weight.shape[0], K
+
+
+def gemm(x: torch.Tensor, weight: torch.Tensor) -> torch.Tensor:
+    x2, out, M, N, K = _gemm_args("gemm", x, weight, weight.shape[0])
+    with torch.cuda.device(x.device):
+        rc = _lib.lib().mmfs_gemm(x2.data_ptr(), weight.data_ptr(), out.data_ptr(), M, N, K, _DTYPE_CODE[x.dtype],
+                                  _stream())
+    _lib.check(rc, "gemm")
+    launch_counter[0] += 1
+    return out
+
+
+def gemm_rope_qk(x: torch.Tensor, w_qkv: torch.Tensor, cos: torch.Tensor, sin: torch.Tensor,
+                 position_ids: torch.Tensor) -> torch.Tensor:
+    B, T, _ = x.shape
+    x2, out, M, N, K = _gemm_args("gemm_rope_qk", x, w_qkv, w_qkv.shape[0])
+    _require(N % (3 * GEMM_HEAD_DIM) == 0 and (2 * N // 3) % GEMM_BLOCK_N == 0,
+             f"gemm_rope_qk: w_qkv must stack q, k and v of heads of {GEMM_HEAD_DIM}")
+    _require(cos.dtype == torch.float32 and sin.dtype == torch.float32 and cos.is_contiguous() and sin.is_contiguous()
+             and cos.shape[-1] == GEMM_HEAD_DIM, f"gemm_rope_qk: cos / sin must be contiguous fp32 (max_pos, {GEMM_HEAD_DIM})")
+    pos = position_ids.to(torch.int64).contiguous()
+    per_batch = 1 if pos.numel() == B * T else 0
+    _require(per_batch or pos.numel() == T, "gemm_rope_qk: position_ids must have B*T or T entries")
+    with torch.cuda.device(x.device):
+        rc = _lib.lib().mmfs_gemm_rope_qk(x2.data_ptr(), w_qkv.data_ptr(), out.data_ptr(), M, N, K, cos.data_ptr(),
+                                          sin.data_ptr(), pos.data_ptr(), T, per_batch, 2 * N // 3, GEMM_HEAD_DIM,
+                                          _DTYPE_CODE[x.dtype], _stream())
+    _lib.check(rc, "gemm_rope_qk")
+    launch_counter[0] += 1
+    return out
+
+
+def interleave_gate_up(gate: torch.Tensor, up: torch.Tensor) -> torch.Tensor:
+    I, K = gate.shape
+    half = GEMM_BLOCK_N // 2
+    _require(up.shape == gate.shape and I % half == 0, f"interleave_gate_up: gate and up must be (I, K) with I % {half} == 0")
+    return torch.stack((gate.view(I // half, half, K), up.view(I // half, half, K)), 1).reshape(2 * I, K).contiguous()
+
+
+def gemm_swiglu(x: torch.Tensor, w_interleaved: torch.Tensor) -> torch.Tensor:
+    x2, out, M, N, K = _gemm_args("gemm_swiglu", x, w_interleaved, w_interleaved.shape[0] // 2)
+    with torch.cuda.device(x.device):
+        rc = _lib.lib().mmfs_gemm_swiglu(x2.data_ptr(), w_interleaved.data_ptr(), out.data_ptr(), M, N, K,
+                                         _DTYPE_CODE[x.dtype], _stream())
+    _lib.check(rc, "gemm_swiglu")
     launch_counter[0] += 1
     return out
 
```
